# NilsJochem/audio-matcher

Hardware: AMD Instinct MI355X
Metric: audio samples/s matched (whole node), 10 s needle vs 1 h haystack, 1/2/4/8 GPU (higher is better)
Workload: dtype f32

## Files before the change

audio-matcher_amd/build.py:

```python
from __future__ import annotations

import os
import shutil
import subprocess
import sys
from concurrent.futures import ThreadPoolExecutor

HERE = os.path.dirname(os.path.abspath(__file__))
CSRC = os.path.join(HERE, "csrc")
OBJ = os.path.join(HERE, "build")
LIB = os.path.join(HERE, "libaudiomatch_amd.so")
SOURCES = ["am_fft.hip", "am_peaks.hip", "am_context.hip", "am_correlate.hip", "am_engine.hip", "am_stream.hip", "am_monitor.hip", "am_pool.hip", "am_norm.hip", "am_hits.hip", "am_segments.hip", "am_bands.hip", "am_significance.hip", "am_resample.hip", "am_whiten.hip", "am_estimate.hip",
           "am_best.hip", "am_api.hip"]
HEADERS = [os.path.join(CSRC, "am_kernels.h"), os.path.join(CSRC, "am_internal.h"), os.path.join(CSRC, "am_walk.h"), os.path.join(CSRC, "am_spans.h"),
           os.path.join(HERE, "..", "include", "audiomatch.h")]
ARCH = "gfx950"
FLAGS = ["-O3", "-std=c++17", "-fPIC", f"--offload-arch={ARCH}", "-ffp-contract=fast", "-fno-slp-vectorize",
         "-Wall", "-Wno-unused-result"]


def _hipcc() -> str:
    for cand in (shutil.which("hipcc"), "/opt/rocm/bin/hipcc"):
        if cand and os.path.exists(cand):
            return cand
    raise RuntimeError("hipcc not found: the HIP extension cannot be built")


def _stale(target: str, deps: list[str]) -> bool:
    if not os.path.exists(target):
        return True
    t = os.path.getmtime(target)
    return any(os.path.getmtime(d) > t for d in deps if os.path.exists(d))


def build_library(force: bool = False, verbose: bool = False) -> str:
    srcs = [os.path.join(CSRC, s) for s in SOURCES]
    if not force and not _stale(LIB, srcs + HEADERS + [os.path.abspath(__file__)]):
        return LIB
    os.makedirs(OBJ, exist_ok=True)
    hipcc = _hipcc()

    def compile_one(src: str) -> str:
        obj = os.path.join(OBJ, os.path.basename(src) + ".o")
        if force or _stale(obj, [src] + HEADERS + [os.path.abspath(__file__)]):
            cmd = [hipcc, *FLAGS, "-c", src, "-o", obj]
            if verbose:
                print(" ".join(cmd), file=sys.stderr)
            subprocess.check_call(cmd)
        return obj

    with ThreadPoolExecutor(max_workers=len(srcs)) as ex:
        objs = list(ex.map(compile_one, srcs))
    cmd = [hipcc, "-shared", "-fPIC", f"--offload-arch={ARCH}", "-o", LIB, *objs]
    if verbose:
        print(" ".join(cmd), file=sys.stderr)
    subprocess.check_call(cmd)
    return LIB


def build_variant(name: str, defines: list[str]) -> str:
    vdir = os.path.join(OBJ, "variants")
    odir = os.path.join(OBJ, "variants_obj", name)
    os.makedirs(vdir, exist_ok=True)
    os.makedirs(odir, exist_ok=True)
    hipcc = _hipcc()
    objs = []
    for s_ in SOURCES:
        obj = os.path.join(odir, s_ + ".o")
        subprocess.check_call([hipcc, *FLAGS, *[f"-D{d}" for d in defines], "-c", os.path.join(CSRC, s_), "-o", obj])
        objs.append(obj)
    out = os.path.join(vdir, name + ".so")
    subprocess.check_call([hipcc, "-shared", "-fPIC", f"--offload-arch={ARCH}", "-o", out, *objs])
    return out


CLI = os.path.join(HERE, "bin", "audiomatch")
HOST = os.path.join(HERE, "host")


def build_cli(force: bool = False) -> str:
    lib = build_library()
    srcs = [os.path.join(HOST, "audiomatch_cli.cpp"), os.path.join(HOST, "am_host.hpp")]
    if not force and not _stale(CLI, srcs + [lib]):
        return CLI
    os.makedirs(os.path.dirname(CLI), exist_ok=True)
    cmd = [_hipcc(), "-O2", "-std=c++17", "-x", "c++", srcs[0], "-o", CLI,
           f"-L{HERE}", "-laudiomatch_amd", "-Wl,-rpath,$ORIGIN/.."]
    subprocess.check_call(cmd)
    return CLI


PUSHBENCH = os.path.join(HERE, "bin", "pushbench")


def build_pushbench(force: bool = False) -> str:
    lib = build_library()
    src = os.path.join(HOST, "pushbench.cpp")
    if not force and not _stale(PUSHBENCH, [src, lib]):
        return PUSHBENCH
    os.makedirs(os.path.dirname(PUSHBENCH), exist_ok=True)
    subprocess.check_call([_hipcc(), "-O2", "-std=c++17", "-x", "c++", src, "-o", PUSHBENCH,
                           f"-L{HERE}", "-laudiomatch_amd", "-Wl,-rpath,$ORIGIN/.."])
    return PUSHBENCH


def build_selftest() -> str:
    out = os.path.join(OBJ, "am_host_selftest")
    os.makedirs(OBJ, exist_ok=True)
    src = os.path.join(HOST, "selftest.cpp")
    if _stale(out, [src, os.path.join(HOST, "am_host.hpp")]):
        subprocess.check_call(["g++", "-std=c++17", "-O1", "-I", os.path.join(HERE, "..", "include"), "-o", out, src])
    return out


if __name__ == "__main__":
    print(build_library(force="--force" in sys.argv, verbose=True))
    print(build_cli(force="--force" in sys.argv))
    print(build_pushbench(force="--force" in sys.argv))
```

audio-matcher_amd/csrc/am_context.hip:

```cpp
#include "am_internal.h"

namespace am {

thread_local std::string t_err;

int fail(int code, const std::string& msg) {
    t_err = msg;
    return code;
}
int hip_fail(hipError_t e, const char* what) {
    char buf[256];
    snprintf(buf, sizeof(buf), "%s: %s", what, hipGetErrorString(e));
    t_err = buf;
    return e == hipErrorOutOfMemory ? AM_ERR_OOM : AM_ERR_HIP;
}

static std::mutex g_hooks_mu;
static Hooks g_hooks;
Hooks snapshot_hooks() {
    std::lock_guard<std::mutex> lk(g_hooks_mu);
    return g_hooks;
}

using OptRule = const char* (*)(long long& v);
static const char* opt_any(long long&) { return nullptr; }
static const char* opt_bool(long long& v) { v = v ? 1 : 0; return nullptr; }
static const char* opt_log_n(long long& v) { return v != 0 && (v < kLogNMin || v > kLogNMax) ? "log_n out of range" : nullptr; }
static const char* opt_half(long long& v) { v = v <= 0 ? 0 : (v >= 2 ? 2 : 1); return nullptr; }
static const char* opt_every(long long& v) { v = v < 1 ? 1 : v; return nullptr; }
static const char* opt_arm_at(long long& v) { v = v < -1 ? -2 : v; return nullptr; }
static const char* opt_needle_group(long long& v) { return v < 1 || v > kMaxNeedleGroup ? "needle_group out of range" : nullptr; }
static const char* opt_pairs(long long& v) { return v < 1 || v > 64 ? "pairs_per_group out of range" : nullptr; }
static const char* opt_score_norm(long long& v) { return v < 0 || v > 1 ? "score_norm out of range (0 = off, 1 = NCC)" : nullptr; }
static const char* opt_floor_db(long long& v) { return v < 0 || v > 200 ? "score_norm_floor_db out of range (0..200)" : nullptr; }
static const char* opt_distance(long long& v) {
    return v < 0 || v > 3 ? "distance_rule out of range (bit 0: inclusive, bit 1: between plateau starts)" : nullptr;
}
struct Option {
    const char* name;
    std::atomic<long long> value;
    OptRule rule;
    long long Opts::*field;
};
static Option g_options[] = {
    {"log_n", {0}, opt_log_n, &Opts::log_n},
    {"pairs_per_group", {64}, opt_pairs, &Opts::pairs_per_group},
    {"profile_mask", {-1}, opt_any, &Opts::profile_mask},
    {"profile_every", {1}, opt_every, &Opts::profile_every},
    {"half_pipeline", {0}, opt_half, &Opts::half},
    {"batch_overlap", {1}, opt_bool, &Opts::batch_overlap},
    {"needle_group", {8}, opt_needle_group, &Opts::needle_group},
    {"pick_stream_priority", {0}, opt_bool, &Opts::pick_priority},
    {"pick_group", {1}, opt_bool, &Opts::pick_group},
    {"k3_group", {1}, opt_bool, &Opts::k3_group},
    {"host_pick_wait", {1}, opt_bool, &Opts::host_pick_wait},
    {"device_redo", {1}, opt_bool, &Opts::device_redo},
    {"tail_block", {1}, opt_bool, &Opts::tail_block},
    {"dense_scores", {0}, opt_bool, &Opts::dense},
    {"score_norm", {0}, opt_score_norm, &Opts::score_norm},
    {"score_norm_floor_db", {60}, opt_floor_db, &Opts::score_norm_floor_db},
    {"debug_no_realloc", {0}, opt_bool, &Opts::debug_no_realloc},
    {"debug_redo_arm_at", {-2}, opt_arm_at, &Opts::debug_redo_arm_at},
    {"peak_filter_order", {0}, opt_bool, &Opts::peak_filter_order},
    {"distance_rule", {0}, opt_distance, &Opts::distance_rule},
    {"tail_window", {0}, opt_bool, &Opts::tail_window},
    {"surrounding_from", {0}, opt_bool, &Opts::surrounding_from},
};
static Option* find_option(const char* key) {
    for (Option& r : g_options)
        if (!strcmp(key, r.name)) return &r;
    return nullptr;
}

thread_local const Opts* t_opts_pin = nullptr;
Opts snapshot_opts(const am_needle* h) {
    if (t_opts_pin) return *t_opts_pin;
    Opts o;
    for (const Option& r : g_options) o.*r.field = r.value.load(std::memory_order_relaxed);
    if (h && h->opt_log_n >= 0) o.log_n = h->opt_log_n;
    if (h && h->opt_half >= 0) o.half = h->opt_half;
    if (h && h->opt_score_norm >= 0) o.score_norm = h->opt_score_norm;
    return o;
}

thread_local int t_no_realloc = 0;
int realloc_refused(const char* what, size_t bytes, size_t cap) {
    char buf[160];
    snprintf(buf, sizeof(buf), "debug_no_realloc: %s buffer would grow from %zu to %zu bytes while a call is queueing", what, cap, bytes);
    return fail(AM_ERR_HIP, buf);
}

static const char* kKernelNames[] = {"k1_cols_fwd", "k2_rows", "k3_cols_inv", "tile_stats", "peaks", "other"};
static std::mutex g_ctx_mu;
static std::map<int, Ctx*> g_ctx;

int get_ctx(int device, Ctx** out) {
    std::lock_guard<std::mutex> lk(g_ctx_mu);
    int n = 0;
    hipError_t e = hipGetDeviceCount(&n);
    if (e != hipSuccess || n <= 0) return fail(AM_ERR_NO_DEVICE, "no HIP device available");
    if (device < 0 || device >= n) return fail(AM_ERR_NO_DEVICE, "device ordinal out of range");
    auto it = g_ctx.find(device);
    if (it != g_ctx.end()) { *out = it->second; AM_HIP(hipSetDevice(device)); return AM_OK; }
    AM_HIP(hipSetDevice(device));
    (void)hipSetDeviceFlags(hipDeviceScheduleSpin);
    (void)hipGetLastError();
    AM_HIP(fft_kernels_init());
    Ctx* c = new Ctx();
    c->device = device;
    c->hdr.flags = hipHostMallocMapped | hipHostMallocCoherent;
    c->failcnt.flags = hipHostMallocMapped | hipHostMallocCoherent;
    c->spill.flags = hipHostMallocMapped | hipHostMallocCoherent;
    hipError_t se = hipStreamCreateWithFlags(&c->stream, hipStreamNonBlocking);
    if (se != hipSuccess) { delete c; return hip_fail(se, "hipStreamCreate"); }
    {
        int least = 0, greatest = 0;
        if (snapshot_opts(nullptr).pick_priority && hipDeviceGetStreamPriorityRange(&least, &greatest) == hipSuccess && least != greatest)
            (void)hipStreamCreateWithPriority(&c->stream2, hipStreamNonBlocking, least);
        else
            (void)hipStreamCreateWithFlags(&c->stream2, hipStreamNonBlocking);
        (void)hipGetLastError();
    }
    (void)hipStreamCreateWithFlags(&c->stream_tail, hipStreamNonBlocking);
    (void)hipEventCreateWithFlags(&c->ev_fork, kSyncEvent);
    (void)hipEventCreateWithFlags(&c->ev_join, kSyncEvent);
    (void)hipGetLastError();
    for (int i = 0; i < 2; ++i) {
        (void)hipEventCreateWithFlags(&c->ev_k3[i], kSyncEvent);
        (void)hipEventCreateWithFlags(&c->ev_pick[i], kSyncEvent);
    }
    g_ctx[device] = c;
    *out = c;
    return AM_OK;
}

static hipEvent_t prof_event(Ctx* c) {
    if (!c->pool.empty()) { hipEvent_t e = c->pool.back(); c->pool.pop_back(); return e; }
    hipEvent_t e = nullptr;
    (void)hipEventCreateWithFlags(&e, AM_EVENT_NO_SYSTEM_FENCE ? hipEventDisableSystemFence : hipEventDefault);
    return e;
}
ProfScope::ProfScope(Ctx* c_, int name_, hipStream_t st_) : c(c_), name(name_), st(st_ ? st_ : c_->stream) {
    on = c->prof;
    if (on) {
        const Opts o = snapshot_opts(nullptr);
        on = ((o.profile_mask >> name) & 1) && (c->prof_seq[name]++ % (uint64_t)std::max<long long>(1, o.profile_every)) == 0;
    }
    if (on) { e0 = prof_event(c); e1 = prof_event(c); (void)hipEventRecord(e0, st); }
}
static void prof_harvest(Ctx* c) {
    if (c->pending.empty()) return;
    (void)hipStreamSynchronize(c->stream);
    if (c->stream2) (void)hipStreamSynchronize(c->stream2);
    if (c->stream_tail) (void)hipStreamSynchronize(c->stream_tail);
    for (auto& r : c->pending) {
        float ms = 0.f;
        if (hipEventElapsedTime(&ms, r.e0, r.e1) == hipSuccess) { c->prof_ms[r.name] += ms; c->prof_n[r.name] += 1; }
        c->pool.push_back(r.e0); c->pool.push_back(r.e1);
    }
    c->pending.clear();
}

hipError_t copy_on_stream(Ctx* c, void* dst, const void* src, size_t bytes, hipMemcpyKind kind) {
    hipError_t e = hipMemcpyAsync(dst, src, bytes, kind, c->stream);
    if (e != hipSuccess) return e;
    return hipStreamSynchronize(c->stream);
}

static void fill_twiddles(std::vector<float2>& v, size_t off, size_t count, double denom, double mult) {
    for (size_t k = 0; k < count; ++k) {
        const double ang = -2.0 * M_PI * (double)k * mult / denom;
        v[off + k] = make_float2((float)std::cos(ang), (float)std::sin(ang));
    }
}

static void build_mfma_tables(std::vector<unsigned>& tab) {
    tab.assign((size_t)k2_mfma_table_dwords(), 0u);
    auto pack = [](double re, double im) {
        const _Float16 a = (_Float16)re, b = (_Float16)im;
        unsigned short ua, ub;
        memcpy(&ua, &a, 2); memcpy(&ub, &b, 2);
        return (unsigned)ua | ((unsigned)ub << 16);
    };
    auto operand = [&](size_t base, int m_off, int p_off, double denom) {
        for (int ri = 0; ri < 2; ++ri)
            for (int lane = 0; lane < 64; ++lane)
                for (int pp = 0; pp < 4; ++pp) {
                    const int m = m_off + (lane & 15), pt = p_off + 4 * (lane >> 4) + pp;
                    const double ang = 2.0 * M_PI * (double)((m * pt) % (int)denom) / denom;
                    tab[base + (size_t)ri * 256 + (size_t)lane * 4 + pp] = ri == 0 ? pack(std::cos(ang), std::sin(ang)) : pack(-std::sin(ang), std::cos(ang));
                }
    };
    operand(0, 0, 0, 16.0);
    for (int mb = 0; mb < 2; ++mb)
        for (int ks = 0; ks < 2; ++ks) operand(512 + (size_t)(mb * 2 + ks) * 512, 16 * mb, 16 * ks, 32.0);
    const size_t t1 = 512 + 2048, t2 = t1 + 256 * 32;
    for (int t = 0; t < 256; ++t) {
        const int w = t >> 6, g = (t >> 4) & 3, n = t & 15;
        for (int gl = 0; gl < 4; ++gl)
            for (int e = 0; e < 2; ++e)
                for (int r = 0; r < 4; ++r) {
                    const long long m = ((long long)(32 * (4 * w + gl) + 2 * n + e) * (4 * g + r)) % 8192;
                    const double ang = -2.0 * M_PI * (double)m / 8192.0;
                    tab[t1 + (size_t)t * 32 + gl * 8 + e * 4 + r] = pack(std::cos(ang), std::sin(ang));
                }
        for (int ch = 0; ch < 2; ++ch)
            for (int r = 0; r < 4; ++r) {
                const int m = ((16 * ch + n) * (4 * g + r)) % 512;
                const double ang = -2.0 * M_PI * (double)m / 512.0;
                tab[t2 + (size_t)t * 8 + ch * 4 + r] = pack(std::cos(ang), std::sin(ang));
            }
    }
}

int get_plan(Ctx* c, int logN, const Plan** out, int force_logN1) {
    const int key = force_logN1 ? 1000 * force_logN1 + logN : logN;
    auto it = c->plans.find(key);
    if (it != c->plans.end()) { *out = &it->second; return AM_OK; }
    if (logN < kLogNMin || logN > kLogNMax) return fail(AM_ERR_INVALID_ARG, "unsupported transform size");
    Plan p;
    int logN1 = logN - 13;
    if (logN1 < kColsLog) logN1 = kColsLog;
    if (logN1 > 10) logN1 = 10;
    if (force_logN1) logN1 = force_logN1;
    int logN2 = logN - logN1;
    const int logLo = (logN + 1) / 2;
    const size_t n1h = (size_t)1 << (logN1 - 1), n2h = (size_t)1 << (logN2 - 1);
    const size_t nlo = (size_t)1 << logLo, nhi = (size_t)1 << (logN - logLo);
    const size_t f2count = (n1h + n2h + nlo + nhi + 1) & ~(size_t)1;
    const size_t nk2j = logN2 == 13 ? 2 * 256 : 0, nk2c = logN2 == 13 ? 2 * 16 : 0;
    std::vector<float2> host(f2count + 2 * (nlo + nhi + nk2j + nk2c));
    fill_twiddles(host, 0, n1h, (double)(1u << logN1), 1.0);
    fill_twiddles(host, n1h, n2h, (double)(1u << logN2), 1.0);
    fill_twiddles(host, n1h + n2h, nlo, (double)((size_t)1 << logN), 1.0);
    fill_twiddles(host, n1h + n2h + nlo, nhi, (double)((size_t)1 << logN), (double)nlo);
    auto tw = [](double num, double denom) {
        const double ang = -2.0 * M_PI * std::fmod(num, denom) / denom;
        return make_float2((float)std::cos(ang), (float)std::sin(ang));
    };
    const double dN = (double)((size_t)1 << logN);
    size_t o = f2count;
    const size_t o_lo4 = o;
    for (size_t k = 0; k < nlo; ++k) { host[o++] = tw((double)k, dN); host[o++] = tw(4.0 * (double)k, dN); }
    const size_t o_hi4 = o;
    for (size_t k = 0; k < nhi; ++k) { host[o++] = tw((double)k * (double)nlo, dN); host[o++] = tw(4.0 * (double)k * (double)nlo, dN); }
    const size_t o_k2j = o;
    for (size_t t = 0; t < nk2j / 2; ++t) {
        host[o++] = tw(2.0 * t, 8192.0); host[o++] = tw(2.0 * t + 1.0, 8192.0);
        host[o++] = tw(8.0 * t, 8192.0); host[o++] = tw(8.0 * t + 4.0, 8192.0);
    }
    const size_t o_k2c = o;
    for (size_t cidx = 0; cidx < nk2c / 2; ++cidx) {
        host[o++] = tw(32.0 * cidx, 8192.0); host[o++] = tw(32.0 * cidx + 16.0, 8192.0);
        host[o++] = tw(128.0 * cidx, 8192.0); host[o++] = tw(128.0 * cidx + 64.0, 8192.0);
    }
    AM_HIP(hipMalloc((void**)&p.tables, host.size() * sizeof(float2)));
    AM_HIP(copy_on_stream(c, p.tables, host.data(), host.size() * sizeof(float2), hipMemcpyHostToDevice));
    p.dev.logN = logN; p.dev.logN1 = logN1; p.dev.logN2 = logN2; p.dev.logLo = logLo;
    p.dev.tw1 = p.tables;
    p.dev.tw2 = p.tables + n1h;
    p.dev.twlo = p.tables + n1h + n2h;
    p.dev.twhi = p.tables + n1h + n2h + nlo;
    p.dev.twlo4 = reinterpret_cast<const float4*>(p.tables + o_lo4);
    p.dev.twhi4 = reinterpret_cast<const float4*>(p.tables + o_hi4);
    p.dev.k2j = nk2j ? reinterpret_cast<const float4*>(p.tables + o_k2j) : nullptr;
    p.dev.k2c = nk2c ? reinterpret_cast<const float4*>(p.tables + o_k2c) : nullptr;
    p.dev.mf = nullptr;
    if (logN2 == 13) {
        std::vector<unsigned> tab;
        build_mfma_tables(tab);
        AM_HIP(hipMalloc((void**)&p.mf, tab.size() * sizeof(unsigned)));
        AM_HIP(copy_on_stream(c, p.mf, tab.data(), tab.size() * sizeof(unsigned), hipMemcpyHostToDevice));
        p.dev.mf = p.mf;
    }
    auto ins = c->plans.emplace(key, p);
    *out = &ins.first->second;
    return AM_OK;
}

static int needle_spectrum(am_needle* h, const Plan* pl, const float2** out) {
    Ctx* c = h->ctx;
    const int key = pl->dev.logN;
    auto it = h->spectra.find(key);
// ... 27 lines not shown
    std::map<int, unsigned*>& cache = mfma ? h->spectra16m : h->spectra16;
    auto it = cache.find(key);
    if (it != cache.end()) { *out = reinterpret_cast<const float2*>(it->second); return AM_OK; }
    const float2* hc = nullptr;
    int rc = needle_spectrum(h, pl, &hc);
    if (rc) return rc;
    Ctx* c = h->ctx;
    const size_t N = (size_t)1 << pl->dev.logN;
    unsigned* h16 = nullptr;
    AM_HIP(hipMalloc((void**)&h16, N * sizeof(unsigned)));
    hipError_t e;
    { ProfScope ps(c, KN_OTHER);
      e = mfma ? launch_spectrum_to_half_mfma(c->stream, hc, (long long)N, hscale, h16) : launch_spectrum_to_half(c->stream, hc, (long long)N, hscale, h16); }
    if (e == hipSuccess) e = hipStreamSynchronize(c->stream);
    if (e != hipSuccess) { (void)hipFree(h16); return hip_fail(e, "needle spectrum (f16)"); }
    cache[key] = h16;
    *out = reinterpret_cast<const float2*>(h16);
    return AM_OK;
}
HalfScale half_scale(const am_needle* h, const Opts& o, const PlanDev& pl) {
    HalfScale s{0, 1.0f, 1.0f};
    if (!o.half || !(plan_is_r16(pl) || plan_is_c512(pl))) return s;
    s.level = o.half >= 2 ? 2 : 1;
    if (s.level == 1) s.hscale = kHalfGain * h->inv_autocorr;
    else {
        s.pre = 1.0f / 128.0f;
        s.hscale = (float)((double)(1ull << pl.logN) * std::sqrt((double)h->inv_autocorr) / 8.0);
    }
    return s;
}

int needle_k2_spectrum(am_needle* h, const Opts& o, const Plan* pl, const float2** hc, HalfScale* hs) {
    int rc = needle_spectrum(h, pl, hc);
    if (rc) return rc;
    *hs = half_scale(h, o, pl->dev);
    return hs->level == 2 ? needle_spectrum16(h, pl, hs->hscale, hc) : AM_OK;
}

int check_needle(const am_needle* h) {
    if (!h || !h->ctx) return fail(AM_ERR_INVALID_ARG, "null needle handle");
    AM_HIP(hipSetDevice(h->ctx->device));
    return AM_OK;
}

int create_needle_common(Ctx* c, float* d_needle, size_t n, am_needle** out) {
    am_needle* h = new am_needle();
    h->ctx = c; h->d_needle = d_needle; h->n = n;
    const int parts = sumsq_parts((long long)n);
    int rc = c->sum.ensure(sizeof(double) * (size_t)parts);
    if (rc) { (void)hipFree(d_needle); delete h; return rc; }
    hipError_t e = launch_sumsq(c->stream, d_needle, (long long)n, (double*)c->sum.p);
    std::vector<double> part((size_t)parts, 0.0);
    if (e == hipSuccess) e = hipStreamSynchronize(c->stream);
    if (e == hipSuccess) e = copy_on_stream(c, part.data(), c->sum.p, sizeof(double) * (size_t)parts, hipMemcpyDeviceToHost);
    if (e != hipSuccess) { (void)hipFree(d_needle); delete h; return hip_fail(e, "needle energy"); }
    double ss = 0.0;
    for (double v : part) ss += v;
    h->inv_autocorr = (float)(1.0 / ss);
    h->energy = ss;
    *out = h;
    return AM_OK;
}

}

using namespace am;

extern "C" {

int am_needle_create(int device, const float* needle, size_t n, am_needle** out) {
    if (!needle || !out || n == 0) return fail(AM_ERR_INVALID_ARG, "needle must be non-empty");
    Ctx* c = nullptr;
    int rc = get_ctx(device, &c);
    if (rc) return rc;
    std::lock_guard<std::recursive_mutex> lk(c->mu);
    float* d = nullptr;
    AM_HIP(hipMalloc((void**)&d, n * sizeof(float)));
    hipError_t e = copy_on_stream(c, d, needle, n * sizeof(float), hipMemcpyHostToDevice);
    if (e != hipSuccess) { (void)hipFree(d); return hip_fail(e, "copy_on_stream(c, needle)"); }
    return create_needle_common(c, d, n, out);
}

int am_needle_create_device(int device, const float* d_needle, size_t n, am_needle** out) {
    if (!d_needle || !out || n == 0) return fail(AM_ERR_INVALID_ARG, "needle must be non-empty");
    Ctx* c = nullptr;
    int rc = get_ctx(device, &c);
    if (rc) return rc;
    std::lock_guard<std::recursive_mutex> lk(c->mu);
    float* d = nullptr;
    AM_HIP(hipMalloc((void**)&d, n * sizeof(float)));
    hipError_t e = copy_on_stream(c, d, d_needle, n * sizeof(float), hipMemcpyDeviceToDevice);
    if (e != hipSuccess) { (void)hipFree(d); return hip_fail(e, "copy_on_stream(c, needle d2d)"); }
    return create_needle_common(c, d, n, out);
}

void am_needle_destroy(am_needle* h) {
    if (!h) return;
    if (h->ctx) {
        std::lock_guard<std::recursive_mutex> lk(h->ctx->mu);
        (void)hipSetDevice(h->ctx->device);
        (void)hipStreamSynchronize(h->ctx->stream);
        auto free_spectra = [](am_needle* x) {
            for (auto& kv : x->spectra) (void)hipFree(kv.second);
            for (auto* m : {&x->spectra16, &x->spectra16m})
                for (auto& kv : *m) (void)hipFree(kv.second);
        };
        for (am_needle* sub : h->segments) { free_spectra(sub); delete sub; }
        free_spectra(h);
        if (h->d_needle && h->owns_data) (void)hipFree(h->d_needle);
    }
    delete h;
}

int am_needle_len(const am_needle* h, size_t* n) {
    if (!h || !n) return fail(AM_ERR_INVALID_ARG, "null pointer");
    *n = h->n;
    return AM_OK;
}

int am_needle_inv_autocorr(const am_needle* h, float* out) {
    if (!h || !out) return fail(AM_ERR_INVALID_ARG, "null pointer");
    *out = h->inv_autocorr;
    return AM_OK;
}

int am_needle_create_pcm16(int device, const int16_t* interleaved, size_t frames, am_needle** out) {
    if (!interleaved || !out || frames == 0) return fail(AM_ERR_INVALID_ARG, "needle must be non-empty");
    Ctx* c = nullptr;
    int rc = get_ctx(device, &c);
    if (rc) return rc;
    std::lock_guard<std::recursive_mutex> lk(c->mu);
    if ((rc = c->io_in.ensure(frames * 2 * sizeof(int16_t)))) return rc;
    AM_HIP(copy_on_stream(c, c->io_in.p, interleaved, frames * 2 * sizeof(int16_t), hipMemcpyHostToDevice));
    float* d = nullptr;
    AM_HIP(hipMalloc((void**)&d, frames * sizeof(float)));
    hipError_t e = launch_pcm_downmix(c->stream, (const int16_t*)c->io_in.p, (long long)frames, d);
    if (e == hipSuccess) e = hipStreamSynchronize(c->stream);
    if (e != hipSuccess) { (void)hipFree(d); return hip_fail(e, "needle down-mix"); }
    return create_needle_common(c, d, frames, out);
}

int am_shutdown(void) {
    std::lock_guard<std::mutex> lk(g_ctx_mu);
    for (auto& kv : g_ctx) {
        Ctx* c = kv.second;
        std::lock_guard<std::recursive_mutex> lk2(c->mu);
        (void)hipSetDevice(c->device);
        (void)hipStreamSynchronize(c->stream);
        if (c->stream2) (void)hipStreamSynchronize(c->stream2);
        if (c->stream_tail) (void)hipStreamSynchronize(c->stream_tail);
        for (ScoreSide& sd : c->side)
            for (DevBuf* b : {&sd.scores, &sd.stats, &sd.stats32, &sd.wflags, &sd.peaks, &sd.work}) b->release();
        for (DevBuf* b : {&c->work2, &c->segs, &c->redo_pairs[0], &c->redo_pairs[1],
                          &c->io_in, &c->io_out, &c->sum, &c->arena_cur, &c->wide_ctl, &c->wide_list, &c->wide_tiles})
            b->release();
        for (HostBuf* b : {&c->pinned, &c->hdr, &c->spill, &c->badflag, &c->failcnt}) b->release();
        c->ranges.release(); c->range_flags.release(); c->big.release(); c->norm_blk.release();
        for (DevBuf* b : {&c->hit_tab, &c->hit_parts, &c->hit_flags, &c->hit_out, &c->hit_stage}) b->release();
        c->hit_io.release();
        for (DevBuf* b : {&c->sig_span, &c->sig_scores, &c->sig_psum, &c->sig_pmax, &c->sig_mean, &c->sig_hmax}) b->release();
        for (DevBuf* b : {&c->best_stats, &c->best_lmax, &c->best_ctl, &c->best_trans, &c->best_list, &c->best_scores, &c->best_mono}) b->release();
        for (auto& kv : c->rs_taps) kv.second.release();
        c->rs_taps.clear();
        c->lag_parts.release(); c->lag_r.release();
        for (auto& kv : c->band_tabs) kv.second.release();
        c->band_tabs.clear();
        c->work_tail.release(); c->tail_scores.release(); c->tail_stats.release(); c->work_tail2.release();
        for (int set = 0; set < 2; ++set)
            for (int i = 0; i < kMaxNeedleGroup; ++i) { c->grp_scores[set][i].release(); c->grp_stats32[set][i].release(); c->grp_wflags[set][i].release(); }
        for (int i = 0; i < kMaxNeedleGroup; ++i) c->grp_stats[i].release();
        c->segs_resident.clear();
        for (auto& pk : c->plans) { if (pk.second.tables) (void)hipFree(pk.second.tables); if (pk.second.mf) (void)hipFree(pk.second.mf); }
        c->plans.clear();
        for (auto& r : c->pending) { (void)hipEventDestroy(r.e0); (void)hipEventDestroy(r.e1); }
        c->pending.clear();
        for (hipEvent_t e : c->pool) (void)hipEventDestroy(e);
        c->pool.clear();
    }
    return AM_OK;
}

int am_set_progress_callback(am_progress_fn fn, void* user) {
    std::lock_guard<std::mutex> lk(g_hooks_mu);
    g_hooks.fn = fn;
    g_hooks.user = user;
    return AM_OK;
}

int am_set_chunk_progress_callback(am_chunk_progress_fn fn, void* user) {
    std::lock_guard<std::mutex> lk(g_hooks_mu);
    g_hooks.chunk_fn = fn;
    g_hooks.chunk_user = user;
    return AM_OK;
}

int am_profile_enable(int device, int on) {
    Ctx* c = nullptr;
    int rc = get_ctx(device, &c);
    if (rc) return rc;
    std::lock_guard<std::recursive_mutex> lk(c->mu);
    prof_harvest(c);
    c->prof = on != 0;
    return AM_OK;
}
int am_profile_reset(int device) {
    Ctx* c = nullptr;
    int rc = get_ctx(device, &c);
    if (rc) return rc;
    std::lock_guard<std::recursive_mutex> lk(c->mu);
    prof_harvest(c);
    for (int i = 0; i < KN_COUNT; ++i) { c->prof_ms[i] = 0; c->prof_n[i] = 0; }
    return AM_OK;
}
int am_profile_query(int device, const char* kernel, double* total_ms, uint64_t* launches) {
    if (!kernel || !total_ms || !launches) return fail(AM_ERR_INVALID_ARG, "null pointer");
    Ctx* c = nullptr;
    int rc = get_ctx(device, &c);
    if (rc) return rc;
    std::lock_guard<std::recursive_mutex> lk(c->mu);
    prof_harvest(c);
    double ms = 0; uint64_t n = 0; bool found = false;
    for (int i = 0; i < KN_COUNT; ++i) {
        if (!strcmp(kernel, "*") || !strcmp(kernel, kKernelNames[i])) { ms += c->prof_ms[i]; n += c->prof_n[i]; found = true; }
    }
    if (!found) return fail(AM_ERR_INVALID_ARG, "unknown kernel name");
    *total_ms = ms; *launches = n;
    return AM_OK;
}

int am_set_option(const char* key, long long value) {
    if (!key) return fail(AM_ERR_INVALID_ARG, "null key");
    if (!strcmp(key, "k2_mfma")) { set_k2_mfma(value != 0); return AM_OK; }
    Option* r = find_option(key);
    if (!r) return fail(AM_ERR_INVALID_ARG, "unknown option");
    if (const char* err = r->rule(value)) return fail(AM_ERR_INVALID_ARG, err);
    r->value = value;
    return AM_OK;
}
int am_get_option(const char* key, long long* value) {
    if (!key || !value) return fail(AM_ERR_INVALID_ARG, "null pointer");
    if (!strcmp(key, "k2_mfma")) { *value = k2_mfma_enabled() ? 1 : 0; return AM_OK; }
    const Option* r = find_option(key);
    if (!r) return fail(AM_ERR_INVALID_ARG, "unknown option");
    *value = r->value.load();
    return AM_OK;
}

int am_needle_set_option(am_needle* h, const char* key, long long value) {
    if (!h || !h->ctx || !key) return fail(AM_ERR_INVALID_ARG, "null pointer");
    std::lock_guard<std::recursive_mutex> lk(h->ctx->mu);
    if (!strcmp(key, "log_n")) {
        if (value > 0 && (value < kLogNMin || value > kLogNMax)) return fail(AM_ERR_INVALID_ARG, "log_n out of range");
        h->opt_log_n = value < 0 ? -1 : value; return AM_OK;
    }
    if (!strcmp(key, "half_pipeline")) { h->opt_half = value < 0 ? -1 : (value >= 2 ? 2 : (value ? 1 : 0)); return AM_OK; }
    if (!strcmp(key, "score_norm")) {
        if (value > 1) return fail(AM_ERR_INVALID_ARG, "score_norm out of range (-1 = default, 0 = off, 1 = NCC)");
        h->opt_score_norm = value < 0 ? -1 : value; return AM_OK;
    }
    return fail(AM_ERR_INVALID_ARG, "unknown per-handle option (log_n, half_pipeline, score_norm)");
}
int am_needle_get_option(const am_needle* h, const char* key, long long* value) {
    if (!h || !h->ctx || !key || !value) return fail(AM_ERR_INVALID_ARG, "null pointer");
    std::lock_guard<std::recursive_mutex> lk(h->ctx->mu);
    if (!strcmp(key, "log_n")) { *value = h->opt_log_n; return AM_OK; }
    if (!strcmp(key, "half_pipeline")) { *value = h->opt_half; return AM_OK; }
    if (!strcmp(key, "score_norm")) { *value = h->opt_score_norm; return AM_OK; }
    return fail(AM_ERR_INVALID_ARG, "unknown per-handle option (log_n, half_pipeline, score_norm)");
}

}
```

audio-matcher_amd/csrc/am_correlate.hip:

```cpp
#include "am_internal.h"

namespace am {

static int pick_log_n(size_t s, long long out_count, const Opts& o, int* logN_out) {
    int min_log = kLogNMin;
    while (min_log <= kLogNMax && ((size_t)1 << min_log) < s + 1) ++min_log;
    if (min_log > kLogNMax) return fail(AM_ERR_INVALID_ARG, "needle too long for a forced transform size (2^23 at most; leave log_n at 0 for needle partitioning)");
    if (o.log_n > 0) {
        int l = (int)o.log_n;
        if (l < min_log) l = min_log;
        if (l > kLogNMax) l = kLogNMax;
        *logN_out = l;
        return AM_OK;
    }
    const long long span = out_count + (long long)s - 1;
    if (span > (1ll << 19)) {
        if ((long long)s <= kWideFromSamples) { *logN_out = 21; return AM_OK; }
        if ((long long)s <= kWidestFromSamples) {
            long long hop21 = (1ll << 21) - (long long)s + 1;
            if (hop21 >= 8 * kTile) hop21 = (hop21 / kTile) * kTile;
            *logN_out = (hop21 > 0 && out_count <= 2 * hop21) ? 21 : 22;
            return AM_OK;
        }
        if ((long long)s <= kSegmentFrom) {
// ... 143 lines not shown
        const BallotLayout bl = ballot_layout(pp.pl->dev.logN1, pp.pl->dev.logN2);
        const size_t blk = (size_t)(pp.g.nblocks - 1);
        AM_HIP(hipMemsetAsync(main_scan.wbits + blk * bl.words, 0xFF, bl.words * sizeof(unsigned long long), st));
        AM_HIP(hipMemsetD32Async(reinterpret_cast<hipDeviceptr_t>(main_scan.tile_theta + blk * bl.tiles), (int)0xFF7FFFFFu, bl.tiles, st));
    }
    return AM_OK;
}

static int run_correlation_one(am_needle* h, const PassPlan& pp, const void* d_src, long long src_len, long long lead,
                               float* d_dst, long long out_count, float factor,
                               const ScanRequest* scan_req, ScanResult* res, int src_kind, bool accumulate);

int run_correlation(am_needle* h, const Opts& o, const void* d_src, long long src_len, long long lead,
                           float* d_dst, long long out_count, float factor,
                           const ScanRequest* scan_req, ScanResult* res, int src_kind, const PassPlan* plan) {
    int rc;
    PassPlan own;
    if (!plan) {
        if ((rc = pass_plan(h, o, out_count, scan_req && !scan_req->no_scan && lead == 0, &own))) return rc;
        plan = &own;
    }
    if (res) { res->fused = false; res->redo_ok = false; res->sparse = plain_scores(); }
    if (plan->kind != PassKind::Partitioned) return run_correlation_one(h, *plan, d_src, src_len, lead, d_dst, out_count, factor, scan_req, res, src_kind, false);
    if (scan_req && scan_req->skip_launch) return fail(AM_ERR_INVALID_ARG, "internal: streaming ingest does not run early pairs for partitioned needles");
    for (size_t i = 0; i < plan->parts.size(); ++i) {
        ScanRequest plain{};
        if (scan_req) {
            plain.margin = -1.0f; plain.range_a = scan_req->range_a; plain.range_b = scan_req->range_b;
            plain.before_k3 = i == 0 ? scan_req->before_k3 : nullptr;
            plain.no_scan = true;
        }
        if ((rc = run_correlation_one(h->segments[i], plan->parts[i], d_src, src_len, lead - h->seg_off[i], d_dst, out_count, factor,
                                      scan_req ? &plain : nullptr, nullptr, src_kind, i > 0)))
            return rc;
    }
    return AM_OK;
}

static int run_correlation_one(am_needle* h, const PassPlan& pp, const void* d_src, long long src_len, long long lead,
                               float* d_dst, long long out_count, float factor,
                               const ScanRequest* scan_req, ScanResult* res, int src_kind, bool accumulate) {
    Ctx* c = h->ctx;
    Job job{};
    job.src = d_src; job.src_len = src_len; job.lead = lead; job.src_kind = src_kind;
    job.dst = d_dst; job.out_count = out_count;
    if (pp.kind == PassKind::Direct) {
        ProfScope ps(c, KN_OTHER);
        AM_HIP(launch_direct(c->stream, job, h->d_needle, (int)h->n, factor));
        return AM_OK;
    }
    int rc;
    const PlanDev& pl = pp.pl->dev;
    const HalfScale& hs = pp.hs;
    const TailPlan& tail = pp.tail;
    const long long N = pp.g.N, hop = pp.g.hop, npairs = pp.npairs, ppg = pp.ppg;
    const ScanBuffers out = (scan_req && scan_req->out.work) ? scan_req->out : scan_buffers(c->side[0]);
    DevBuf& wk = *out.work;
    if ((rc = wk.ensure((size_t)ppg * (size_t)N * sizeof(float2)))) return rc;
    ScanCfg scan{};
    bool fused = false;
    if (scan_req && !scan_req->no_scan) {
        if (res) res->sparse = SparseScores{nullptr, nullptr, nullptr, (int)hop, pl.logN2, pl.logN1, 1.0 / (double)hop};
        if (pp.fused) {
            const long long side_blocks = std::max(pp.g.nblocks, scan_req->side_nblocks);
            if ((rc = out.stats32->ensure((size_t)((out_count + 31) / 32) * sizeof(float2)))) return rc;
            if ((rc = out.wflags->ensure(sparse_bytes(side_blocks, pl)))) return rc;
            fill_scan_cfg(&scan, out.stats32->p, out.wflags->p, side_blocks, pl, scan_req->margin, scan_req->hist_min, scan_req->seg_c, scan_req->seg_d);
            fused = true;
            if (res) { res->fused = true; res->sparse = sparse_view(scan, hop, pl); }
        }
    }
    const float k3scale = hs.k3(factor);
    job.out_count = pp.main_count; job.hop = (int)hop; job.nblocks = (int)pp.nblocks;
    if (scan_req && scan_req->skip_launch) return AM_OK;
    long long pair_lo = 0, pair_hi = npairs;
    bool with_tail = tail.on;
    if (scan_req && scan_req->range_b > scan_req->range_a) {
        pair_lo = (scan_req->range_a / hop) / 2;
        pair_hi = std::min(npairs, ((scan_req->range_b - 1) / hop) / 2 + 1);
        with_tail = tail.on && scan_req->range_b > tail.T;
    }
    if (scan_req && scan_req->tail_by_caller) with_tail = false;
    if (with_tail) {
        AM_HIP(hipEventRecord(c->ev_fork, c->stream));
        AM_HIP(hipStreamWaitEvent(c->stream_tail, c->ev_fork, 0));
        if ((rc = run_tail_block(c, pp, d_src, src_len, d_dst, out_count, factor, scan, src_kind))) return rc;
        AM_HIP(hipEventRecord(c->ev_join, c->stream_tail));
    }
    bool waited = false;
    for (long long first = pair_lo; first < pair_hi; first += ppg) {
        const int np = (int)std::min(ppg, pair_hi - first);
        job.first_pair = (int)first;
        { ProfScope ps(c, KN_K1); AM_HIP(launch_k1(c->stream, job, np, (float2*)wk.p, pl, hs.level)); }
        { ProfScope ps(c, KN_K2); AM_HIP(launch_k2(c->stream, np, (float2*)wk.p, pp.hc, pl, nullptr, hs.level, hs.hscale, hs.pre)); }
        if (!waited && scan_req && scan_req->before_k3) AM_HIP(hipStreamWaitEvent(c->stream, scan_req->before_k3, 0));
        waited = true;
        { ProfScope ps(c, KN_K3); AM_HIP(launch_k3(c->stream, job, np, (const float2*)wk.p, pl, k3scale, scan, hs.level, accumulate)); }
    }
    if (with_tail) AM_HIP(hipStreamWaitEvent(c->stream, c->ev_join, 0));
    if (res && fused && !accumulate && pair_lo == 0 && pair_hi == npairs && npairs <= ppg) {
        res->redo_ok = true;
        job.first_pair = 0;
        res->redo_job = job; res->redo_pl = pl; res->redo_scale = k3scale; res->redo_half = hs.level;
        res->redo_npairs = (int)npairs; res->redo_work = (const float2*)wk.p; res->redo_cfg = scan;
    }
    return AM_OK;
}

float scale_factor(const am_needle* h, int scale, size_t w) {
    if (scale == AM_SCALE_LIB) return h->inv_autocorr;
    if (scale == AM_SCALE_MY) return h->inv_autocorr / (float)w;
    return 1.0f;
}

static uint64_t start_nanos(uint64_t start, uint32_t sr) {
    const double t = (double)start / (double)sr;
    if (!(t > 0.0)) return 0;
    int e = 0;
    const double m = std::frexp(t, &e);
    const unsigned long long mant = (unsigned long long)std::ldexp(m, 53);
    const int sh = e - 53;
    unsigned __int128 v = (unsigned __int128)mant * 1000000000ull;
    if (sh >= 0) return (uint64_t)(v << sh);
    const int r = -sh;
    if (r >= 127) return 0;
    unsigned __int128 q = v >> r;
    const unsigned __int128 rem = v & (((unsigned __int128)1 << r) - 1);
    const unsigned __int128 half = (unsigned __int128)1 << (r - 1);
    if (rem > half || (rem == half && (q & 1))) ++q;
    return (uint64_t)q;
}

static bool is_overshadowed(const am_peak& element, const am_peak* other, uint32_t sr, double max_distance_s) {
    if (!other) return false;
    uint64_t e = start_nanos(element.start, sr), b = start_nanos(other->start, sr);
    if (e < b) std::swap(e, b);
    const uint64_t maxd = (uint64_t)std::llround(max_distance_s * 1e9);
    return (e - b) < maxd && other->prominence > element.prominence;
}

int upload_segments(Ctx* c, const std::vector<Segment>& segs) {
    const size_t bytes = sizeof(Segment) * segs.size();
    if (c->segs.p && segs.size() == c->segs_resident.size() &&
        memcmp(segs.data(), c->segs_resident.data(), bytes) == 0)
        return AM_OK;
    int rc;
    c->segs_resident.clear();
    if ((rc = c->segs.ensure(bytes))) return rc;
    if ((rc = c->pinned.ensure(bytes))) return rc;
    memcpy(c->pinned.p, segs.data(), bytes);
    AM_HIP(hipMemcpyAsync(c->segs.p, c->pinned.p, bytes, hipMemcpyHostToDevice, c->stream));
    AM_HIP(hipStreamSynchronize(c->stream));
    c->segs_resident = segs;
    return AM_OK;
}

int prepare_results(Ctx* c, size_t nhdr, size_t arena_entries, PeakArena* arena) {
    const size_t hdr_bytes = (sizeof(SegHeader) * nhdr + 63) / 64 * 64;
    int rc;
    if ((rc = c->hdr.ensure(hdr_bytes + sizeof(am_peak) * arena_entries))) return rc;
    if ((rc = c->arena_cur.ensure(sizeof(unsigned)))) return rc;
    AM_HIP(hipMemsetAsync(c->arena_cur.p, 0, sizeof(unsigned), c->stream));
    arena->base = reinterpret_cast<am_peak*>(static_cast<char*>(c->hdr.p) + hdr_bytes);
    arena->cursor = static_cast<unsigned*>(c->arena_cur.p);
    arena->cap = (unsigned)arena_entries;
    return AM_OK;
}

int wide_reserve(Ctx* c, size_t n) {
    int rc;
    if ((rc = c->wide_ctl.ensure(n * kWideCtlBytes))) return rc;
    if ((rc = c->wide_list.ensure(n * AM_MAX_PEAKS_PER_CHUNK * sizeof(am_peak)))) return rc;
    return c->wide_tiles.ensure(n * kWideTileList * sizeof(int));
}
WideState wide_carve(Ctx* c, size_t n) {
    WideState wide{};
    wide.best = static_cast<unsigned long long*>(c->wide_ctl.p);
    wide.state = reinterpret_cast<int*>(wide.best + n);
    wide.count = reinterpret_cast<unsigned*>(wide.state + n);
    wide.seg_min = reinterpret_cast<float*>(wide.state + 2 * n);
    wide.ntiles = wide.state + 3 * n;
    wide.tiles = static_cast<int*>(c->wide_tiles.p);
    wide.list = static_cast<am_peak*>(c->wide_list.p);
    wide.cap = AM_MAX_PEAKS_PER_CHUNK;
    return wide;
}

int launch_pick(Ctx* c, ScoreSide& side, const float* d_scores, long long n_scores, int seg_off, int nsegs,
                       float min_prom, long long min_dist, int* bad, const ScanResult* res, int hdr_off,
                       const PeakArena& arena, const PeakPolicy& pol, hipStream_t st, bool only_failed) {
    if (!st) st = c->stream;
    const SparseScores sp = (res && res->fused) ? res->sparse : plain_scores();
    if (nsegs == 0 || n_scores <= 0) return AM_OK;
    int rc;
    const long long ntiles = (n_scores + kTile - 1) / kTile;
    if ((rc = side.stats.ensure((size_t)ntiles * sizeof(float2)))) return rc;
    if (!only_failed) {
        ProfScope ps(c, KN_STATS, st);
        if (sp.stats32) AM_HIP(launch_stats_reduce(st, sp.stats32, n_scores, (float2*)side.stats.p, bad));
        else AM_HIP(launch_tile_stats(st, d_scores, n_scores, (float2*)side.stats.p, bad));
    }
    if ((rc = wide_reserve(c, (size_t)nsegs))) return rc;
    {
        ProfScope ps(c, KN_PEAKS, st);
        AM_HIP(launch_peaks(st, d_scores, n_scores, (const float2*)side.stats.p,
                            (const Segment*)c->segs.p + seg_off, nsegs, min_prom, min_dist,
                            (am_peak*)side.peaks.p, (SegHeader*)c->hdr.p + hdr_off, sp, arena, wide_carve(c, (size_t)nsegs), only_failed, pol));
    }
    return AM_OK;
}

int pick_chunk_big(Ctx* c, const float* d_scores, long long n_scores, int seg_idx, const Segment& sg,
                          float min_prom, long long min_dist, const ScanResult* res, float seg_min,
                          std::vector<am_peak>& all, const PeakPolicy& pol) {
    const long long a = sg.a, b = std::min(sg.b, n_scores);
    if (b - a >= 0xFFFFFFFFll) return fail(AM_ERR_PEAK_OVERFLOW, "chunk of 2^32 scores or more with more than AM_MAX_PEAKS_PER_CHUNK peaks");
    const SparseScores sp = (res && res->fused) ? res->sparse : plain_scores();
    const DevBuf& stats = c->side[0].stats;
    int rc;
    if ((rc = c->wide_ctl.ensure(kWideCtlBytes))) return rc;
    struct Ctl { unsigned long long best; int state; unsigned count; float seg_min; int ntiles; } ctl{0ull, 7, 0u, seg_min, -1};
    static_assert(sizeof(Ctl) == kWideCtlBytes, "one chunk's control words, in wide_carve's order");
    WideState wide = wide_carve(c, 1);
    wide.tiles = nullptr;
    const Segment* d_seg = (const Segment*)c->segs.p + seg_idx;
    wide.list = nullptr; wide.cap = 0;
    AM_HIP(hipMemcpyAsync(c->wide_ctl.p, &ctl, sizeof(ctl), hipMemcpyHostToDevice, c->stream));
    AM_HIP(launch_peaks_wide_one(c->stream, d_scores, n_scores, (const float2*)stats.p, d_seg, min_prom, min_dist, sp, wide, pol));
    unsigned n = 0;
    AM_HIP(hipMemcpyAsync(&n, wide.count, sizeof(unsigned), hipMemcpyDeviceToHost, c->stream));
    AM_HIP(hipStreamSynchronize(c->stream));
    if (n == 0) return AM_OK;
    if (n >= 0x40000000u) return fail(AM_ERR_PEAK_OVERFLOW, "peak list build failed");
    const size_t nb = min_dist > 0 ? (size_t)((b - a) / min_dist) + 3 : 1;
    const size_t off_out = sizeof(am_peak) * (size_t)n, off_keys = 2 * off_out, off_table = off_keys + 16 * (size_t)n,
                 off_idx = off_table + 8 * nb, off_n = off_idx + 8 * (size_t)n;
    if ((rc = c->big.ensure(off_n + 16))) return rc;
    char* base = static_cast<char*>(c->big.p);
    wide.list = reinterpret_cast<am_peak*>(base); wide.cap = n;
    AM_HIP(hipMemcpyAsync(c->wide_ctl.p, &ctl, sizeof(ctl), hipMemcpyHostToDevice, c->stream));
    AM_HIP(launch_peaks_wide_one(c->stream, d_scores, n_scores, (const float2*)stats.p, d_seg, min_prom, min_dist, sp, wide, pol));
    AM_HIP(hipMemsetAsync(base + off_table, 0xFF, 8 * nb, c->stream));
    AM_HIP(launch_peaks_big_finish(c->stream, wide.list, n, a, min_dist, reinterpret_cast<unsigned long long*>(base + off_keys),
                                   reinterpret_cast<unsigned*>(base + off_idx), reinterpret_cast<long long*>(base + off_table),
                                   reinterpret_cast<am_peak*>(base + off_out), reinterpret_cast<unsigned*>(base + off_n), pol));
    unsigned kept = 0;
    AM_HIP(hipMemcpyAsync(&kept, base + off_n, sizeof(unsigned), hipMemcpyDeviceToHost, c->stream));
    AM_HIP(hipStreamSynchronize(c->stream));
    if (kept > n) return fail(AM_ERR_PEAK_OVERFLOW, "peak filter failed");
    const size_t old = all.size();
    all.resize(old + kept);
    if (kept) {
        AM_HIP(hipMemcpyAsync(all.data() + old, base + off_out, sizeof(am_peak) * (size_t)kept, hipMemcpyDeviceToHost, c->stream));
        AM_HIP(hipStreamSynchronize(c->stream));
    }
    return AM_OK;
}

void make_segments(size_t len, size_t s, const am_match_params* p, bool drop_tail, std::vector<Segment>& segs,
                          std::vector<size_t>* widths, size_t max_windows) {
    const unsigned long long window = p->chunk + p->overlap;
    size_t i = 0;
    for (unsigned long long off = 0; off < len && i < max_windows; off += p->chunk, ++i) {
        const unsigned long long w = std::min<unsigned long long>(window, len - off);
        if (w < s || (drop_tail && w < window)) continue;
        Segment sg; sg.a = (long long)off; sg.b = (long long)(off + w - s + 1);
        segs.push_back(sg);
        if (widths) widths->push_back((size_t)w);
    }
}

int merge_peaks(std::vector<am_peak>& all, const am_match_params* p, bool from_filtered, am_peak* out, size_t cap, size_t* n_out) {
    std::stable_sort(all.begin(), all.end(), [](const am_peak& x, const am_peak& y) { return x.start < y.start; });
    MergeCursor cur;
    std::vector<am_peak> kept;
    merge_settle(p, from_filtered, cur, all.data(), all.size(), 0, true, &kept);
    const size_t n = kept.size();
    for (size_t i = 0; i < n && i < cap; ++i) out[i] = kept[i];
    *n_out = n;
    if (n > cap) return fail(AM_ERR_CAPACITY, "peak output buffer too small");
    return AM_OK;
}

size_t merge_settle(const am_match_params* p, bool from_filtered, MergeCursor& cur, const am_peak* sorted, size_t n,
                    uint64_t horizon, bool ended, std::vector<am_peak>* kept_out) {
    am_peak strongest{};
    strongest.start = horizon;
    strongest.prominence = INFINITY;
    for (size_t i = 0; i < n; ++i) {
        const am_peak& x = sorted[i];
        const am_peak* before = from_filtered ? (cur.has_kept ? &cur.kept : nullptr) : (cur.has_prev ? &cur.prev : nullptr);
        const am_peak* after = i + 1 < n ? &sorted[i + 1] : nullptr;
        const bool shadowed_before = is_overshadowed(x, before, p->sr, p->overshadow_distance_s);
        if (!after && !ended && !shadowed_before && is_overshadowed(x, &strongest, p->sr, p->overshadow_distance_s)) return i;
        if (!shadowed_before && !is_overshadowed(x, after, p->sr, p->overshadow_distance_s)) {
            cur.kept = x; cur.has_kept = true;
            if (kept_out) kept_out->push_back(x);
        }
        cur.prev = x; cur.has_prev = true;
    }
    return n;
}

void append_header_peaks(const SegHeader& hd, const PeakArena& arena, std::vector<am_peak>& all) {
    if (hd.n <= kInlinePeaks) {
        for (int j = 0; j < hd.n; ++j) all.push_back(hd.first[j]);
    } else {
        const am_peak* src = arena.base + hd.arena_off;
        all.insert(all.end(), src, src + hd.n);
    }
}

float write_margin(const Opts& o, const am_match_params* p) {
    return (p->scale != AM_SCALE_MY && !o.dense && p->min_prominence > 0.f) ? 0.5f * p->min_prominence : -1.0f;
}

Job tail_job(const TailPlan& t, const void* d_src, long long src_len, long long out_count, int src_kind) {
    Job job{};
    job.src = advance_src(d_src, (size_t)t.T);
    job.src_len = src_len - t.T; job.lead = 0; job.src_kind = src_kind;
    job.out_count = out_count - t.T; job.hop = (int)t.g.hop; job.nblocks = (int)t.g.nblocks; job.first_pair = 0;
    return job;
}

int nonfinite_flags(Ctx* c, const float* d_src, const Segment* ranges, int n, int* flags) {
    int rc;
    if ((rc = c->ranges.ensure(sizeof(Segment) * n))) return rc;
    if ((rc = c->range_flags.ensure(sizeof(int) * n))) return rc;
    AM_HIP(hipMemcpyAsync(c->ranges.p, ranges, sizeof(Segment) * n, hipMemcpyHostToDevice, c->stream));
    AM_HIP(hipMemsetAsync(c->range_flags.p, 0, sizeof(int) * n, c->stream));
    AM_HIP(launch_nonfinite_ranges(c->stream, d_src, (const Segment*)c->ranges.p, n, (int*)c->range_flags.p));
    AM_HIP(hipMemcpyAsync(flags, c->range_flags.p, sizeof(int) * n, hipMemcpyDeviceToHost, c->stream));
    AM_HIP(hipStreamSynchronize(c->stream));
    return AM_OK;
}
}

extern "C" int am_merge_ready(const am_match_params* p, const am_peak* sorted, size_t n, uint64_t horizon, int ended, size_t* n_ready) {
    using namespace am;
    if (!p || !n_ready || (!sorted && n)) return fail(AM_ERR_INVALID_ARG, "null pointer");
    if (p->sr == 0) return fail(AM_ERR_INVALID_ARG, "p->sr must be > 0");
    *n_ready = 0;
    for (size_t i = 1; i < n; ++i)
        if (sorted[i].start < sorted[i - 1].start) return fail(AM_ERR_INVALID_ARG, "sorted: peaks not sorted by start");
    if (!ended && n && sorted[n - 1].start >= horizon) return fail(AM_ERR_INVALID_ARG, "sorted: a peak starts at or after horizon");
    MergeCursor cur;
    *n_ready = merge_settle(p, snapshot_opts(nullptr).surrounding_from != 0, cur, sorted, n, horizon, ended != 0, nullptr);
    return AM_OK;
}
```

audio-matcher_amd/csrc/am_engine.hip:

```cpp
#include "am_internal.h"

namespace am {

static int launch_pick_group(Ctx* c, const K3Group& kg, long long n_scores, int seg_off, int nsegs, float min_prom, long long min_dist,
                             const SparseScores& sp_common, int* bad, const int* hdr_off, const PeakArena& arena, const PeakPolicy& pol,
                             hipStream_t st) {
    if (nsegs == 0 || n_scores <= 0 || kg.n <= 0) return AM_OK;
    int rc;
    const size_t nz = (size_t)kg.n, total = nz * (size_t)nsegs;
    const long long ntiles = (n_scores + kTile - 1) / kTile;
    PickGroup pg{};
    pg.n = kg.n;
    for (int z = 0; z < kg.n; ++z) {
        if ((rc = c->grp_stats[z].ensure((size_t)ntiles * sizeof(float2)))) return rc;
        pg.g[z] = kg.dst[z]; pg.stats[z] = static_cast<float2*>(c->grp_stats[z].p);
        pg.stats32[z] = kg.stats32[z]; pg.wbits[z] = kg.wbits[z]; pg.theta[z] = kg.tile_theta[z];
        pg.hdr_off[z] = hdr_off[z];
    }
    { ProfScope ps(c, KN_STATS, st);
      AM_HIP(launch_stats_reduce(st, pg.stats32[0], n_scores, pg.stats[0], bad, &pg)); }
    if ((rc = wide_reserve(c, total))) return rc;
    if ((rc = c->side[0].peaks.ensure(total * AM_MAX_PEAKS_PER_CHUNK * sizeof(am_peak)))) return rc;
    {
        ProfScope ps(c, KN_PEAKS, st);
        AM_HIP(launch_peaks(st, pg.g[0], n_scores, pg.stats[0], (const Segment*)c->segs.p + seg_off, nsegs, min_prom, min_dist,
                            (am_peak*)c->side[0].peaks.p, (SegHeader*)c->hdr.p, sp_common, arena, wide_carve(c, total), false, pol, &pg));
    }
    return AM_OK;
}


struct ChunkPlan {
    std::vector<Segment> segs, short_segs;
    std::vector<size_t> widths, short_w;
    std::vector<int> seg_off, short_off;
    std::vector<int> n_chunks;
    size_t max_scores = 0, max_segs = 1;
    int ns(size_t k) const { return seg_off[k + 1] - seg_off[k]; }
    bool too_many(size_t nn) const { return max_segs > (size_t)1 << 18 || segs.size() * nn > (size_t)1 << 24; }
};
static void plan_chunks(size_t s, const void* const* d_hays, const size_t* lens, size_t n_hay, const am_match_params* p, const Opts& o,
                        bool split_short, size_t max_windows, ChunkPlan* cp) {
    const size_t window = (size_t)(p->chunk + p->overlap);
    cp->seg_off.assign(n_hay + 1, 0);
    cp->short_off.assign(n_hay + 1, 0);
    cp->n_chunks.assign(n_hay, 0);
    for (size_t k = 0; k < n_hay; ++k) {
        cp->seg_off[k] = (int)cp->segs.size();
        cp->short_off[k] = (int)cp->short_segs.size();
        if (!d_hays[k] || lens[k] < s) continue;
        std::vector<Segment> one;
        std::vector<size_t> w1;
        make_segments(lens[k], s, p, o.tail_window != 0, one, &w1, max_windows);
        cp->n_chunks[k] = (int)one.size();
        for (size_t i = 0; i < one.size(); ++i) {
            const bool shorter = split_short && w1[i] != window;
            (shorter ? cp->short_segs : cp->segs).push_back(one[i]);
            (shorter ? cp->short_w : cp->widths).push_back(w1[i]);
        }
        if (!one.empty()) cp->max_scores = std::max(cp->max_scores, lens[k] - s + 1);
        cp->max_segs = std::max(cp->max_segs, cp->segs.size() - (size_t)cp->seg_off[k]);
    }
    cp->seg_off[n_hay] = (int)cp->segs.size();
    cp->short_off[n_hay] = (int)cp->short_segs.size();
}

struct ScoreSets {
    Ctx* c;
    bool overlap;
    size_t seq = 0;
    ScoreSets(Ctx* c_, const Opts& o, size_t n_items)
        : c(c_), overlap(o.batch_overlap && n_items > 1 && c_->stream2 && c_->ev_k3[0] && c_->ev_k3[1] && c_->ev_pick[0] && c_->ev_pick[1]) {}
    int count() const { return overlap ? 2 : 1; }
    int set() const { return overlap ? (int)(seq & 1) : 0; }
    ScoreSide& side() const { return c->side[set()]; }
    float* scores() const { return (float*)side().scores.p; }
    hipStream_t pick_stream() const { return overlap ? c->stream2 : c->stream; }
    int size(size_t max_scores, size_t max_segs) {
        int rc;
        for (int set = 0; set < count(); ++set) {
            ScoreSide& sd = c->side[set];
            if ((rc = sd.scores.ensure(max_scores * sizeof(float)))) return rc;
            if ((rc = sd.peaks.ensure(sizeof(am_peak) * max_segs * AM_MAX_PEAKS_PER_CHUNK))) return rc;
            if ((rc = sd.stats.ensure((max_scores + kTile - 1) / kTile * sizeof(float2)))) return rc;
        }
        return wide_reserve(c, max_segs);
    }
    int wait_pick(bool on_host) {
        if (!overlap || seq < 2) return AM_OK;
        if (on_host) AM_HIP(hipEventSynchronize(c->ev_pick[set()]));
        else AM_HIP(hipStreamWaitEvent(c->stream, c->ev_pick[set()], 0));
        return AM_OK;
    }
    int k3_done() {
        if (!overlap) return AM_OK;
        AM_HIP(hipEventRecord(c->ev_k3[set()], c->stream));
        AM_HIP(hipStreamWaitEvent(c->stream2, c->ev_k3[set()], 0));
        return AM_OK;
    }
    int pick_done() {
        if (overlap) AM_HIP(hipEventRecord(c->ev_pick[set()], c->stream2));
        ++seq;
        return AM_OK;
    }
    int drain() {
        AM_HIP(hipStreamSynchronize(c->stream));
        if (overlap) AM_HIP(hipStreamSynchronize(c->stream2));
        return AM_OK;
    }
};

static int match_alone(am_needle* h, const void* d_hay, size_t len, const am_match_params* p, am_peak* out, size_t cap, size_t slot,
                       size_t* n_out, int src_kind, const PartSpec* part, int* worst) {
    const int rc = match_many(h, &d_hay, &len, 1, p, out ? out + slot * cap : nullptr, cap, &n_out[slot], src_kind, 0, 1, false, nullptr, part);
    if (rc == AM_ERR_CAPACITY) *worst = rc;
    return rc == AM_ERR_CAPACITY ? AM_OK : rc;
}

static int pick_alone(am_needle* h, const Opts& o, const am_match_params* p, const void* src, long long src_len, float factor,
                      const ScanRequest& req, long long n_scores, int seg_idx, const Segment& sg, int spare_hdr, uint64_t shift, int src_kind,
                      const NormSpec& nrm, std::vector<am_peak>& all) {
    Ctx* c = h->ctx;
    const PeakPolicy pol = o.peak_policy();
    int rc;
    PeakArena own{};
    if ((rc = c->spill.ensure(sizeof(am_peak) * AM_MAX_PEAKS_PER_CHUNK))) return rc;
    AM_HIP(hipMemsetAsync(c->arena_cur.p, 0, sizeof(unsigned), c->stream));
    own.base = static_cast<am_peak*>(c->spill.p); own.cursor = static_cast<unsigned*>(c->arena_cur.p);
    own.cap = AM_MAX_PEAKS_PER_CHUNK;
    ScoreSide& side = c->side[0];
    if ((rc = side.scores.ensure((size_t)n_scores * sizeof(float)))) return rc;
    float* d_scores = (float*)side.scores.p;
    ScanResult res{};
    if ((rc = run_correlation(h, o, src, src_len, 0, d_scores, n_scores, factor, &req, &res, src_kind))) return rc;
    if (nrm.on) {
        if ((rc = normalise_scores(c, c->stream, nrm, src, src_len, src_kind, 0, (long long)h->n, d_scores, sg.a, std::min(sg.b, n_scores))))
            return rc;
        res.fused = false;
    }
    if ((rc = launch_pick(c, side, d_scores, n_scores, seg_idx, 1, p->min_prominence, (long long)p->min_distance, nullptr, &res, spare_hdr, own, pol))) return rc;
    AM_HIP(hipStreamSynchronize(c->stream));
    const SegHeader& hd = static_cast<const SegHeader*>(c->hdr.p)[spare_hdr];
    const size_t old = all.size();
    if (hd.overflow & 1) {
        if ((rc = pick_chunk_big(c, d_scores, n_scores, seg_idx, sg, p->min_prominence, (long long)p->min_distance, &res, hd.seg_min, all, pol)))
            return rc;
    } else append_header_peaks(hd, own, all);
    for (size_t j = old; j < all.size(); ++j) { all[j].start += shift; all[j].end += shift; }
    return AM_OK;
}

struct TailSlots { size_t scores, stats; };
static bool tail_batchable(const TailPlan& t) { return t.on && t.g.logN == 21; }
static int launch_tail_batch(am_needle* h, const std::vector<PassPlan>& plans, const std::vector<size_t>& members, int half_idx,
                             const TailSlots& sl, const void* const* d_hays, const size_t* lens, float factor, int src_kind) {
    Ctx* c = h->ctx;
    const PassPlan& lead = plans[members[0]];
    const TailPlan& first = lead.tail;
    const Plan* pl = lead.tail_pl;
    const float2* hc = lead.tail_hc;
    const HalfScale& hs = lead.tail_hs;
    TailBatch tb{};
    tb.n = (int)members.size();
    for (int j = 0; j < tb.n; ++j) {
        const size_t k = members[j];
        const size_t slot = (size_t)half_idx * kMaxTailBatch + (size_t)j;
        const Job job = tail_job(plans[k].tail, d_hays[k], (long long)lens[k], (long long)(lens[k] - h->n + 1), src_kind);
        tb.src[j] = job.src;
        tb.src_len[j] = job.src_len;
        tb.out_count[j] = job.out_count;
        tb.dst[j] = static_cast<float*>(c->tail_scores.p) + slot * sl.scores;
        tb.stats32[j] = static_cast<float2*>(c->tail_stats.p) + slot * sl.stats;
    }
    float2* work = static_cast<float2*>(c->work_tail.p);
    { ProfScope ps(c, KN_OTHER); AM_HIP(launch_tail_batch_k1(c->stream, tb, (int)first.g.hop, src_kind, work, pl->dev, hs.level)); }
    { ProfScope ps(c, KN_OTHER); AM_HIP(launch_k2(c->stream, tb.n, work, hc, pl->dev, nullptr, hs.level, hs.hscale, hs.pre, true)); }
    { ProfScope ps(c, KN_OTHER); AM_HIP(launch_tail_batch_k3(c->stream, tb, (int)first.g.hop, work, pl->dev, hs.k3(factor), hs.level)); }
    return AM_OK;
}

static int classify_nonfinite(am_needle* h, const PassPlan& pp, const float* d_hay, size_t len,
                              const std::vector<Segment>& segs, int s0, int s1,
                              std::vector<char>* drop, std::vector<char>* again) {
    Ctx* c = h->ctx;
    const long long s = (long long)h->n;
    const int nch = s1 - s0;
    drop->assign(nch, 0); again->assign(nch, 0);
    std::vector<Segment> ranges;
    for (int i = s0; i < s1; ++i)
        ranges.push_back(Segment{segs[i].a, std::min<long long>((long long)len, segs[i].b + s - 1)});
    const long long npairs = pp.kind == PassKind::Transform ? pp.npairs : 0;
    for (long long q = 0; q < npairs; ++q) ranges.push_back(pp.pair_reads(q, (long long)len));
    if (pp.tail.on) ranges.push_back(pp.tail_reads((long long)len));
    std::vector<int> flags(ranges.size(), 0);
    int rc = nonfinite_flags(c, d_hay, ranges.data(), (int)ranges.size(), flags.data());
    if (rc) return rc;
    for (int i = 0; i < nch; ++i) {
        if (flags[i]) { (*drop)[i] = 1; continue; }
        if (pp.kind == PassKind::Partitioned) { (*again)[i] = 1; continue; }
        const Segment sg = segs[s0 + i];
        for (long long q = 0; q < npairs && !(*again)[i]; ++q)
            if (flags[nch + q] && 2 * q * pp.g.hop < sg.b && (2 * q + 2) * pp.g.hop > sg.a) (*again)[i] = 1;
        if (pp.tail.on && flags[nch + npairs] && pp.tail.T < sg.b) (*again)[i] = 1;
    }
    return AM_OK;
}

int match_many(am_needle* h, const void* const* d_hays, const size_t* lens, size_t n_hay,
               const am_match_params* p, am_peak* out, size_t cap_per_hay, size_t* n_out, int src_kind,
               size_t index_base, size_t index_stride, bool fire_hooks, const StreamPre* pre, const PartSpec* part) {
    Ctx* c = h->ctx;
    const Opts o = snapshot_opts(h);
    const PeakPolicy pol = o.peak_policy();
    Hooks hooks = fire_hooks ? snapshot_hooks() : Hooks{};
    if (part) hooks.fn = nullptr;
    if (part && n_hay != 1) return fail(AM_ERR_INVALID_ARG, "internal: a part is one haystack");
    auto G = [&](size_t k) { return index_base + k * index_stride; };
    const size_t s = h->n;
    if (p->chunk == 0) return fail(AM_ERR_INVALID_ARG, "chunk must be > 0");
    if (p->scale < AM_SCALE_NONE || p->scale > AM_SCALE_MY) return fail(AM_ERR_INVALID_ARG, "bad scale");
    const NormSpec nrm = norm_spec(h, o);
    if (nrm.on && (pre || part)) return fail(AM_ERR_INVALID_ARG, AM_NORM_UNSUPPORTED);
    int rc = norm_check(nrm, p->scale);
    if (rc) return rc;
    const bool my = p->scale == AM_SCALE_MY;
    const float factor = nrm.on ? norm_factor(nrm) : scale_factor(h, p->scale, (size_t)(p->chunk + p->overlap));
    const int sm = p->scale == AM_SCALE_LIB ? 1 : 0;
    ScanRequest base{};
    base.margin = nrm.on ? -1.0f : write_margin(o, p);
    const bool sparse_ok = base.margin >= 0.0f;
    base.hist_min = nrm.on ? FLT_MAX : h->hist_min(sm);
    base.seg_c = (long long)p->chunk;
    base.seg_d = (long long)(p->chunk + p->overlap) - (long long)s;
    for (size_t k = 0; k < n_hay; ++k) n_out[G(k)] = 0;
    ChunkPlan cp;
    plan_chunks(s, d_hays, lens, n_hay, p, o, my, part ? part->max_windows : (size_t)-1, &cp);
    const std::vector<Segment>& segs = cp.segs;
    const std::vector<int>& seg_off = cp.seg_off;
    const size_t nsegs = segs.size();
    if (nsegs == 0 && cp.short_segs.empty()) return AM_OK;
    if (cp.too_many(1)) return fail(AM_ERR_INVALID_ARG, "chunk size too small for this haystack (more than 2^18 chunks)");
    size_t n_active = 0;
    for (size_t k = 0; k < n_hay; ++k) n_active += cp.ns(k) > 0;
    ScoreSets sets(c, o, n_active);
    if ((rc = sets.size(cp.max_scores, cp.max_segs))) return rc;
    std::vector<PassPlan> plans(n_hay);
    Footprint need;
    for (size_t k = 0; k < n_hay; ++k) {
        if (cp.n_chunks[k] == 0 || cp.ns(k) == 0) continue;
        if ((rc = pass_plan(h, o, (long long)(lens[k] - s + 1), pre == nullptr, &plans[k]))) return rc;
        need.take(plans[k].need);
    }
    std::vector<int> tail_slot(n_hay, -1);
    TailSlots tslots{0, 0};
    bool batch_tails = false;
    if (need.work_tail) {
        size_t n_tails = 0;
        for (size_t k = 0; k < n_hay; ++k)
            if (tail_batchable(plans[k].tail)) {
                ++n_tails;
                tslots.scores = std::max(tslots.scores, (size_t)(2 * plans[k].tail.g.hop));
            }
        tslots.stats = tslots.scores / 32;
        batch_tails = sets.overlap && n_tails > 1;
        const size_t nslot = batch_tails ? kMaxTailBatch : 1;
        if ((rc = c->work_tail.ensure(need.work_tail * nslot))) return rc;
        if (batch_tails) {
            if ((rc = c->tail_scores.ensure(2 * kMaxTailBatch * tslots.scores * sizeof(float)))) return rc;
            if ((rc = c->tail_stats.ensure(2 * kMaxTailBatch * tslots.stats * sizeof(float2)))) return rc;
        }
    }
    int tail_batches = 0;
    for (int set = 0; set < sets.count(); ++set) {
        if (need.work && (rc = c->side[set].work.ensure(need.work))) return rc;
        if (pre) continue;
        if (need.stats32 && (rc = c->side[set].stats32.ensure(need.stats32))) return rc;
        if (need.side && (rc = c->side[set].wflags.ensure(need.side))) return rc;
    }
    PeakArena arena{};
    if ((rc = prepare_results(c, nsegs + 1, std::min<size_t>(cp.max_segs * AM_MAX_PEAKS_PER_CHUNK, (size_t)1 << 20) + nsegs * 8, &arena))) return rc;
    std::vector<Segment> resident = segs;
    for (const Segment& sg : cp.short_segs) resident.push_back(Segment{0, sg.b - sg.a});
    const int local_seg = (int)resident.size();
    resident.push_back(Segment{0, std::max<long long>(base.seg_d + 1, 1)});
    if ((rc = upload_segments(c, resident))) return rc;
    if ((rc = c->badflag.ensure(sizeof(int) * n_hay))) return rc;
    int* h_bad = static_cast<int*>(c->badflag.p);
    memset(h_bad, 0, sizeof(int) * n_hay);
    if ((rc = c->failcnt.ensure(nsegs + 1))) return rc;
    if (nrm.on) {
        size_t max_len = 0;
        for (size_t k = 0; k < n_hay; ++k) if (cp.ns(k) > 0) max_len = std::max(max_len, lens[k]);
        if ((rc = norm_reserve(c, (long long)max_len))) return rc;
    }
    unsigned char* h_fail = static_cast<unsigned char*>(c->failcnt.p);
    memset(h_fail, 0, nsegs + 1);
    const bool device_redo = sets.overlap && sparse_ok && !needle_is_segmented(h, o) && o.device_redo != 0;
    if (device_redo) {
        for (int set = 0; set < 2; ++set)
            if ((rc = c->redo_pairs[set].ensure(sizeof(int) * (size_t)std::max<long long>(need.npairs, 1)))) return rc;
    }
    SegHeader* h_hdr = static_cast<SegHeader*>(c->hdr.p);
    auto chunk_events = [&](size_t k, int stage) {
        if (hooks.chunk_fn)
            for (int i = 0; i < cp.n_chunks[k]; ++i)
                hooks.chunk_fn(hooks.chunk_user, G(k), (part ? part->chunk_base : 0) + (size_t)i,
                               part ? part->chunk_total : (size_t)cp.n_chunks[k], stage);
    };
    const bool arm_forced = o.debug_redo_arm_at >= -1;
    bool redo_armed = device_redo && (arm_forced ? o.debug_redo_arm_at == 0 : h->redo_armed_left[sm] > 0);
    QueueingScope queueing(o.debug_no_realloc != 0);
    for (size_t k = 0; k < n_hay; ++k) {
        const int ns = cp.ns(k);
        if (cp.n_chunks[k] == 0) continue;
        if (device_redo && arm_forced) redo_armed = o.debug_redo_arm_at >= 0 && (long long)k >= o.debug_redo_arm_at;
        else if (device_redo && !redo_armed && (k & 3) == 0) {
            const volatile unsigned char* f = h_fail;
            for (int i = 0; i < seg_off[k] && !redo_armed; ++i) redo_armed = f[i] != 0;
        }
        if (hooks.fn) hooks.fn(hooks.user, G(k), 0, (size_t)cp.n_chunks[k]);
        chunk_events(k, 0);
        if (ns == 0) continue;
        const long long out_count = (long long)(lens[k] - s + 1);
        const int set = sets.set();
        const PassPlan& pp = plans[k];
        ScoreSide& side = sets.side();
        float* d_scores = sets.scores();
        ScanRequest req = base;
        req.out = scan_buffers(side);
        if ((rc = sets.wait_pick(o.host_pick_wait != 0))) return rc;
        int* d_redo = nullptr;
        if (redo_armed) {
            AM_HIP(hipMemsetAsync(c->redo_pairs[set].p, 0, sizeof(int) * (size_t)std::max<long long>(pp.g.npairs, 1), c->stream));
            d_redo = static_cast<int*>(c->redo_pairs[set].p);
        }
        int* bad = ((src_kind == 0 || o.half) && std::isfinite(factor)) ? &h_bad[k] : nullptr;
        if (pre) {
            d_scores = pre->scores;
            req.out.stats32 = pre->stats32; req.out.wflags = pre->side;
            req.side_nblocks = pre->layout_nblocks;
            req.range_a = std::min(pre->pairs_done, pp.g.npairs) * 2 * pp.g.hop;
            req.range_b = out_count;
            req.skip_launch = req.range_a >= out_count;
        }
        if (batch_tails && tail_batchable(pp.tail)) {
            if (tail_slot[k] < 0) {
                std::vector<size_t> members;
                for (size_t k2 = k; k2 < n_hay && members.size() < (size_t)kMaxTailBatch; ++k2)
                    if (tail_batchable(plans[k2].tail) && tail_slot[k2] < 0) {
                        tail_slot[k2] = (tail_batches & 1) * kMaxTailBatch + (int)members.size();
                        members.push_back(k2);
                    }
                if ((rc = launch_tail_batch(h, plans, members, tail_batches & 1, tslots, d_hays, lens, factor, src_kind))) return rc;
                ++tail_batches;
            }
            req.tail_by_caller = true;
        }
        ScanResult res{};
        if ((rc = run_correlation(h, o, d_hays[k], (long long)lens[k], 0, d_scores, out_count, factor, &req, &res, src_kind, &pp))) return rc;
        if ((rc = sets.k3_done())) return rc;
        if (req.tail_by_caller && res.fused) {
            const TailPlan& t = pp.tail;
            const BallotLayout bl = ballot_layout(res.sparse.log_n1, res.sparse.log_n2);
            const size_t blk = (size_t)(t.T / res.sparse.hop);
            ProfScope ps(c, KN_OTHER, c->stream2);
            AM_HIP(launch_tail_commit(c->stream2, static_cast<const float*>(c->tail_scores.p) + (size_t)tail_slot[k] * tslots.scores, d_scores + t.T,
                                      out_count - t.T, static_cast<const float2*>(c->tail_stats.p) + (size_t)tail_slot[k] * tslots.stats,
                                      const_cast<float2*>(res.sparse.stats32) + t.T / 32,
                                      res.sparse.wbits ? const_cast<unsigned long long*>(res.sparse.wbits) + blk * bl.words : nullptr, (long long)bl.words,
                                      res.sparse.tile_theta ? const_cast<float*>(res.sparse.tile_theta) + blk * bl.tiles : nullptr, (int)bl.tiles));
        }
        if (res.fused && res.sparse.wbits) {
            res.sparse.fail_flags = h_fail + seg_off[k];
            res.sparse.redo_pairs = (redo_armed && res.redo_ok) ? d_redo : nullptr;
        }
        if (nrm.on) {
            if ((rc = normalise_scores(c, sets.pick_stream(), nrm, d_hays[k], (long long)lens[k], src_kind, 0, (long long)s, d_scores, 0, out_count)))
                return rc;
        }
        if ((rc = launch_pick(c, side, d_scores, out_count, seg_off[k], ns, p->min_prominence,
                              (long long)p->min_distance, bad, nrm.on ? nullptr : &res, seg_off[k], arena, pol, sets.pick_stream()))) return rc;
        if (res.fused && res.sparse.redo_pairs) {
            ScanCfg cfg = res.redo_cfg;
            cfg.margin = -1.0f;
            cfg.only_pairs = d_redo;
            { ProfScope ps(c, KN_OTHER, c->stream2);
              AM_HIP(launch_k3(c->stream2, res.redo_job, res.redo_npairs, res.redo_work, res.redo_pl, res.redo_scale, cfg, res.redo_half)); }
            res.sparse.redo_pairs = nullptr; res.sparse.fail_flags = nullptr;
            if ((rc = launch_pick(c, side, d_scores, out_count, seg_off[k], ns, p->min_prominence, (long long)p->min_distance,
                                  nullptr, &res, seg_off[k], arena, pol, c->stream2, true))) return rc;
        }
        if ((rc = sets.pick_done())) return rc;
    }
    queueing.end();
    if ((rc = sets.drain())) return rc;
    int worst = AM_OK;
    std::vector<am_peak> all;
    std::vector<size_t> retry_f32;
    const int spare_hdr = (int)nsegs;
    for (size_t k = 0; k < n_hay; ++k) {
        const int s0 = seg_off[k], s1 = seg_off[k + 1];
        if (cp.n_chunks[k] == 0) continue;
        const long long out_count = (long long)(lens[k] - s + 1);
        if (h_bad[k] && o.half) { retry_f32.push_back(k); continue; }
        if (!my && !nrm.on && !h_bad[k] && s1 > s0) {
            std::vector<float> mins;
            int failed = 0;
            for (int i = s0; i < s1; ++i) { mins.push_back(h_hdr[i].seg_min); failed += h_fail[i] != 0; }
            std::sort(mins.begin(), mins.end());
            if (failed * 8 > s1 - s0) h->conservative_left[sm] = 64;
            const bool robust = device_redo && h->conservative_left[sm] == 0;
            h->remember_min(sm, robust ? mins[mins.size() / 2] : mins.front());
            if (h->conservative_left[sm] > 0) --h->conservative_left[sm];
            if (failed) h->redo_armed_left[sm] = 64;
            else if (h->redo_armed_left[sm] > 0) --h->redo_armed_left[sm];
        }
        all.clear();
        std::vector<char> drop, again;
        if (h_bad[k]) {
            if ((rc = classify_nonfinite(h, plans[k], (const float*)d_hays[k], lens[k], segs, s0, s1, &drop, &again))) return rc;
        }
        for (int i = s0; i < s1; ++i) {
            if (!drop.empty() && drop[i - s0]) continue;
            const Segment sg = segs[i];
            if (!again.empty() && again[i - s0]) {
                ScanRequest one{};
                one.margin = -1.0f;
                if ((rc = pick_alone(h, o, p, advance_src(d_hays[k], (size_t)sg.a), (long long)cp.widths[i], factor, one, sg.b - sg.a,
                                     local_seg, Segment{0, sg.b - sg.a}, spare_hdr, (uint64_t)sg.a, src_kind, nrm, all))) return rc;
                continue;
            }
            if (!(h_hdr[i].overflow & 7)) { append_header_peaks(h_hdr[i], arena, all); continue; }
            ScanRequest full = base;
            full.margin = -1.0f;
            full.range_a = sg.a; full.range_b = sg.b;
            if ((rc = pick_alone(h, o, p, d_hays[k], (long long)lens[k], factor, full, out_count, i, sg, spare_hdr, 0, src_kind, nrm, all))) return rc;
        }
        for (int i = cp.short_off[k]; i < cp.short_off[k + 1]; ++i) {
            const Segment sg = cp.short_segs[i];
            ScanRequest one{};
            one.margin = -1.0f;
            if ((rc = pick_alone(h, o, p, advance_src(d_hays[k], (size_t)sg.a), (long long)cp.short_w[i], scale_factor(h, p->scale, cp.short_w[i]),
                                 one, sg.b - sg.a, (int)nsegs + i, Segment{0, sg.b - sg.a}, spare_hdr, (uint64_t)sg.a, src_kind, nrm, all))) return rc;
        }
        if (part) {
            for (am_peak& q : all) { q.start += part->first_sample; q.end += part->first_sample; }
            part->raw->insert(part->raw->end(), all.begin(), all.end());
            n_out[G(k)] = all.size();
            rc = AM_OK;
        } else rc = merge_peaks(all, p, o.surrounding_from != 0, out ? out + G(k) * cap_per_hay : nullptr, cap_per_hay, &n_out[G(k)]);
        chunk_events(k, 1);
        if (hooks.fn) hooks.fn(hooks.user, G(k), 1, (size_t)cp.n_chunks[k]);
        if (rc == AM_ERR_CAPACITY) worst = rc;
        else if (rc) return rc;
    }
    for (size_t k : retry_f32) {
        const long long keep = h->opt_half;
        h->opt_half = 0;
        rc = match_alone(h, d_hays[k], lens[k], p, out, cap_per_hay, G(k), n_out, src_kind, part, &worst);
        h->opt_half = keep;
        chunk_events(k, 1);
        if (hooks.fn) hooks.fn(hooks.user, G(k), 1, (size_t)cp.n_chunks[k]);
        if (rc) return rc;
    }
    return worst;
}

int match_multi_many(am_needle* const* needles, size_t nn, const void* const* d_hays, const size_t* lens, size_t n_hay,
                     int src_kind, const am_match_params* p, am_peak* out, size_t cap_per_pair, size_t* n_out,
                     size_t index_base, size_t index_stride, const uint64_t* overlaps, bool varlen) {
    am_needle* h0 = needles[0];
    Ctx* c = h0->ctx;
    const Opts o = snapshot_opts(h0);
    const PeakPolicy pol = o.peak_policy();
    const Hooks hooks = snapshot_hooks();
    auto G = [&](size_t k) { return index_base + k * index_stride; };
    for (size_t j = 0; j < nn; ++j) {
        if (!needles[j] || needles[j]->ctx != c) return fail(AM_ERR_INVALID_ARG, "needles must live on one device");
        if (!varlen && needles[j]->n != h0->n) return fail(AM_ERR_INVALID_ARG, "am_match_multi: needles must have equal length");
    }
    if (o.score_norm) return fail(AM_ERR_INVALID_ARG, AM_NORM_UNSUPPORTED);
    if (p->chunk == 0) return fail(AM_ERR_INVALID_ARG, "chunk must be > 0");
    if (p->scale != AM_SCALE_NONE && p->scale != AM_SCALE_LIB)
        return fail(AM_ERR_INVALID_ARG, "am_match_multi supports AM_SCALE_NONE and AM_SCALE_LIB");
    for (size_t k = 0; k < n_hay; ++k)
        for (size_t j = 0; j < nn; ++j) n_out[G(k) * nn + j] = 0;
    std::vector<am_match_params> pj(nn, *p);
    if (overlaps)
        for (size_t j = 0; j < nn; ++j) pj[j].overlap = overlaps[j];
    int rc, worst = AM_OK;
    std::vector<size_t> ord;
    bool any_segmented = false;
    for (size_t j = 0; j < nn; ++j) {
        if (needle_is_segmented(needles[j], o)) any_segmented = true;
        else ord.push_back(j);
    }
    if (any_segmented)
        for (size_t k = 0; k < n_hay; ++k)
            for (size_t j = 0; j < nn; ++j)
                if (needle_is_segmented(needles[j], o) &&
                    (rc = match_alone(needles[j], d_hays[k], lens[k], &pj[j], out, cap_per_pair, G(k) * nn + j, n_out, src_kind, nullptr, &worst)))
                    return rc;
    if (ord.empty()) return worst;
    std::stable_sort(ord.begin(), ord.end(), [&](size_t a, size_t b) { return needles[a]->n > needles[b]->n; });
    const size_t m = ord.size();
    const size_t s = needles[ord[0]]->n;
    const size_t s_min = needles[ord[m - 1]]->n;
    const int sm = p->scale == AM_SCALE_LIB ? 1 : 0;
    std::vector<ChunkPlan> cps;
    std::vector<std::pair<size_t, uint64_t>> keys;
    std::vector<int> plan_of(m), seg_base, hdr_base(m);
    for (size_t i = 0; i < m; ++i) {
        const size_t j = ord[i];
        const std::pair<size_t, uint64_t> key(needles[j]->n, pj[j].overlap);
        const size_t u = (size_t)(std::find(keys.begin(), keys.end(), key) - keys.begin());
        if (u == keys.size()) {
            keys.push_back(key);
            cps.emplace_back();
            plan_chunks(key.first, d_hays, lens, n_hay, &pj[j], o, false, (size_t)-1, &cps.back());
        }
        plan_of[i] = (int)u;
    }
    std::vector<Segment> all_segs;
    size_t max_scores = 0, max_segs = 1, nhdr = 0;
    bool too_many = false;
    for (const ChunkPlan& cpu : cps) {
        seg_base.push_back((int)all_segs.size());
        all_segs.insert(all_segs.end(), cpu.segs.begin(), cpu.segs.end());
        max_scores = std::max(max_scores, cpu.max_scores);
        max_segs = std::max(max_segs, cpu.max_segs);
        too_many = too_many || cpu.too_many(1);
    }
    for (size_t i = 0; i < m; ++i) { hdr_base[i] = (int)nhdr; nhdr += cps[plan_of[i]].segs.size(); }
    if (nhdr == 0) return worst;
    if (too_many || nhdr > (size_t)1 << 24) return fail(AM_ERR_INVALID_ARG, "chunk size too small for this batch (too many chunks)");
    auto plan_i = [&](size_t i) -> const ChunkPlan& { return cps[plan_of[i]]; };
    auto seg_of = [&](size_t k, size_t i) { return seg_base[plan_of[i]] + plan_i(i).seg_off[k]; };
    auto hdr_of = [&](size_t k, size_t i) { return hdr_base[i] + plan_i(i).seg_off[k]; };
    auto ns_max = [&](size_t k) { int n = 0; for (const ChunkPlan& cpu : cps) n = std::max(n, cpu.ns(k)); return n; };
    auto count_of = [&](size_t k, size_t i) { return (long long)lens[k] - (long long)needles[ord[i]]->n + 1; };
    std::vector<Geometry> geo(n_hay);
    std::vector<TailPlan> tails(n_hay);
    size_t max_matrix = 0, max_wflags = 0, max_tail = 0;
    for (size_t k = 0; k < n_hay; ++k) {
        if (ns_max(k) == 0) continue;
        const long long out_count = (long long)(lens[k] - s_min + 1);
        if ((rc = plan_geometry(s, out_count, o, &geo[k]))) return rc;
        max_matrix = std::max(max_matrix, (size_t)geo[k].npairs * (size_t)geo[k].N);
// ... 244 lines not shown
```

audio-matcher_amd/csrc/am_internal.h:

```cpp
#pragma once
#include <algorithm>
#include <atomic>
#include <cfloat>
#include <cmath>
#include <cstdio>
#include <cstring>
#include <map>
#include <mutex>
#include <string>
#include <vector>

#include "am_kernels.h"
#include "am_spans.h"

namespace am {

extern thread_local std::string t_err;
int fail(int code, const std::string& msg);
int hip_fail(hipError_t e, const char* what);
#define AM_HIP(call)                                         \
    do {                                                     \
        hipError_t e_ = (call);                              \
        if (e_ != hipSuccess) return hip_fail(e_, #call);    \
    } while (0)

struct Hooks {
    am_progress_fn fn = nullptr;
    void* user = nullptr;
    am_chunk_progress_fn chunk_fn = nullptr;
    void* chunk_user = nullptr;
};
Hooks snapshot_hooks();

struct Opts {
    long long log_n, pairs_per_group, half, batch_overlap, needle_group, dense, device_redo, debug_no_realloc, debug_redo_arm_at;
    long long peak_filter_order, distance_rule, tail_window, surrounding_from, k3_group, pick_group, tail_block, host_pick_wait;
    long long profile_mask, profile_every, pick_priority;
    long long score_norm, score_norm_floor_db;
    PeakPolicy peak_policy() const { return PeakPolicy{(int)peak_filter_order, (int)(distance_rule & 1), (int)((distance_rule >> 1) & 1)}; }
};
static const float kHalfGain = 1024.0f;
static const double kMinEfficiency = 0.75;
static const int kLogNMin = 10, kLogNMax = 23;
static const long long kWideFromSamples = 140000;
static const long long kWidestFromSamples = 1500000;
static const long long kSegmentFrom = 1ll << 22;
static const long long kSegmentLen = 1ll << 22;

extern thread_local int t_no_realloc;
struct QueueingScope {
    bool on;
    explicit QueueingScope(bool enable) : on(enable) { if (on) ++t_no_realloc; }
    ~QueueingScope() { end(); }
    void end() { if (on) { --t_no_realloc; on = false; } }
    QueueingScope(const QueueingScope&) = delete;
    QueueingScope& operator=(const QueueingScope&) = delete;
};
int realloc_refused(const char* what, size_t bytes, size_t cap);

struct DevBuf {
    void* p = nullptr;
    size_t cap = 0;
    int ensure(size_t bytes) {
        if (bytes <= cap) return AM_OK;
        if (t_no_realloc > 0) return realloc_refused("a device", bytes, cap);
        release();
        size_t want = bytes + bytes / 8;
        hipError_t e = hipMalloc(&p, want);
        if (e != hipSuccess) {
            e = hipMalloc(&p, bytes);
            want = bytes;
            if (e != hipSuccess) { p = nullptr; return hip_fail(e, "hipMalloc(scratch)"); }
        }
        cap = want;
        return AM_OK;
    }
    void release() {
        if (p) (void)hipFree(p);
        p = nullptr; cap = 0;
    }
};
struct HostBuf {
    void* p = nullptr;
    size_t cap = 0;
    unsigned flags = hipHostMallocDefault;
    int ensure(size_t bytes) {
        if (bytes <= cap) return AM_OK;
        if (t_no_realloc > 0) return realloc_refused("a pinned host", bytes, cap);
        release();
        hipError_t e = hipHostMalloc(&p, bytes, flags);
        if (e != hipSuccess) { p = nullptr; return hip_fail(e, "hipHostMalloc"); }
        cap = bytes;
        return AM_OK;
    }
    void release() {
        if (p) (void)hipHostFree(p);
        p = nullptr; cap = 0;
    }
};

struct Plan {
    PlanDev dev{};
    float2* tables = nullptr;
    unsigned* mf = nullptr;
};

struct ScoreSide { DevBuf scores, stats, stats32, wflags, peaks, work; };

struct ProfRec { int name; hipEvent_t e0, e1; };
enum { KN_K1 = 0, KN_K2, KN_K3, KN_STATS, KN_PEAKS, KN_OTHER, KN_COUNT };

struct Ctx {
    int device = -1;
    hipStream_t stream = nullptr;
    hipStream_t stream2 = nullptr;
    hipStream_t stream_tail = nullptr;
    hipEvent_t ev_fork = nullptr, ev_join = nullptr;
    DevBuf work_tail, tail_scores, tail_stats;
    DevBuf work_tail2;
    std::recursive_mutex mu;
    std::map<int, Plan> plans;
    ScoreSide side[2];
    DevBuf work2, segs, io_in, io_out, sum, arena_cur, wide_ctl, wide_list, wide_tiles;
    DevBuf norm_blk;
    DevBuf hit_tab, hit_parts, hit_flags, hit_out, hit_stage;
    HostBuf hit_io;
    std::map<int, DevBuf> band_tabs;
    DevBuf sig_span, sig_scores, sig_psum, sig_pmax, sig_mean, sig_hmax;
    std::map<std::pair<int, int>, DevBuf> rs_taps;
    DevBuf lag_parts, lag_r;
    DevBuf redo_pairs[2];
    DevBuf grp_scores[2][kMaxNeedleGroup], grp_stats32[2][kMaxNeedleGroup], grp_wflags[2][kMaxNeedleGroup];
    DevBuf grp_stats[kMaxNeedleGroup];
    HostBuf failcnt;
    hipEvent_t ev_k3[2] = {nullptr, nullptr}, ev_pick[2] = {nullptr, nullptr};
    HostBuf pinned;
    HostBuf hdr;
    HostBuf spill;
    HostBuf badflag;
    DevBuf ranges, range_flags;
    DevBuf big;
    DevBuf best_stats, best_lmax, best_ctl, best_trans, best_list, best_scores, best_mono;
    std::vector<Segment> segs_resident;
    bool prof = false;
    std::vector<ProfRec> pending;
    std::vector<hipEvent_t> pool;
    double prof_ms[KN_COUNT] = {0};
    uint64_t prof_n[KN_COUNT] = {0};
    uint64_t prof_seq[KN_COUNT] = {0};
};

#ifndef AM_EVENT_NO_SYSTEM_FENCE
#define AM_EVENT_NO_SYSTEM_FENCE 1
#endif
constexpr unsigned kSyncEvent = hipEventDisableTiming | (AM_EVENT_NO_SYSTEM_FENCE ? hipEventDisableSystemFence : 0u);

int get_ctx(int device, Ctx** out);
struct ProfScope {
    Ctx* c; int name; hipStream_t st; hipEvent_t e0 = nullptr, e1 = nullptr;
    bool on;
    ProfScope(Ctx* c_, int name_, hipStream_t st_ = nullptr);
    ~ProfScope() {
        if (on) { (void)hipEventRecord(e1, st); c->pending.push_back({name, e0, e1}); }
    }
};
hipError_t copy_on_stream(Ctx* c, void* dst, const void* src, size_t bytes, hipMemcpyKind kind);
int get_plan(Ctx* c, int logN, const Plan** out, int force_logN1 = 0);

}

struct am_needle {
    am::Ctx* ctx = nullptr;
    float* d_needle = nullptr;
    size_t n = 0;
    float inv_autocorr = 0.f;
    double energy = 0.0;
    std::map<int, float2*> spectra;
    std::map<int, unsigned*> spectra16;
    std::map<int, unsigned*> spectra16m;
    static constexpr int kRecent = 8;
    float recent_min[2][kRecent];
    int recent_n[2] = {0, 0}, recent_pos[2] = {0, 0};
    void remember_min(int sm, float v) {
        recent_min[sm][recent_pos[sm]] = v;
        recent_pos[sm] = (recent_pos[sm] + 1) % kRecent;
        if (recent_n[sm] < kRecent) ++recent_n[sm];
    }
    int conservative_left[2] = {0, 0};
    int redo_armed_left[2] = {0, 0};
    float hist_min(int sm) const {
        float m = FLT_MAX;
        for (int i = 0; i < recent_n[sm]; ++i) m = std::min(m, recent_min[sm][i]);
        return m;
    }
    long long opt_log_n = -1, opt_half = -1, opt_score_norm = -1;
    std::vector<am_needle*> segments;
    std::vector<long long> seg_off;
    bool owns_data = true;
};

namespace am {

struct ScanBuffers { DevBuf* work; DevBuf* stats32; DevBuf* wflags; };
inline ScanBuffers scan_buffers(ScoreSide& sd) { return ScanBuffers{&sd.work, &sd.stats32, &sd.wflags}; }
struct ScanRequest {
    float margin;
    float hist_min;
    long long seg_c, seg_d;
    ScanBuffers out;
    hipEvent_t before_k3;
    long long range_a, range_b;
    long long side_nblocks;
    bool skip_launch;
    bool tail_by_caller;
    bool no_scan;
};
struct ScanResult {
    bool fused;
    SparseScores sparse;
    bool redo_ok;
    Job redo_job; PlanDev redo_pl; float redo_scale; int redo_half; int redo_npairs; const float2* redo_work; ScanCfg redo_cfg;
};
inline SparseScores plain_scores() { return SparseScores{nullptr, nullptr, nullptr, 1, 5, 5, 1.0}; }
struct Geometry {
    int logN;
    long long N, hop, nblocks, npairs;
};
struct TailPlan {
    bool on;
    long long T;
    Geometry g;
};
struct HalfScale {
    int level;
    float pre, hscale;
    float k3(float factor) const { return level ? factor / (hscale * pre) : factor; }
};
struct Footprint {
    size_t work = 0, stats32 = 0, side = 0, work_tail = 0;
    long long npairs = 0;
    void take(const Footprint& f) {
        work = std::max(work, f.work); stats32 = std::max(stats32, f.stats32); side = std::max(side, f.side);
        work_tail = std::max(work_tail, f.work_tail);
        npairs = std::max(npairs, f.npairs);
    }
};
enum class PassKind { Direct, Partitioned, Transform };
struct PassPlan {
    PassKind kind = PassKind::Direct;
    Geometry g{};
    const Plan* pl = nullptr;
    const float2* hc = nullptr;
    HalfScale hs{};
    bool fused = false;
    TailPlan tail{};
    const Plan* tail_pl = nullptr;
    const float2* tail_hc = nullptr;
    HalfScale tail_hs{};
    long long nblocks = 0, npairs = 0;
    long long ppg = 0;
    long long main_count = 0;
    std::vector<PassPlan> parts;
    Footprint need;
    Segment pair_reads(long long q, long long len) const {
        const long long last_block = (2 * q + 1 < nblocks) ? 2 * q + 1 : 2 * q;
        return Segment{2 * q * g.hop, std::min(len, last_block * g.hop + g.N)};
    }
    Segment tail_reads(long long len) const { return Segment{tail.T, std::min(len, tail.T + (tail.g.nblocks - 1) * tail.g.hop + tail.g.N)}; }
};
struct PartSpec {
    size_t max_windows;
    uint64_t first_sample;
    size_t chunk_base, chunk_total;
    std::vector<am_peak>* raw;
};
struct StreamPre {
    float* scores;
    DevBuf* stats32; DevBuf* side;
    long long pairs_done;
    long long layout_nblocks;
};

inline const void* advance_src(const void* src, size_t elements) {
    return static_cast<const char*>(src) + 4 * elements;
}

Opts snapshot_opts(const am_needle* h);
extern thread_local const Opts* t_opts_pin;
struct OptsPin {
    const Opts* prev;
    explicit OptsPin(const Opts* o) : prev(t_opts_pin) { t_opts_pin = o; }
    ~OptsPin() { t_opts_pin = prev; }
    OptsPin(const OptsPin&) = delete;
    OptsPin& operator=(const OptsPin&) = delete;
};
int check_needle(const am_needle* h);
// ... 4 lines not shown
struct NormSpec { bool on; double energy, thr; };
NormSpec norm_spec(const am_needle* h, const Opts& o);
int norm_check(const NormSpec& ns, int scale);
float norm_factor(const NormSpec& ns);
int norm_reserve(Ctx* c, long long max_src_len);
int normalise_scores(Ctx* c, hipStream_t st, const NormSpec& ns, const void* src, long long src_len, int src_kind, long long lead,
                     long long s, float* scores, long long a, long long b);
#define AM_NORM_UNSUPPORTED "score_norm: not supported by this entry point"

int hit_check_format(int sample_format);
double hit_floor(const am_needle* h);
double hit_floor_ratio(const am_needle* h);
struct HitWhere { long long pair; size_t hay, needle, hit; };
std::string hit_pair_name(const HitWhere& w);
std::string hit_needle_name(long long j);
int hit_check_device(const void* p, int device, const HitWhere& where);
int hit_desc(const am_needle* h, const void* hay, size_t len, int sample_format, const am_peak& pk, double thr,
             const HitWhere& where, HitDesc* d);

int hit_single_prelude(const am_needle* h, int sample_format, size_t n, const void* hay, const am_peak* peaks, const void* out,
                       const void* params, bool* done);
int hit_batch_counts(size_t n_needles, size_t n_hay, int sample_format, const void* needles, const void* d_haystacks, const void* lens,
                     const am_peak* peaks, size_t cap_per_pair, const size_t* n_peaks, const void* out, const void* params, size_t* total);
int hit_batch_needles(const am_needle* const* needles, size_t n_needles);
int stage_spans(Ctx* c, const void* haystack, const HitRange* r, size_t n, const void** at);
int hit_io_reserve(Ctx* c, size_t tab_bytes, size_t out_bytes);
int hit_table_put(Ctx* c, const void* rows, size_t off, size_t bytes);
int hit_results_get(Ctx* c, size_t tab_bytes, size_t out_bytes, const void** res);


template <class F>
int stage_host_spans(const F& f, Ctx* c, const am_needle* h, const void* haystack, size_t len, const am_peak* peaks,
                     std::vector<typename F::Desc>& hits) {
    const size_t n = hits.size();
    std::vector<HitRange> r(n);
    std::vector<const void*> at(n);
    for (size_t i = 0; i < n; ++i) r[i] = f.span(h, (size_t)peaks[i].start, len);
    int rc;
    if ((rc = stage_spans(c, haystack, r.data(), n, at.data()))) return rc;
    for (size_t i = 0; i < n; ++i) {
        const size_t e = (size_t)(static_cast<const char*>(hits[i].win) - static_cast<const char*>(haystack)) / 4;
        hits[i].win = advance_src(at[i], e - r[i].lo);
    }
    return AM_OK;
}

template <class F>
int hit_call(const F& f, bool on_host, const am_needle* h, const void* hay, size_t len, int sample_format, const am_peak* peaks,
             size_t n, typename F::Rec* out) {
    bool done = false;
    int rc = hit_single_prelude(h, sample_format, n, hay, peaks, out, f.params(), &done);
    if (rc || done) return rc;
    if ((rc = f.check_call()) || (rc = f.check(h, -1))) return rc;
    Ctx* c = h->ctx;
    std::lock_guard<std::recursive_mutex> lk(c->mu);
    if (!on_host && (rc = hit_check_device(hay, c->device, HitWhere{-1, 0, 0, 0}))) return rc;
    const double floor = f.floor(h);
    std::vector<typename F::Desc> hits(n);
    std::vector<typename F::Rec*> dst(n);
    for (size_t i = 0; i < n; ++i) {
        if ((rc = f.desc(h, hay, len, sample_format, peaks[i], floor, HitWhere{-1, 0, 0, i}, &hits[i]))) return rc;
        dst[i] = out + i * f.recs();
    }
    if (on_host && (rc = stage_host_spans(f, c, h, hay, len, peaks, hits))) return rc;
    return f.score(c, hits, dst.data());
}

template <class F>
int hit_call_batch(const F& f, const am_needle* const* needles, size_t n_needles, const void* const* d_haystacks, const size_t* lens,
                   size_t n_hay, int sample_format, const am_peak* peaks, size_t cap_per_pair, const size_t* n_peaks,
                   typename F::Rec* out) {
    size_t total = 0;
    int rc = hit_batch_counts(n_needles, n_hay, sample_format, needles, d_haystacks, lens, peaks, cap_per_pair, n_peaks, out, f.params(), &total);
    if (rc || total == 0) return rc;
    if ((rc = f.check_call()) || (rc = hit_batch_needles(needles, n_needles))) return rc;
    for (size_t j = 0; j < n_needles; ++j)
        if ((rc = f.check(needles[j], (long long)j))) return rc;
    Ctx* c = needles[0]->ctx;
    std::lock_guard<std::recursive_mutex> lk(c->mu);
    std::vector<double> floor(n_needles);
    for (size_t j = 0; j < n_needles; ++j) floor[j] = f.floor(needles[j]);
    std::vector<typename F::Desc> hits;
    std::vector<typename F::Rec*> dst;
    hits.reserve(total);
    dst.reserve(total);
    for (size_t k = 0; k < n_hay; ++k) {
        bool checked = false;
        for (size_t j = 0; j < n_needles; ++j) {
            const size_t pair = k * n_needles + j, np = std::min(n_peaks[pair], cap_per_pair);
            if (np == 0) continue;
            if (!checked) {
                const HitWhere w{(long long)pair, k, j, 0};
                if (!d_haystacks[k]) return fail(AM_ERR_INVALID_ARG, hit_pair_name(w) + "null haystack");
                if ((rc = hit_check_device(d_haystacks[k], c->device, w))) return rc;
                checked = true;
            }
            for (size_t i = 0; i < np; ++i) {
                typename F::Desc d{};
                const size_t slot = pair * cap_per_pair + i;
                if ((rc = f.desc(needles[j], d_haystacks[k], lens[k], sample_format, peaks[slot], floor[j], HitWhere{(long long)pair, k, j, i}, &d)))
                    return rc;
                hits.push_back(d);
                dst.push_back(out + slot * f.recs());
            }
        }
    }
    return f.score(c, hits, dst.data());
}

template <class Desc, class Rec, class Launch>
int hit_round_trip(Ctx* c, const std::vector<Desc>& hits, size_t part_bytes, size_t n_parts, size_t recs, Rec* const* out, Launch launch) {
    const size_t n = hits.size(), tab_bytes = sizeof(Desc) * n, out_bytes = sizeof(Rec) * recs * n;
    int rc;
    if ((rc = hit_io_reserve(c, tab_bytes, out_bytes)) || (rc = c->hit_parts.ensure(part_bytes * n_parts)) ||
        (rc = c->hit_flags.ensure(sizeof(unsigned) * n_parts)) || (rc = hit_table_put(c, hits.data(), 0, tab_bytes)))
        return rc;
    {
        ProfScope ps(c, KN_OTHER, c->stream);
        AM_HIP(launch(static_cast<const Desc*>(c->hit_tab.p), static_cast<double*>(c->hit_parts.p), static_cast<unsigned*>(c->hit_flags.p),
                      static_cast<Rec*>(c->hit_out.p)));
    }
    const void* res = nullptr;
    if ((rc = hit_results_get(c, tab_bytes, out_bytes, &res))) return rc;
    for (size_t i = 0; i < n; ++i) std::memcpy(out[i], static_cast<const Rec*>(res) + i * recs, sizeof(Rec) * recs);
    return AM_OK;
}

int estimate_slots(int method, int n);

int plan_geometry(size_t s, long long out_count, const Opts& o, Geometry* g);
bool plan_fuses_scan(const PlanDev& pl, const Geometry& g);
bool tail_plan(size_t s, long long out_count, const Opts& o, const Geometry& g, TailPlan* t);
int pass_plan(am_needle* h, const Opts& o, long long out_count, bool allow_tail, PassPlan* pp);
Job tail_job(const TailPlan& t, const void* d_src, long long src_len, long long out_count, int src_kind);
struct BallotLayout { size_t tiles, words; };
inline BallotLayout ballot_layout(int log_n1, int log_n2) {
    const size_t tiles = (size_t)1 << (log_n2 - kColsLog);
    return BallotLayout{tiles, tiles << (log_n1 - 6)};
}
size_t sparse_bytes(long long nblocks, const PlanDev& pl);
void fill_scan_cfg(ScanCfg* cfg, void* stats32, void* side, long long nblocks, const PlanDev& pl, float margin, float hist_min,
                   long long seg_c, long long seg_d);
SparseScores sparse_view(const ScanCfg& cfg, long long hop, const PlanDev& pl);
bool needle_is_segmented(const am_needle* h, const Opts& o);
float write_margin(const Opts& o, const am_match_params* p);
int run_correlation(am_needle* h, const Opts& o, const void* d_src, long long src_len, long long lead,
                    float* d_dst, long long out_count, float factor, const ScanRequest* scan_req = nullptr, ScanResult* res = nullptr,
                    int src_kind = 0, const PassPlan* plan = nullptr);
int nonfinite_flags(Ctx* c, const float* d_src, const Segment* ranges, int n, int* flags);
float scale_factor(const am_needle* h, int scale, size_t w);
void make_segments(size_t len, size_t s, const am_match_params* p, bool drop_tail, std::vector<Segment>& segs,
                   std::vector<size_t>* widths = nullptr, size_t max_windows = (size_t)-1);
int upload_segments(Ctx* c, const std::vector<Segment>& segs);
int prepare_results(Ctx* c, size_t nhdr, size_t arena_entries, PeakArena* arena);
constexpr size_t kWideCtlBytes = sizeof(unsigned long long) + sizeof(int) + sizeof(unsigned) + sizeof(float) + sizeof(int);
int wide_reserve(Ctx* c, size_t n);
WideState wide_carve(Ctx* c, size_t n);
int launch_pick(Ctx* c, ScoreSide& side, const float* d_scores, long long n_scores, int seg_off, int nsegs,
                float min_prom, long long min_dist, int* bad, const ScanResult* res, int hdr_off,
                const PeakArena& arena, const PeakPolicy& pol, hipStream_t st = nullptr, bool only_failed = false);
int pick_chunk_big(Ctx* c, const float* d_scores, long long n_scores, int seg_idx, const Segment& sg,
                   float min_prom, long long min_dist, const ScanResult* res, float seg_min,
                   std::vector<am_peak>& all, const PeakPolicy& pol);
int find_peaks_host_array(Ctx* c, const float* d_scores, long long n, float min_prom, long long min_dist, std::vector<am_peak>& all);
int valid_scores(am_needle* h, const Opts& o0, const NormSpec& nrm, float factor, const float* d_x, long long w, float* d_out);
int best_transitions(Ctx* c, const float* d_x, long long n, std::vector<long long>& trans);
int best_select(Ctx* c, const float* d_g, long long n, float min_prom, long long min_dist, size_t k, const PeakPolicy& pol,
                std::vector<am_peak>& res);
int match_best_one(am_needle* h, const void* d_hay, size_t len, int sample_format, const am_best_params* bp, am_peak* out,
                   size_t* n_out);
int merge_peaks(std::vector<am_peak>& all, const am_match_params* p, bool from_filtered, am_peak* out, size_t cap, size_t* n_out);
struct MergeCursor { am_peak prev{}, kept{}; bool has_prev = false, has_kept = false; };
size_t merge_settle(const am_match_params* p, bool from_filtered, MergeCursor& cur, const am_peak* sorted, size_t n,
                    uint64_t horizon, bool ended, std::vector<am_peak>* kept_out);
void append_header_peaks(const SegHeader& hd, const PeakArena& arena, std::vector<am_peak>& all);

int match_many(am_needle* h, const void* const* d_hays, const size_t* lens, size_t n_hay,
               const am_match_params* p, am_peak* out, size_t cap_per_hay, size_t* n_out, int src_kind = 0,
               size_t index_base = 0, size_t index_stride = 1, bool fire_hooks = true, const StreamPre* pre = nullptr,
               const PartSpec* part = nullptr);
int match_multi_many(am_needle* const* needles, size_t nn, const void* const* d_hays, const size_t* lens, size_t n_hay,
                     int src_kind, const am_match_params* p, am_peak* out, size_t cap_per_pair, size_t* n_out,
                     size_t index_base = 0, size_t index_stride = 1, const uint64_t* overlaps = nullptr, bool varlen = false);

}
```

audio-matcher_amd/csrc/am_kernels.h:

```cpp
#pragma once

#include <hip/hip_runtime.h>
#include <stdint.h>

#include "../../include/audiomatch.h"

namespace am {

struct Job {
    const void* src;
    long long src_len;
    long long lead;
    float* dst;
    long long out_count;
    int hop;
    int nblocks;
    int first_pair;
    int src_kind;
};

struct PlanDev {
    int logN, logN1, logN2, logLo;
    const float2* tw1;
    const float2* tw2;
    const float2* twlo;
    const float2* twhi;
    const float4* twlo4;
    const float4* twhi4;
    const float4* k2j;
    const float4* k2c;
    const unsigned* mf;
};

constexpr int kColsLog = 5;
constexpr int kCols = 1 << kColsLog;
constexpr int kTile = 1024;
constexpr int kFftThreads = 256;

struct Segment {
    long long a, b;
};

hipError_t launch_k1(hipStream_t st, const Job& job, int npairs, float2* work, const PlanDev& pl, int half = 0);
hipError_t launch_k2(hipStream_t st, int npairs, float2* work, const float2* hc, const PlanDev& pl, float2* dst = nullptr,
                     int half = 0, float hscale = 1.0f, float pre = 1.0f, bool tail = false);
hipError_t launch_spectrum_to_half(hipStream_t st, const float2* hc, long long n, float scale, unsigned* out);
void set_k2_mfma(int on);
bool k2_mfma_enabled();
int k2_mfma_table_dwords();
hipError_t launch_spectrum_to_half_mfma(hipStream_t st, const float2* hc, long long n, float scale, unsigned* out);
hipError_t launch_k2_spectrum(hipStream_t st, float2* work, float2* hc_out, const PlanDev& pl);
constexpr int kMaxNeedleGroup = 8;
struct K2Group {
    const float2* hc[kMaxNeedleGroup];
    float2* dst[kMaxNeedleGroup];
    int n;
};
bool plan_k2_has_group(const PlanDev& pl);
hipError_t launch_k2_group(hipStream_t st, int npairs, const float2* work, const K2Group& grp, const PlanDev& pl);
struct ScanCfg {
    float2* stats32;
    unsigned long long* wbits;
    float* tile_theta;
    float margin;
    float hist_min;
    long long seg_c, seg_d;
    double inv_c;
    const int* only_pairs;
    int redo_tiles;
    static constexpr int kMaxEdgeSlots = 64;
    int edges_n;
    int edge_rel[kMaxEdgeSlots][4];
};
hipError_t launch_k3(hipStream_t st, const Job& job, int npairs, const float2* work,
                     const PlanDev& pl, float out_scale, const ScanCfg& scan, int half = 0, bool accumulate = false);
struct K3Group {
    int n;
    const float2* work[kMaxNeedleGroup];
    float* dst[kMaxNeedleGroup];
    float2* stats32[kMaxNeedleGroup];
    unsigned long long* wbits[kMaxNeedleGroup];
    float* tile_theta[kMaxNeedleGroup];
    float hist_min[kMaxNeedleGroup];
    float out_scale[kMaxNeedleGroup];
    long long out_count[kMaxNeedleGroup];
    long long seg_d[kMaxNeedleGroup];
    long long seg_c;
    double inv_c;
};
bool plan_k3_has_group(const PlanDev& pl);
constexpr int kMaxTailBatch = 8;
struct TailBatch {
    int n;
    const void* src[kMaxTailBatch];
    long long src_len[kMaxTailBatch];
    float* dst[kMaxTailBatch];
    long long out_count[kMaxTailBatch];
    float2* stats32[kMaxTailBatch];
};
hipError_t launch_tail_batch_k1(hipStream_t st, const TailBatch& tb, int hop, int src_kind, float2* work, const PlanDev& pl, int half);
hipError_t launch_tail_batch_k3(hipStream_t st, const TailBatch& tb, int hop, const float2* work, const PlanDev& pl, float out_scale, int half);
hipError_t launch_tail_preset_group(hipStream_t st, const K3Group& grp, long long blk, int log_n1, int log_n2);
hipError_t launch_tail_commit(hipStream_t st, const float* tail_scores, float* scores, long long n, const float2* tail_stats32, float2* stats32,
                              unsigned long long* wbits, long long words, float* theta, int tiles);
hipError_t launch_k3_group(hipStream_t st, const Job& job, int npairs, const K3Group& grp, const PlanDev& pl, const ScanCfg& scan);
constexpr int kDirectMaxNeedle = 64;
hipError_t launch_direct(hipStream_t st, const Job& job, const float* needle, int s, float out_scale);
bool plan_is_r16(const PlanDev& pl);
bool plan_is_c512(const PlanDev& pl);
bool plan_is_c512w(const PlanDev& pl);
bool plan_is_c1024(const PlanDev& pl);
bool plan_has_scan(const PlanDev& pl);
bool plan_k2_is_r16(const PlanDev& pl);
hipError_t fft_kernels_init();

hipError_t launch_nonfinite_ranges(hipStream_t st, const float* x, const Segment* ranges, int nranges, int* flags);
hipError_t launch_tile_stats(hipStream_t st, const float* g, long long n, float2* stats, int* bad = nullptr);
struct PickGroup {
    int n;
    const float* g[kMaxNeedleGroup];
    float2* stats[kMaxNeedleGroup];
    const float2* stats32[kMaxNeedleGroup];
    const unsigned long long* wbits[kMaxNeedleGroup];
    const float* theta[kMaxNeedleGroup];
    int hdr_off[kMaxNeedleGroup];
};
hipError_t launch_stats_reduce(hipStream_t st, const float2* stats32, long long n, float2* stats, int* bad = nullptr,
                               const PickGroup* grp = nullptr);
constexpr int kInlinePeaks = 4;
struct SegHeader {
    int n;
    int overflow;
    float seg_min;
    int arena_off;
    am_peak first[kInlinePeaks];
};
struct PeakArena {
    am_peak* base;
    unsigned* cursor;
    unsigned cap;
};
struct SparseScores {
    const unsigned long long* wbits;
    const float2* stats32;
    const float* tile_theta;
    int hop, log_n2, log_n1;
    double inv_hop;
    int* redo_pairs;
    unsigned char* fail_flags;
};
struct WideState {
    int* state;
    unsigned* count;
    float* seg_min;
    unsigned long long* best;
    am_peak* list;
    unsigned cap;
    int* ntiles;
    int* tiles;
};
constexpr int kWideTileList = 1024;
struct PeakPolicy {
    int order;
    int inclusive;
    int from_start;
};
hipError_t launch_peaks_wide_one(hipStream_t st, const float* g, long long g_len, const float2* stats, const Segment* d_seg,
                                 float min_prom, long long min_dist, const SparseScores& sp, const WideState& wide, const PeakPolicy& pol);
hipError_t launch_peaks_big_finish(hipStream_t st, const am_peak* list, unsigned n, long long a, long long min_dist,
                                   unsigned long long* keys, unsigned* idx, long long* table, am_peak* out, unsigned* out_n,
                                   const PeakPolicy& pol);
hipError_t launch_peaks(hipStream_t st, const float* g, long long g_len, const float2* stats,
                        const Segment* d_segs, int nsegs, float min_prom, long long min_dist,
                        am_peak* d_out, SegHeader* d_hdr, const SparseScores& sp, const PeakArena& arena,
                        const WideState& wide, bool only_failed, const PeakPolicy& pol, const PickGroup* grp = nullptr);
int sumsq_parts(long long n);
hipError_t launch_sumsq(hipStream_t st, const float* x, long long n, double* d_parts);
hipError_t launch_synth(hipStream_t st, float* out, uint32_t seed, uint32_t stream, uint64_t first,
                        long long n, float amp);
hipError_t launch_axpy(hipStream_t st, float* dst, const float* src, long long n, float gain);
hipError_t launch_synth_pcm16(hipStream_t st, int16_t* out, uint32_t seed, uint32_t stream, uint64_t first, long long frames, float amp);
hipError_t launch_add_pcm16(hipStream_t st, int16_t* dst, const int16_t* src, long long frames);
hipError_t launch_pcm_downmix(hipStream_t st, const int16_t* in, long long frames, float* out);

__device__ __forceinline__ float norm_downmix(short2 lr) {
    return __fmul_rn((float)((int)lr.x + (int)lr.y), 0.5f * (1.0f / 65535.0f));
}
typedef __attribute__((address_space(1))) const float gfloat;
typedef __attribute__((address_space(1))) const unsigned guint;
template <int KIND>
__device__ __forceinline__ float hit_sample(const void* win, long long u) {
    return KIND ? norm_downmix(__builtin_bit_cast(short2, ((guint*)win)[u])) : ((gfloat*)win)[u];
}

constexpr int kNormBlock = 1024;
constexpr int kNormTile = 2048;
inline long long norm_blocks(long long src_len) { return (src_len + kNormBlock - 1) / kNormBlock; }
hipError_t launch_block_energy(hipStream_t st, const void* src, long long src_len, int src_kind, double* blk);
struct NormJob {
    const void* src;
    long long src_len;
    int src_kind;
    long long lead, s;
    const double* blk;
    long long nblk;
    double thr;
    float* scores;
    long long a, b;
};
hipError_t launch_norm_scores(hipStream_t st, const NormJob& j);

constexpr int kHitSlice = 4096;
constexpr long long kHitMaxGridY = 65535;
struct HitDesc {
    const void* win;
    const float* needle;
    long long s;
    int kind;
    int edge;
    long long t;
    double en, thr;
    long long part0;
};
hipError_t launch_hit_scores(hipStream_t st, const HitDesc* d_hits, long long n, long long max_slices, int kind, double* parts,
                             unsigned* pflags, am_hit_score* d_out);

constexpr int kSegRadii[3] = {1, 4, 16};
inline int seg_kernel_radius(int r) { return r <= kSegRadii[0] ? kSegRadii[0] : r <= kSegRadii[1] ? kSegRadii[1] : kSegRadii[2]; }
inline int seg_record_len(int rt) { return 2 * (2 * rt + 1) + 1; }
struct SegDesc {
    const void* win;
    const float* needle;
    long long s;
    long long ulo, uhi;
    long long part0;
    double floor_ratio;
    int kind;
    int nsl;
};
hipError_t launch_hit_segments(hipStream_t st, const SegDesc* d_hits, long long n, int m, int r, int max_nsl, int kind,
                               double* parts, unsigned* pflags, am_hit_segment* d_out);

constexpr int kBandGroup = 8;
inline int band_record_len(int n_bands) { return 4 * n_bands + 1; }
struct BandDesc {
    const void* win;
    const float* needle;
    long long nframes;
    long long part0;
    double floor_ratio;
    int kind;
    int ngroups;
};
hipError_t launch_hit_bands(hipStream_t st, const BandDesc* d_hits, long long n, const am_band_params& bp, int max_groups,
                            double empty_ratio, const double* tab, double* parts, unsigned* pflags, am_hit_band* d_out);

constexpr int kSigSlice = 4096;
struct SigDesc {
    long long z0;
    long long nz;
    long long c;
    long long g;
    long long part0;
    unsigned flags;
    unsigned pad;
};
hipError_t launch_hit_significance(hipStream_t st, const SigDesc* d_hits, long long n, long long max_slices, const float* scores,
                                   double* psum, unsigned* pmax, double* mean, unsigned* hmax, am_significance* d_out);

constexpr int kRsThreads = 256;
constexpr int kRsJ = 8;
constexpr int kRsTc = 8;
struct ResampleJob {
    const void* src;
    long long n_in;
    float* dst;
    long long n_out;
    const float* taps;
    int L, M, H, ts;
    int W;
    int xs_cap;
    int tab_lds;
    int vec;
};
hipError_t launch_resample(hipStream_t st, const ResampleJob& j, int kind);

constexpr int kLagBlock = 8192;
constexpr int kLagThreads = 256;
constexpr int kLagChunk = 8;
constexpr int kLagHist = AM_WHITEN_MAX_ORDER + kLagChunk;
inline long long lag_blocks(long long n) { return (n + kLagBlock - 1) / kLagBlock; }
hipError_t launch_lag_products(hipStream_t st, const void* src, long long n, int kind, int vec, int order, double* parts, double* r);
constexpr int kFirThreads = 256;
constexpr int kFirPer = 4;
constexpr int kFirPasses = 2;
constexpr int kFirTile = kFirThreads * kFirPer * kFirPasses;
constexpr int kFirChunk = 8;
constexpr int kFirHist = AM_FIR_MAX_TAPS - 1 + kFirChunk;
struct FirJob {
    const void* src;
    long long n_in, lead;
    float* dst;
    long long n_out;
    int n_taps;
    int vec;
    int vec_out;
    float taps[AM_FIR_MAX_TAPS + kFirChunk - 1];
};
hipError_t launch_fir(hipStream_t st, const FirJob& j, int kind);

struct EstHit {
    const void* src;
// ... 19 lines not shown
```

audio-matcher_amd/csrc/am_peaks.hip:

```cpp
#include "am_kernels.h"

#include <float.h>

namespace am {

constexpr int kPeakThreads = 256;
constexpr int kWaves = kPeakThreads / 64;
constexpr int kQueueCap = kTile / 2;
constexpr int kCandCap = kWideTileList;

#include "am_walk.h"

__global__ void __launch_bounds__(256) tile_stats(const float* __restrict__ g, long long n, float2* __restrict__ stats, int* bad) {
    __shared__ float smin[4], smax[4];
    const long long base = (long long)blockIdx.x * kTile;
    float mn = FLT_MAX, mx = -FLT_MAX;
    bool nf = false;
    for (int i = threadIdx.x; i < kTile; i += 256) {
        const long long idx = base + i;
        if (idx < n) { const float v = g[idx]; mn = fminf(mn, v); mx = fmaxf(mx, v); nf |= not_finite(v); }
    }
    if (nf && bad != nullptr) *bad = 1;
    mn = wave_min(mn); mx = wave_max(mx);
    const int lane = threadIdx.x & 63, wv = threadIdx.x >> 6;
    if (lane == 0) { smin[wv] = mn; smax[wv] = mx; }
    __syncthreads();
    if (threadIdx.x == 0) {
        for (int k = 1; k < 4; ++k) { mn = fminf(mn, smin[k]); mx = fmaxf(mx, smax[k]); }
        stats[blockIdx.x] = make_float2(fminf(mn, smin[0]), fmaxf(mx, smax[0]));
    }
}

__device__ __forceinline__ bool bad_run(float mn, float mx) { return !(mn <= mx) || not_finite(mn) || not_finite(mx); }
__global__ void __launch_bounds__(256) stats_reduce(const float2* __restrict__ s32, long long n32,
                                                    float2* __restrict__ stats, long long ntiles, int* bad, PickGroup grp) {
    if (grp.n > 0) { s32 = grp.stats32[blockIdx.y]; stats = grp.stats[blockIdx.y]; }
    const long long gid = (long long)blockIdx.x * 256 + threadIdx.x;
    const long long tile = gid >> 3;
    const int l = threadIdx.x & 7;
    float mn = FLT_MAX, mx = -FLT_MAX;
    const long long idx = tile * 32 + 4 * l;
    if (tile < ntiles) {
        if (idx + 3 < n32) {
            const float4 a = *reinterpret_cast<const float4*>(s32 + idx);
            const float4 b = *reinterpret_cast<const float4*>(s32 + idx + 2);
            mn = fminf(fminf(a.x, a.z), fminf(b.x, b.z));
            mx = fmaxf(fmaxf(a.y, a.w), fmaxf(b.y, b.w));
            if (bad != nullptr && (bad_run(a.x, a.y) || bad_run(a.z, a.w) || bad_run(b.x, b.y) || bad_run(b.z, b.w))) *bad = 1;
        } else {
            for (int k = 0; k < 4; ++k)
                if (idx + k < n32) {
                    const float2 v = s32[idx + k]; mn = fminf(mn, v.x); mx = fmaxf(mx, v.y);
                    if (bad != nullptr && bad_run(v.x, v.y)) *bad = 1;
                }
        }
    }
#pragma unroll
    for (int o = 4; o > 0; o >>= 1) { mn = fminf(mn, __shfl_xor(mn, o)); mx = fmaxf(mx, __shfl_xor(mx, o)); }
    if (l == 0 && tile < ntiles) stats[tile] = make_float2(mn, mx);
}

struct Cand { long long ps, pe; float h; };

#ifndef AM_PEAK_HALO
#define AM_PEAK_HALO 256
#endif
constexpr int kHalo = AM_PEAK_HALO;
constexpr int kNear = 32;
constexpr int kWin = kTile + 2 * kHalo;
constexpr int kWinRuns = kWin / 32 + 1;

struct ChunkView {
    const float* g;
    const float2* stats;
    SparseScores sp;
    long long a, b;
    float seg_min, min_prom;
    int keep_failed;
};
__device__ __forceinline__ float failed_prom() { return __uint_as_float(0x7FC00000u); }
__device__ __forceinline__ long long dist_pos(const am_peak& pk, int from_start) {
    return from_start ? (long long)pk.start : (long long)((pk.start + pk.end) / 2);
}
__device__ __forceinline__ bool too_close(long long d, long long min_dist, int inclusive) {
    return inclusive ? d <= min_dist : d < min_dist;
}

template <int STEP>
__device__ __forceinline__ bool side_scan(const float* win, int from, int end, float h, float& mn) {
    int j = from;
    while ((end - j) * STEP >= 8) {
        float v[8];
#pragma unroll
        for (int q = 0; q < 8; ++q) v[q] = win[j + q * STEP];
#pragma unroll
        for (int q = 0; q < 8; ++q) {
            if (v[q] > h) return true;
            mn = fminf(mn, v[q]);
        }
        j += 8 * STEP;
    }
    for (; j != end; j += STEP) {
        const float v = win[j];
        if (v > h) return true;
        mn = fminf(mn, v);
    }
    return false;
}

template <int STEP>
__device__ __forceinline__ bool side_scan_wave(const float* win, int from, int end, float h, float& mn, int lane) {
    for (int j = from; (end - j) * STEP > 0; j += 64 * STEP) {
        const int idx = j + lane * STEP;
        const bool valid = (end - idx) * STEP > 0;
        const float v = valid ? win[idx] : 0.0f;
        const unsigned long long higher = __ballot(valid && v > h);
        const int nval = __popcll(__ballot(valid));
        const int ntake = higher ? (__ffsll((long long)higher) - 1) : nval;
        mn = fminf(mn, wave_min(lane < ntake ? v : FLT_MAX));
        if (higher) return true;
    }
    return false;
}

template <class Emit>
__device__ void scan_piece(const ChunkView& cv, long long lo, long long hi, float* win, float2* wruns, Cand* queue, int qcap,
                           int* queue_n, int* overflow, int tid, Emit emit) {
    const int lane = tid & 63, wv = tid >> 6;
    const long long a = cv.a, b = cv.b;
    const long long w_lo = lo - kHalo > a ? lo - kHalo : a;
    const long long w_hi = hi + kHalo < b ? hi + kHalo : b;
    const int wn = (int)(w_hi - w_lo);
    const long long rb0 = w_lo >> 5;
    const int nr = (int)(((w_hi - 1) >> 5) - rb0) + 1;
    if (tid < nr) {
        const long long first = ((rb0 + tid) << 5) > w_lo ? ((rb0 + tid) << 5) : w_lo;
        const bool wr = run_written(cv.sp, first);
        wruns[tid] = make_float2(wr ? 1.0f : 0.0f, wr ? 0.0f : cv.sp.stats32[first >> 5].x);
    }
    __syncthreads();
    {
        float v[kWin / kPeakThreads];
#pragma unroll
        for (int q = 0; q < kWin / kPeakThreads; ++q) {
            const long long i = w_lo + tid + q * kPeakThreads;
            v[q] = (i < w_hi && wruns[(i >> 5) - rb0].x != 0.0f) ? cv.g[i] : 0.0f;
        }
#pragma unroll
        for (int q = 0; q < kWin / kPeakThreads; ++q) {
            const long long i = w_lo + tid + q * kPeakThreads;
            if (i < w_hi) { const float2 f = wruns[(i >> 5) - rb0]; win[i - w_lo] = f.x != 0.0f ? v[q] : f.y; }
        }
    }
    __syncthreads();
    for (int r = tid >> 3; r < nr; r += kPeakThreads >> 3) {
        const long long base = ((rb0 + r) << 5) + (tid & 7) * 4;
        float mn = FLT_MAX, mx = -FLT_MAX;
#pragma unroll
        for (int q = 0; q < 4; ++q)
            if (base + q >= w_lo && base + q < w_hi) { const float v = win[base + q - w_lo]; mn = fminf(mn, v); mx = fmaxf(mx, v); }
#pragma unroll
        for (int o = 4; o > 0; o >>= 1) { mn = fminf(mn, __shfl_xor(mn, o)); mx = fmaxf(mx, __shfl_xor(mx, o)); }
        if ((tid & 7) == 0) wruns[r] = make_float2(mn, mx);
    }
    __syncthreads();
    for (long long i = lo + tid; i < hi; i += kPeakThreads) {
        if (i <= a || i >= b - 1) continue;
        const int wi = (int)(i - w_lo);
        const float x = win[wi];
        if (!((x - cv.seg_min) >= cv.min_prom) || !(win[wi - 1] < x)) continue;
        long long k = i + 1;
        while (k < b - 1 && (k < w_hi ? win[k - w_lo] : score_for_cmp(cv.g, cv.sp, k)) == x) ++k;
        if (!((k < w_hi ? win[k - w_lo] : score_for_cmp(cv.g, cv.sp, k)) < x)) continue;
        {
            const int R = (int)((i >> 5) - rb0);
            const float2 own = wruns[R];
            bool rejected = false;
            if (!((x - own.x) >= cv.min_prom)) {
                rejected = own.y > x;
                float acc = own.x;
                for (int d = 1; !rejected && d <= 8 && R + d < nr; ++d) {
                    const float2 st = wruns[R + d];
                    acc = fminf(acc, st.x);
                    if ((x - acc) >= cv.min_prom) break;
                    rejected = st.y > x;
                }
                acc = own.x;
                for (int d = 1; !rejected && d <= 8 && R - d >= 0; ++d) {
                    const float2 st = wruns[R - d];
                    acc = fminf(acc, st.x);
                    if ((x - acc) >= cv.min_prom) break;
                    rejected = st.y > x;
                }
            }
            if (rejected) { if (cv.keep_failed) emit((long long)i, k, x, failed_prom()); continue; }
        }
// ... 18 lines not shown
    const int qn = *queue_n < qcap ? *queue_n : qcap;
    for (int q = wv; q < qn; q += kWaves) {
        const Cand cd = queue[q];
        if (cd.pe <= w_hi) {
            float lmn = cd.h, rmn = cd.h;
            const bool dl = side_scan_wave<-1>(win, (int)(cd.ps - 1 - w_lo), -1, cd.h, lmn, lane) || w_lo == a;
            if (dl && !((cd.h - lmn) >= cv.min_prom)) { if (cv.keep_failed && lane == 0) emit(cd.ps, cd.pe, cd.h, failed_prom()); continue; }
            const bool dr = side_scan_wave<1>(win, (int)(cd.pe - w_lo), wn, cd.h, rmn, lane) || w_hi == b;
            if (dr && !((cd.h - rmn) >= cv.min_prom)) { if (cv.keep_failed && lane == 0) emit(cd.ps, cd.pe, cd.h, failed_prom()); continue; }
            if (dl && dr) {
                if (lane == 0) emit(cd.ps, cd.pe, cd.h, cd.h - fmaxf(lmn, rmn));
                continue;
            }
        }
        float prom = 0.0f;
        const bool keep = prominence(cv.g, cv.stats, cv.sp, a, b, cd.ps, cd.pe, cd.h, cv.min_prom, lane, prom);
        if (lane == 0 && (keep || cv.keep_failed)) emit(cd.ps, cd.pe, cd.h, keep ? prom : failed_prom());
    }
    __syncthreads();
    if (tid == 0) *queue_n = 0;
    __syncthreads();
}

__device__ void finish_chunk(am_peak* res, int rn, int* order, int overflow, long long min_dist, float seg_min,
                             am_peak* my_out, SegHeader* hd, const PeakArena& arena, int* kept_s, int* spill_off_s, int tid,
                             const PeakPolicy& pol) {
    for (int i = tid; i < rn; i += kPeakThreads) {
        const float hi_ = res[i].height; const uint64_t si = res[i].start;
        int rank = 0;
        for (int j = 0; j < rn; ++j) {
            const float hj = res[j].height;
            if (hj > hi_ || (hj == hi_ && res[j].start < si)) ++rank;
        }
        order[rank] = i;
    }
    __syncthreads();
    if (tid == 0) {
        int kept = 0, nfilt = 0;
        for (int r = 0; r < rn; ++r) {
            const int ir = order[r];
            const am_peak pk = res[ir];
            const long long mid = dist_pos(pk, pol.from_start);
            bool ok = true;
            if (min_dist > 0) {
                for (int k = 0; k < nfilt && ok; ++k) {
                    const long long mk = dist_pos(res[order[k]], pol.from_start);
                    const long long d = mid > mk ? mid - mk : mk - mid;
                    if (too_close(d, min_dist, pol.inclusive)) ok = false;
                }
            }
            if (!ok) continue;
            order[nfilt++] = ir;
            if (pol.order && !(pk.prominence == pk.prominence)) continue;
            if (kept < kInlinePeaks) hd->first[kept] = pk;
            my_out[kept++] = pk;
        }
        int off = -1, ovf = overflow;
        if (kept > kInlinePeaks && arena.base != nullptr) {
            const unsigned o = atomicAdd(arena.cursor, (unsigned)kept);
            if (o + (unsigned)kept <= arena.cap) off = (int)o;
            else ovf |= 4;
        }
        *kept_s = kept; *spill_off_s = off;
        hd->n = kept;
        hd->overflow = ovf;
        hd->seg_min = seg_min;
        hd->arena_off = off;
    }
    __syncthreads();
    if (*spill_off_s >= 0) {
        __threadfence_block();
        for (int i = tid; i < *kept_s; i += kPeakThreads) arena.base[*spill_off_s + i] = my_out[i];
    }
}

__device__ __forceinline__ unsigned long long best_key(float h, long long rel) {
    unsigned u = __float_as_uint(h + 0.0f);
    u = (u & 0x80000000u) ? ~u : (u | 0x80000000u);
    return ((unsigned long long)u << 32) | (unsigned long long)(0xFFFFFFFFu - (unsigned)rel);
}
__device__ void finish_best(const ChunkView& cv, unsigned long long key, am_peak* my_out, SegHeader* hd,
                            long long* pe_s, int tid) {
    const int lane = tid & 63, wv = tid >> 6;
    if (key == 0ull) {
        if (tid == 0) { hd->n = 0; hd->overflow = 0; hd->seg_min = cv.seg_min; hd->arena_off = -1; }
        return;
    }
    unsigned u = (unsigned)(key >> 32);
    u = (u & 0x80000000u) ? (u & 0x7FFFFFFFu) : ~u;
    const long long ps = cv.a + (long long)(0xFFFFFFFFu - (unsigned)(key & 0xFFFFFFFFull));
    const float hk = __uint_as_float(u), hs = score_for_cmp(cv.g, cv.sp, ps);
    const float h = hs == hk ? hs : hk;
    if (tid == 0) {
        long long k = ps + 1;
        while (k < cv.b - 1 && score_for_cmp(cv.g, cv.sp, k) == h) ++k;
        *pe_s = k;
    }
    __syncthreads();
    if (wv == 0) {
        float prom = 0.0f;
        const bool keep = prominence(cv.g, cv.stats, cv.sp, cv.a, cv.b, ps, *pe_s, h, cv.min_prom, lane, prom);
        if (lane == 0) {
            if (keep) {
                am_peak pk; pk.start = (uint64_t)ps; pk.end = (uint64_t)*pe_s; pk.height = h; pk.prominence = prom;
                hd->first[0] = pk;
                my_out[0] = pk;
            }
            hd->n = keep ? 1 : 0; hd->overflow = 0; hd->seg_min = cv.seg_min; hd->arena_off = -1;
        }
    }
}

constexpr int kWideTiles = 0;
constexpr int kWideParts = 64;
constexpr int kWideRows = 16;
constexpr int kWideQueue = kTile / 2;

constexpr int kBoundSteps = 32;
__device__ __forceinline__ bool tile_can_qualify(const float2* tiles, long long t, long long tf, long long tl, float min_prom) {
    const float2* stats = tiles - tf;
    const float2 own = stats[t];
    const float M = own.y;
    float L = own.x;
    if ((M - L) >= min_prom) return true;
    for (long long u = t - 1, n = 0; u >= tf && n < kBoundSteps; --u, ++n) {
        const float2 v = stats[u];
        L = fminf(L, v.x);
        if ((M - L) >= min_prom) break;
        if (v.y > M) return false;
    }
    float R = own.x;
    for (long long u = t + 1, n = 0; u < tl && n < kBoundSteps; ++u, ++n) {
        const float2 v = stats[u];
        R = fminf(R, v.x);
        if ((M - R) >= min_prom) break;
        if (v.y > M) return false;
    }
    return true;
}

__device__ __forceinline__ void pick_group_view(const PickGroup& grp, unsigned z, unsigned nsegs, const float*& g, const float2*& stats,
                                                SparseScores& sp, SegHeader*& hdr, am_peak*& out, WideState& wide) {
    g = grp.g[z];
    stats = grp.stats[z];
    sp.stats32 = grp.stats32[z]; sp.wbits = grp.wbits[z]; sp.tile_theta = grp.theta[z];
    hdr += grp.hdr_off[z];
    const size_t zs = (size_t)z * nsegs;
    if (out != nullptr) out += zs * AM_MAX_PEAKS_PER_CHUNK;
    wide.state += zs; wide.count += zs; wide.seg_min += zs; wide.best += zs; wide.ntiles += zs;
    if (wide.tiles != nullptr) wide.tiles += zs * kWideTileList;
    if (wide.list != nullptr) wide.list += zs * wide.cap;
}

__global__ void __launch_bounds__(kPeakThreads)
peaks_kernel(const float* g, long long g_len, const float2* stats,
             const Segment* __restrict__ segs, float min_prom, long long min_dist,
             am_peak* out, SegHeader* hdr, SparseScores sp, PeakArena arena, WideState wide,
             int only_failed, PeakPolicy pol, PickGroup grp) {
    __shared__ float red[kWaves];
    __shared__ float seg_min_s;
    __shared__ Cand queue[kQueueCap];
    __shared__ int queue_n;
    __shared__ am_peak res[AM_MAX_PEAKS_PER_CHUNK];
    __shared__ int res_n;
    __shared__ int order[AM_MAX_PEAKS_PER_CHUNK];
    __shared__ int overflow;
    __shared__ int cand_tiles[kCandCap];
    __shared__ int cand_n;
    __shared__ int kept_s, spill_off_s;
    __shared__ float win[kWin];
    __shared__ float2 wruns[kWinRuns];
    __shared__ unsigned long long best_s;
    __shared__ long long pe_s;

    const int tid = threadIdx.x, lane = tid & 63, wv = tid >> 6;
    if (grp.n > 0) pick_group_view(grp, blockIdx.y, gridDim.x, g, stats, sp, hdr, out, wide);
    const Segment sg = segs[blockIdx.x];
    const long long a = sg.a, b = sg.b < g_len ? sg.b : g_len;
    am_peak* my_out = out + (size_t)blockIdx.x * AM_MAX_PEAKS_PER_CHUNK;
    if (tid == 0) { queue_n = 0; res_n = 0; overflow = 0; cand_n = 0; best_s = 0ull; wide.state[blockIdx.x] = 0; }
    if (only_failed && !(hdr[blockIdx.x].overflow & 2)) return;
    if (b - a < 3) {
        if (tid == 0) { hdr[blockIdx.x].n = 0; hdr[blockIdx.x].overflow = 0; hdr[blockIdx.x].seg_min = 0.f; hdr[blockIdx.x].arena_off = -1; }
        return;
    }
    const long long tf = (a + kTile - 1) / kTile;
    const long long tl = b / kTile;
    const bool has_full = tl > tf;
    const long long head_hi = has_full ? tf * kTile : b;
    const long long tail_lo = has_full ? tl * kTile : b;
    float2* tstats = reinterpret_cast<float2*>(res);
    constexpr long long kStage = (long long)(sizeof(res) / (sizeof(float2)));
    const long long nfull = has_full ? tl - tf : 0;
    const bool staged = nfull <= kStage;

    float mn = FLT_MAX;
    for (long long i = a + tid; i < head_hi; i += kPeakThreads) mn = fminf(mn, score_for_min(g, sp, i));
    for (long long i = tail_lo + tid; i < b; i += kPeakThreads) mn = fminf(mn, score_for_min(g, sp, i));
    if (has_full) for (long long t = tf + tid; t < tl; t += kPeakThreads) mn = fminf(mn, stats[t].x);
    mn = wave_min(mn);
    if (lane == 0) red[wv] = mn;
    __syncthreads();
    if (tid == 0) seg_min_s = fminf(fminf(red[0], red[1]), fminf(red[2], red[3]));
    __syncthreads();
    const float seg_min = seg_min_s;
    if (sp.wbits != nullptr) {
        __shared__ float th_s[kWaves];
        const int tiles = 1 << (sp.log_n2 - kColsLog);
        const long long b0 = a / sp.hop, b1 = (b - 1) / sp.hop;
        float th = -FLT_MAX;
        for (long long i = b0 * tiles + tid; i < (b1 + 1) * tiles; i += kPeakThreads) th = fmaxf(th, sp.tile_theta[i]);
        th = wave_max(th);
        if (lane == 0) th_s[wv] = th;
        __syncthreads();
        th = fmaxf(fmaxf(th_s[0], th_s[1]), fmaxf(th_s[2], th_s[3]));
        if (!((th - seg_min) < min_prom)) {
            if (tid == 0) { hdr[blockIdx.x].n = 0; hdr[blockIdx.x].overflow = 2; hdr[blockIdx.x].seg_min = seg_min; hdr[blockIdx.x].arena_off = -1; }
            if (sp.redo_pairs != nullptr)
                for (long long q = (b0 >> 1) + tid; q <= (b1 >> 1); q += kPeakThreads) sp.redo_pairs[q] = 1;
            if (tid == 0 && sp.fail_flags != nullptr) sp.fail_flags[blockIdx.x] = 1;
            return;
        }
    }

    {
        __shared__ float bestv_s[kWaves];
        __shared__ long long bestp_s[kWaves];
        __shared__ long long peak_i_s, peak_k_s;
        __shared__ int fast_s;
        float bv = -FLT_MAX;
        long long bp = 0x7fffffffffffffffll;
        auto take = [&](float v, long long pos) { if (v > bv || (v == bv && pos < bp)) { bv = v; bp = pos; } };
        for (long long i = a + tid; i < head_hi; i += kPeakThreads) take(score_for_cmp(g, sp, i), i);
        for (long long i = tail_lo + tid; i < b; i += kPeakThreads) take(score_for_cmp(g, sp, i), i);
        if (has_full) for (long long t = tf + tid; t < tl; t += kPeakThreads) take(stats[t].y, t * kTile);
#pragma unroll
        for (int o = 32; o > 0; o >>= 1) {
            const float ov = __shfl_xor(bv, o);
            const int olo = __shfl_xor((int)(bp & 0xffffffffll), o), ohi = __shfl_xor((int)(bp >> 32), o);
            take(ov, ((long long)ohi << 32) | (unsigned)olo);
        }
        if (lane == 0) { bestv_s[wv] = bv; bestp_s[wv] = bp; }
        if (tid == 0) { peak_i_s = 0x7fffffffffffffffll; fast_s = 0; }
        __syncthreads();
        bv = bestv_s[0]; bp = bestp_s[0];
        for (int k = 1; k < kWaves; ++k) take(bestv_s[k], bestp_s[k]);
        const float M = bv;
        if (!((M - seg_min) >= min_prom)) {
            if (tid == 0) { hdr[blockIdx.x].n = 0; hdr[blockIdx.x].overflow = 0; hdr[blockIdx.x].seg_min = seg_min; hdr[blockIdx.x].arena_off = -1; }
            return;
        }
        if (min_dist >= b - a) {
            const bool in_tile = has_full && bp >= tf * kTile && bp < tl * kTile;
            if (in_tile) {
                long long first = 0x7fffffffffffffffll;
                for (int q = tid; q < kTile; q += kPeakThreads)
                    if (score_for_cmp(g, sp, bp + q) == M && bp + q < first) first = bp + q;
                if (first != 0x7fffffffffffffffll) atomicMin((unsigned long long*)&peak_i_s, (unsigned long long)first);
            } else if (tid == 0) peak_i_s = bp;
            __syncthreads();
            const long long pi = peak_i_s;
            if (tid == 0) {
                long long k = pi + 1;
                bool ok = pi > a && pi < b - 1;
                if (ok) {
                    while (k < b - 1 && score_for_cmp(g, sp, k) == M) ++k;
                    ok = score_for_cmp(g, sp, k) < M;
                }
                peak_k_s = k;
                fast_s = ok ? 1 : 0;
            }
            __syncthreads();
            if (fast_s) {
                __shared__ float side_s[2][kWaves];
                const long long pk_end = peak_k_s;
                float lm = M, rm = M;
                {
                    auto range_min = [&](long long lo, long long hi) {
                        float m = FLT_MAX;
                        long long t0 = (lo + kTile - 1) / kTile, t1 = hi / kTile;
                        if (t0 < tf) t0 = tf;
                        if (t1 > tl) t1 = tl;
                        if (!has_full || t0 >= t1) {
                            for (long long i = lo + tid; i < hi; i += kPeakThreads) m = fminf(m, score_for_min(g, sp, i));
                            return m;
                        }
                        for (long long i = lo + tid; i < t0 * kTile; i += kPeakThreads) m = fminf(m, score_for_min(g, sp, i));
                        for (long long t = t0 + tid; t < t1; t += kPeakThreads) m = fminf(m, stats[t].x);
                        for (long long i = t1 * kTile + tid; i < hi; i += kPeakThreads) m = fminf(m, score_for_min(g, sp, i));
                        return m;
                    };
                    const float l = wave_min(range_min(a, pi)), r = wave_min(range_min(pk_end, b));
                    if (lane == 0) { side_s[0][wv] = l; side_s[1][wv] = r; }
                }
                __syncthreads();
                if (wv == 0) {
                    for (int k = 0; k < kWaves; ++k) { lm = fminf(lm, side_s[0][k]); rm = fminf(rm, side_s[1][k]); }
                    const float hM = score_for_cmp(g, sp, pi);
                    const float prom = hM - fmaxf(lm, rm);
                    const bool keep = prom >= min_prom;
                    if (lane == 0) {
                        if (keep) {
                            am_peak pk; pk.start = (uint64_t)pi; pk.end = (uint64_t)peak_k_s; pk.height = hM; pk.prominence = prom;
                            hdr[blockIdx.x].first[0] = pk;
                            my_out[0] = pk;
                            hdr[blockIdx.x].n = 1; hdr[blockIdx.x].overflow = 0; hdr[blockIdx.x].seg_min = seg_min; hdr[blockIdx.x].arena_off = -1;
                            fast_s = 2;
                        } else if (pol.order) {
                            hdr[blockIdx.x].n = 0; hdr[blockIdx.x].overflow = 0; hdr[blockIdx.x].seg_min = seg_min; hdr[blockIdx.x].arena_off = -1;
                            fast_s = 2;
                        } else fast_s = 0;
                    }
                }
                __syncthreads();
                if (fast_s == 2) return;
            }
        }
    }

    if (staged) for (long long i = tid; i < nfull; i += kPeakThreads) tstats[i] = stats[tf + i];
    __syncthreads();
    if (has_full) {
        for (long long t = tf + tid; t < tl; t += kPeakThreads) {
            if (!((stats[t].y - seg_min) >= min_prom)) continue;
            if (pol.order || (staged ? tile_can_qualify(tstats, t, tf, tl, min_prom) : tile_can_qualify(stats + tf, t, tf, tl, min_prom))) {
                const int slot = atomicAdd(&cand_n, 1);
                if (slot < kCandCap) cand_tiles[slot] = (int)(t - tf);
            }
        }
    }
    __shared__ float pmm_s[4][kWaves];
    __shared__ int piece_can_s;
    {
        float hmn = FLT_MAX, hmx = -FLT_MAX, tmn = FLT_MAX, tmx = -FLT_MAX;
        if (has_full) {
            for (long long i = a + tid; i < head_hi; i += kPeakThreads) {
                hmn = fminf(hmn, score_for_min(g, sp, i)); hmx = fmaxf(hmx, score_for_cmp(g, sp, i));
            }
            for (long long i = tail_lo + tid; i < b; i += kPeakThreads) {
                tmn = fminf(tmn, score_for_min(g, sp, i)); tmx = fmaxf(tmx, score_for_cmp(g, sp, i));
            }
        }
        hmn = wave_min(hmn); hmx = wave_max(hmx); tmn = wave_min(tmn); tmx = wave_max(tmx);
        if (lane == 0) { pmm_s[0][wv] = hmn; pmm_s[1][wv] = hmx; pmm_s[2][wv] = tmn; pmm_s[3][wv] = tmx; }
    }
    __syncthreads();
    if (tid == 0) {
        int can = (head_hi > a ? 1 : 0) | (b > tail_lo ? 2 : 0);
        if (has_full && !pol.order) {
            const float2* tl_stats = staged ? tstats : stats + tf;
            float m = FLT_MAX, M = -FLT_MAX;
            for (int k = 0; k < kWaves; ++k) { m = fminf(m, pmm_s[0][k]); M = fmaxf(M, pmm_s[1][k]); }
            if ((can & 1) && !((M - m) >= min_prom)) {
                float L = m;
                for (long long u = 0; u < nfull && u < kBoundSteps; ++u) {
                    const float2 v = tl_stats[u];
                    L = fminf(L, v.x);
                    if ((M - L) >= min_prom) break;
                    if (v.y > M) { can &= ~1; break; }
                }
            }
            m = FLT_MAX; M = -FLT_MAX;
            for (int k = 0; k < kWaves; ++k) { m = fminf(m, pmm_s[2][k]); M = fmaxf(M, pmm_s[3][k]); }
            if ((can & 2) && !((M - m) >= min_prom)) {
                float L = m;
                for (long long u = nfull - 1; u >= 0 && u >= nfull - kBoundSteps; --u) {
                    const float2 v = tl_stats[u];
                    L = fminf(L, v.x);
                    if ((M - L) >= min_prom) break;
                    if (v.y > M) { can &= ~2; break; }
                }
            }
        }
        piece_can_s = can;
    }
    __syncthreads();
    const int piece_can = piece_can_s;
    if (cand_n == 0 && piece_can == 0) {
        if (tid == 0) { hdr[blockIdx.x].n = 0; hdr[blockIdx.x].overflow = 0; hdr[blockIdx.x].seg_min = seg_min; hdr[blockIdx.x].arena_off = -1; }
        return;
    }
    if (cand_n > kWideTiles && wide.list != nullptr) {
        const bool listed = cand_n <= kCandCap;
        if (listed) for (int i = tid; i < cand_n; i += kPeakThreads) wide.tiles[(size_t)blockIdx.x * kCandCap + i] = cand_tiles[i];
        if (tid == 0) {
            wide.seg_min[blockIdx.x] = seg_min; wide.count[blockIdx.x] = 0; wide.best[blockIdx.x] = 0ull;
            wide.ntiles[blockIdx.x] = listed ? cand_n : -1;
            wide.state[blockIdx.x] = 1 | (piece_can << 1);
        }
        return;
    }
    const bool all_tiles = cand_n > kCandCap;
    const long long nmid = has_full ? (all_tiles ? (tl - tf) : cand_n) : 0;
    ChunkView cv{g, stats, sp, a, b, seg_min, min_prom, pol.order};
    const bool best_mode = min_dist >= b - a && b - a < 0xFFFFFFFFll;
    auto emit = [&](long long ps, long long pe, float h, float prom) {
        if (best_mode) { atomicMax(&best_s, best_key(h, ps - a)); return; }
        const int slot = atomicAdd(&res_n, 1);
        if (slot < AM_MAX_PEAKS_PER_CHUNK) {
            res[slot].start = (uint64_t)ps; res[slot].end = (uint64_t)pe;
            res[slot].height = h; res[slot].prominence = prom;
        } else overflow = 1;
    };
    const long long npieces = nmid + 2;
    for (long long pc = 0; pc < npieces; ++pc) {
        long long lo, hi;
        if (pc == 0) { lo = a; hi = (piece_can & 1) ? head_hi : a; }
        else if (pc == npieces - 1) { lo = tail_lo; hi = (piece_can & 2) ? b : tail_lo; }
        else {
            const long long t = tf + (all_tiles ? (pc - 1) : (long long)cand_tiles[pc - 1]);
            lo = t * kTile; hi = lo + kTile;
            if (all_tiles && !((stats[t].y - seg_min) >= min_prom && (pol.order || tile_can_qualify(stats + tf, t, tf, tl, min_prom)))) continue;
        }
        for (long long q0 = lo; q0 < hi; q0 += kTile)
            scan_piece(cv, q0, q0 + kTile < hi ? q0 + kTile : hi, win, wruns, queue, kQueueCap, &queue_n, &overflow, tid, emit);
    }
    if (best_mode) {
        finish_best(cv, best_s, my_out, &hdr[blockIdx.x], &pe_s, tid);
        return;
    }
    const int rn = res_n < AM_MAX_PEAKS_PER_CHUNK ? res_n : AM_MAX_PEAKS_PER_CHUNK;
    finish_chunk(res, rn, order, overflow, min_dist, seg_min, my_out, &hdr[blockIdx.x], arena, &kept_s, &spill_off_s, tid, pol);
}

__global__ void __launch_bounds__(kPeakThreads)
peaks_wide(const float* g, long long g_len, const float2* stats,
           const Segment* __restrict__ segs, int nsegs, float min_prom, long long min_dist, SparseScores sp, WideState wide, PeakPolicy pol,
           PickGroup grp) {
    __shared__ Cand queue[kWideQueue];
    __shared__ int queue_n;
    __shared__ int overflow;
    __shared__ float win[kWin];
    __shared__ float2 wruns[kWinRuns];
    const int part = blockIdx.x, tid = threadIdx.x;
    if (grp.n > 0) {
        SegHeader* no_hdr = nullptr; am_peak* no_out = nullptr;
        pick_group_view(grp, blockIdx.z, (unsigned)nsegs, g, stats, sp, no_hdr, no_out, wide);
    }
    for (int seg = blockIdx.y; seg < nsegs; seg += gridDim.y) {
    if (!(wide.state[seg] & 1)) continue;
    const Segment sg = segs[seg];
    const long long a = sg.a, b = sg.b < g_len ? sg.b : g_len;
    const long long tf = (a + kTile - 1) / kTile;
    const long long tl = b / kTile;
    const bool has_full = tl > tf;
    const long long head_hi = has_full ? tf * kTile : b;
    const long long tail_lo = has_full ? tl * kTile : b;
    const float seg_min = wide.seg_min[seg];
    if (tid == 0) { queue_n = 0; overflow = 0; }
    __syncthreads();
    ChunkView cv{g, stats, sp, a, b, seg_min, min_prom, pol.order};
    am_peak* list = wide.list + (size_t)seg * wide.cap;
    const bool best_mode = min_dist >= b - a && b - a < 0xFFFFFFFFll;
    auto emit = [&](long long ps, long long pe, float h, float prom) {
        if (best_mode) { atomicMax(&wide.best[seg], best_key(h, ps - a)); return; }
        const unsigned slot = atomicAdd(&wide.count[seg], 1u);
        if (slot < wide.cap) {
            am_peak pk; pk.start = (uint64_t)ps; pk.end = (uint64_t)pe; pk.height = h; pk.prominence = prom;
            list[slot] = pk;
        }
    };
    const int st = wide.state[seg];
    if (part == 0 && (st & 2))
        for (long long q0 = a; q0 < head_hi; q0 += kTile)
            scan_piece(cv, q0, q0 + kTile < head_hi ? q0 + kTile : head_hi, win, wruns, queue, kWideQueue, &queue_n, &overflow, tid, emit);
    if (part == 1 % kWideParts && (st & 4) && b > tail_lo) scan_piece(cv, tail_lo, b, win, wruns, queue, kWideQueue, &queue_n, &overflow, tid, emit);
    const int nlisted = wide.ntiles[seg];
    if (has_full && nlisted >= 0) {
        const int* tiles = wide.tiles + (size_t)seg * kCandCap;
        for (int k = part; k < nlisted; k += kWideParts) {
            const long long t = tf + tiles[k];
            scan_piece(cv, t * kTile, (t + 1) * kTile, win, wruns, queue, kWideQueue, &queue_n, &overflow, tid, emit);
        }
    } else if (has_full) {
        for (long long t = tf + part; t < tl; t += kWideParts) {
            if (!((stats[t].y - seg_min) >= min_prom && (pol.order || tile_can_qualify(stats + tf, t, tf, tl, min_prom)))) continue;
            scan_piece(cv, t * kTile, (t + 1) * kTile, win, wruns, queue, kWideQueue, &queue_n, &overflow, tid, emit);
        }
    }
    if (tid == 0 && overflow) atomicAdd(&wide.count[seg], 0x40000000u);
    __syncthreads();
    }
}

constexpr int kBigThreads = 256;
__global__ void __launch_bounds__(kBigThreads)
peaks_big_finish(const am_peak* __restrict__ list, unsigned n, long long a, long long min_dist,
                 unsigned long long* keys, unsigned* idx, long long* table, am_peak* __restrict__ out, unsigned* out_n, PeakPolicy pol) {
    __shared__ unsigned cnt[16 * kBigThreads];
    __shared__ unsigned part[kBigThreads];
    const int tid = threadIdx.x;
    unsigned long long* k0 = keys; unsigned long long* k1 = keys + n;
    unsigned* i0 = idx; unsigned* i1 = idx + n;
    for (unsigned i = tid; i < n; i += kBigThreads) { k0[i] = best_key(list[i].height, (long long)list[i].start - a); i0[i] = i; }
    const unsigned per = (n + kBigThreads - 1) / kBigThreads;
    const unsigned lo = (unsigned)tid * per < n ? (unsigned)tid * per : n;
    const unsigned hi = lo + per < n ? lo + per : n;
    for (int pass = 0; pass < 16; ++pass) {
        __syncthreads();
        const unsigned long long* kin = (pass & 1) ? k1 : k0;
        unsigned long long* kout = (pass & 1) ? k0 : k1;
        const unsigned* iin = (pass & 1) ? i1 : i0;
        unsigned* iout = (pass & 1) ? i0 : i1;
        const int sh = 4 * pass;
#pragma unroll
        for (int d = 0; d < 16; ++d) cnt[d * kBigThreads + tid] = 0;
        for (unsigned i = lo; i < hi; ++i) ++cnt[(15 - (int)((kin[i] >> sh) & 15ull)) * kBigThreads + tid];
        __syncthreads();
        unsigned sum = 0;
#pragma unroll
        for (int j = 0; j < 16; ++j) sum += cnt[tid * 16 + j];
        part[tid] = sum;
        __syncthreads();
        if (tid == 0) { unsigned run = 0; for (int t = 0; t < kBigThreads; ++t) { const unsigned v = part[t]; part[t] = run; run += v; } }
        __syncthreads();
        unsigned run = part[tid];
#pragma unroll
        for (int j = 0; j < 16; ++j) { const unsigned v = cnt[tid * 16 + j]; cnt[tid * 16 + j] = run; run += v; }
        __syncthreads();
        for (unsigned i = lo; i < hi; ++i) {
            const unsigned long long k = kin[i];
            const unsigned pos = cnt[(15 - (int)((k >> sh) & 15ull)) * kBigThreads + tid]++;
            kout[pos] = k; iout[pos] = iin[i];
        }
    }
    __syncthreads();
    if (tid >= 64) return;
    const int lane = tid;
    unsigned kept = 0;
    for (unsigned base = 0; base < n; base += 64) {
        const unsigned i = base + lane;
        bool ok = i < n;
        am_peak pk; pk.start = 0; pk.end = 0; pk.height = 0.f; pk.prominence = 0.f;
        long long mid = 0, bkt = 0;
        if (ok) {
            pk = list[i0[i]];
            mid = dist_pos(pk, pol.from_start) - a;
            if (min_dist > 0) {
                bkt = mid / min_dist;
                for (long long bb = bkt > 0 ? bkt - 1 : 0; bb <= bkt + 1 && ok; ++bb) {
                    const long long m = __hip_atomic_load(&table[bb], __ATOMIC_RELAXED, __HIP_MEMORY_SCOPE_AGENT);
                    if (m >= 0) { const long long d = mid > m ? mid - m : m - mid; if (too_close(d, min_dist, pol.inclusive)) ok = false; }
                }
            }
        }
        bool keep = ok;
        if (min_dist > 0) {
            keep = false;
            unsigned long long pending = __ballot(ok);
            while (pending) {
                const int L = __ffsll((long long)pending) - 1;
                const long long midL = ((long long)__shfl((int)(mid >> 32), L) << 32) | (unsigned)__shfl((int)(mid & 0xffffffffll), L);
                if (lane == L) keep = true;
                if (ok && lane > L) { const long long d = mid > midL ? mid - midL : midL - mid; if (too_close(d, min_dist, pol.inclusive)) ok = false; }
                pending = __ballot(ok && lane > L);
            }
        }
        const bool result = keep && !(pol.order && !(pk.prominence == pk.prominence));
        const unsigned long long kb = __ballot(result);
        if (result) out[kept + (unsigned)__popcll(kb & ((1ull << lane) - 1ull))] = pk;
        if (keep && min_dist > 0) __hip_atomic_store(&table[bkt], mid, __ATOMIC_RELAXED, __HIP_MEMORY_SCOPE_AGENT);
        kept += (unsigned)__popcll(kb);
        __builtin_amdgcn_fence(__ATOMIC_SEQ_CST, "agent");
    }
    if (lane == 0) *out_n = kept;
}

__global__ void __launch_bounds__(kPeakThreads)
peaks_finish(const float* g, long long g_len, const float2* stats,
             const Segment* __restrict__ segs, float min_prom, long long min_dist, am_peak* out,
             SegHeader* hdr, SparseScores sp, PeakArena arena, WideState wide, PeakPolicy pol, PickGroup grp) {
    __shared__ am_peak res[AM_MAX_PEAKS_PER_CHUNK];
    __shared__ int order[AM_MAX_PEAKS_PER_CHUNK];
    __shared__ int kept_s, spill_off_s;
    __shared__ long long pe_s;
    const int seg = blockIdx.x, tid = threadIdx.x;
    if (grp.n > 0) pick_group_view(grp, blockIdx.y, gridDim.x, g, stats, sp, hdr, out, wide);
    if (!(wide.state[seg] & 1)) return;
    am_peak* my_out = out + (size_t)seg * AM_MAX_PEAKS_PER_CHUNK;
    const Segment sg = segs[seg];
    const long long a = sg.a, b = sg.b < g_len ? sg.b : g_len;
    if (min_dist >= b - a && b - a < 0xFFFFFFFFll) {
        ChunkView cv{g, stats, sp, a, b, wide.seg_min[seg], min_prom, pol.order};
        finish_best(cv, wide.best[seg], my_out, &hdr[seg], &pe_s, tid);
        return;
    }
    const unsigned cnt = wide.count[seg];
    const int rn = cnt < (unsigned)AM_MAX_PEAKS_PER_CHUNK ? (int)cnt : AM_MAX_PEAKS_PER_CHUNK;
    const am_peak* list = wide.list + (size_t)seg * AM_MAX_PEAKS_PER_CHUNK;
    for (int i = tid; i < rn; i += kPeakThreads) res[i] = list[i];
    __syncthreads();
    finish_chunk(res, rn, order, cnt > (unsigned)AM_MAX_PEAKS_PER_CHUNK ? 1 : 0, min_dist, wide.seg_min[seg],
                 my_out, &hdr[seg], arena, &kept_s, &spill_off_s, tid, pol);
}

__global__ void __launch_bounds__(256) sumsq_kernel(const float* __restrict__ x, long long n, double* out) {
    __shared__ double part[4];
    double acc = 0.0;
    for (long long i = (long long)blockIdx.x * 256 + threadIdx.x; i < n; i += (long long)gridDim.x * 256) {
        const double v = (double)x[i];
        acc += v * v;
    }
#pragma unroll
    for (int o = 32; o > 0; o >>= 1) acc += __shfl_xor(acc, o);
    if ((threadIdx.x & 63) == 0) part[threadIdx.x >> 6] = acc;
    __syncthreads();
    if (threadIdx.x == 0) out[blockIdx.x] = (part[0] + part[1]) + (part[2] + part[3]);
}

__device__ __forceinline__ uint32_t fmix32(uint32_t h) {
    h ^= h >> 16; h *= 0x85ebca6bu; h ^= h >> 13; h *= 0xc2b2ae35u; h ^= h >> 16; return h;
}

__global__ void __launch_bounds__(256) synth_kernel(float* __restrict__ out, uint32_t seed, uint32_t stream,
                                                    uint64_t first, long long n, float amp) {
    const uint32_t key = fmix32(seed * 0x9E3779B9u + stream * 0x7F4A7C15u + 0x01234567u);
    for (long long k = (long long)blockIdx.x * 256 + threadIdx.x; k < n; k += (long long)gridDim.x * 256) {
        const uint64_t i = first + (uint64_t)k;
        uint32_t h = fmix32((uint32_t)i ^ key);
        h = fmix32(h + stream * 0x9E3779B9u + (uint32_t)(i >> 32) * 0xC2B2AE35u + seed);
        const int32_t v = (int32_t)(h >> 8) - (1 << 23);
        out[k] = ((float)v * (1.0f / 8388608.0f)) * amp;
    }
}

__device__ __forceinline__ float synth_value(uint32_t seed, uint32_t stream, uint64_t i, float amp) {
    const uint32_t key = fmix32(seed * 0x9E3779B9u + stream * 0x7F4A7C15u + 0x01234567u);
    uint32_t h = fmix32((uint32_t)i ^ key);
    h = fmix32(h + stream * 0x9E3779B9u + (uint32_t)(i >> 32) * 0xC2B2AE35u + seed);
    const int32_t v = (int32_t)(h >> 8) - (1 << 23);
    return __fmul_rn(__fmul_rn((float)v, 1.0f / 8388608.0f), amp);
}
__device__ __forceinline__ short to_s16(float x) {
    const float r = rintf(__fmul_rn(x, 32767.0f));
    return (short)fminf(fmaxf(r, -32768.0f), 32767.0f);
}
__global__ void __launch_bounds__(256) synth_pcm16_kernel(short2* __restrict__ out, uint32_t seed, uint32_t stream,
                                                          uint64_t first, long long frames, float amp) {
    for (long long k = (long long)blockIdx.x * 256 + threadIdx.x; k < frames; k += (long long)gridDim.x * 256) {
        const uint64_t i = first + (uint64_t)k;
        out[k] = make_short2(to_s16(synth_value(seed, stream, i, amp)), to_s16(synth_value(seed, stream + 5000u, i, amp)));
    }
}
__global__ void __launch_bounds__(256) add_pcm16_kernel(short* __restrict__ dst, const short* __restrict__ src, long long n) {
    for (long long k = (long long)blockIdx.x * 256 + threadIdx.x; k < n; k += (long long)gridDim.x * 256) {
        const int v = (int)dst[k] + (int)src[k];
        dst[k] = (short)(v < -32768 ? -32768 : (v > 32767 ? 32767 : v));
    }
}

__global__ void __launch_bounds__(256) axpy_kernel(float* __restrict__ dst, const float* __restrict__ src, long long n, float gain) {
    for (long long k = (long long)blockIdx.x * 256 + threadIdx.x; k < n; k += (long long)gridDim.x * 256)
        dst[k] = __fadd_rn(dst[k], __fmul_rn(gain, src[k]));
}

__global__ void __launch_bounds__(256) pcm_downmix_kernel(const int16_t* __restrict__ in, long long frames, float* __restrict__ out) {
    const float pcm_factor = 1.0f / 65535.0f;
    const short2* in2 = reinterpret_cast<const short2*>(in);
    for (long long k = (long long)blockIdx.x * 256 + threadIdx.x; k < frames; k += (long long)gridDim.x * 256) {
        const short2 lr = in2[k];
        const float sum = __fadd_rn((float)lr.x, (float)lr.y);
        out[k] = __fmul_rn(__fmul_rn(sum, 0.5f), pcm_factor);
    }
}

__global__ void __launch_bounds__(256) nonfinite_ranges_kernel(const float* __restrict__ x, const Segment* __restrict__ ranges,
                                                               int* __restrict__ flags) {
    const Segment r = ranges[blockIdx.y];
    bool found = false;
    for (long long i = r.a + (long long)blockIdx.x * 256 + threadIdx.x; i < r.b; i += (long long)gridDim.x * 256)
        found |= !(fabsf(x[i]) <= FLT_MAX);
    if (found) flags[blockIdx.y] = 1;
}

static inline int grid_for(long long n) {
    long long b = (n + 255) / 256;
    if (b < 1) b = 1;
    if (b > 2048) b = 2048;
    return (int)b;
}

hipError_t launch_tile_stats(hipStream_t st, const float* g, long long n, float2* stats, int* bad) {
    const long long tiles = (n + kTile - 1) / kTile;
    if (tiles <= 0) return hipSuccess;
    hipLaunchKernelGGL(tile_stats, dim3((unsigned)tiles), dim3(256), 0, st, g, n, stats, bad);
    return hipGetLastError();
}

hipError_t launch_stats_reduce(hipStream_t st, const float2* stats32, long long n, float2* stats, int* bad, const PickGroup* grp) {
    const long long n32 = (n + 31) / 32;
    const long long tiles = (n + kTile - 1) / kTile;
    if (tiles <= 0) return hipSuccess;
    const long long blocks = (tiles * 8 + 255) / 256;
    const PickGroup none{};
    hipLaunchKernelGGL(stats_reduce, dim3((unsigned)blocks, grp ? (unsigned)grp->n : 1u), dim3(256), 0, st, stats32, n32, stats, tiles, bad,
                       grp ? *grp : none);
    return hipGetLastError();
}

hipError_t launch_peaks(hipStream_t st, const float* g, long long g_len, const float2* stats,
                        const Segment* d_segs, int nsegs, float min_prom, long long min_dist,
                        am_peak* d_out, SegHeader* d_hdr, const SparseScores& sp, const PeakArena& arena,
                        const WideState& wide, bool only_failed, const PeakPolicy& pol, const PickGroup* grp) {
    if (nsegs <= 0) return hipSuccess;
    const PickGroup none{};
    const PickGroup& pg = grp ? *grp : none;
    const unsigned nz = grp ? (unsigned)grp->n : 1u;
    hipLaunchKernelGGL(peaks_kernel, dim3(nsegs, nz), dim3(kPeakThreads), 0, st, g, g_len, stats, d_segs,
                       min_prom, min_dist, d_out, d_hdr, sp, arena, wide, only_failed ? 1 : 0, pol, pg);
    if (wide.list != nullptr) {
        hipLaunchKernelGGL(peaks_wide, dim3(kWideParts, nsegs < kWideRows ? nsegs : kWideRows, nz), dim3(kPeakThreads), 0, st, g, g_len, stats, d_segs,
                           nsegs, min_prom, min_dist, sp, wide, pol, pg);
        hipLaunchKernelGGL(peaks_finish, dim3(nsegs, nz), dim3(kPeakThreads), 0, st, g, g_len, stats, d_segs, min_prom, min_dist,
                           d_out, d_hdr, sp, arena, wide, pol, pg);
    }
    return hipGetLastError();
}

hipError_t launch_nonfinite_ranges(hipStream_t st, const float* x, const Segment* ranges, int nranges, int* flags) {
    if (nranges <= 0) return hipSuccess;
    hipLaunchKernelGGL(nonfinite_ranges_kernel, dim3(64, nranges), dim3(256), 0, st, x, ranges, flags);
    return hipGetLastError();
}

hipError_t launch_peaks_wide_one(hipStream_t st, const float* g, long long g_len, const float2* stats, const Segment* d_seg,
                                 float min_prom, long long min_dist, const SparseScores& sp, const WideState& wide, const PeakPolicy& pol) {
    hipLaunchKernelGGL(peaks_wide, dim3(kWideParts, 1), dim3(kPeakThreads), 0, st, g, g_len, stats, d_seg, 1, min_prom, min_dist, sp, wide, pol, PickGroup{});
    return hipGetLastError();
}
hipError_t launch_peaks_big_finish(hipStream_t st, const am_peak* list, unsigned n, long long a, long long min_dist,
                                   unsigned long long* keys, unsigned* idx, long long* table, am_peak* out, unsigned* out_n,
                                   const PeakPolicy& pol) {
    hipLaunchKernelGGL(peaks_big_finish, dim3(1), dim3(kBigThreads), 0, st, list, n, a, min_dist, keys, idx, table, out, out_n, pol);
    return hipGetLastError();
}

int sumsq_parts(long long n) { return grid_for(n); }

hipError_t launch_sumsq(hipStream_t st, const float* x, long long n, double* d_parts) {
    hipLaunchKernelGGL(sumsq_kernel, dim3(grid_for(n)), dim3(256), 0, st, x, n, d_parts);
    return hipGetLastError();
}

hipError_t launch_synth(hipStream_t st, float* out, uint32_t seed, uint32_t stream, uint64_t first,
                        long long n, float amp) {
    hipLaunchKernelGGL(synth_kernel, dim3(grid_for(n)), dim3(256), 0, st, out, seed, stream, first, n, amp);
    return hipGetLastError();
}

hipError_t launch_synth_pcm16(hipStream_t st, int16_t* out, uint32_t seed, uint32_t stream, uint64_t first, long long frames, float amp) {
    hipLaunchKernelGGL(synth_pcm16_kernel, dim3(grid_for(frames)), dim3(256), 0, st, reinterpret_cast<short2*>(out), seed, stream, first, frames, amp);
    return hipGetLastError();
}

hipError_t launch_add_pcm16(hipStream_t st, int16_t* dst, const int16_t* src, long long frames) {
    hipLaunchKernelGGL(add_pcm16_kernel, dim3(grid_for(2 * frames)), dim3(256), 0, st, dst, src, 2 * frames);
    return hipGetLastError();
}

hipError_t launch_axpy(hipStream_t st, float* dst, const float* src, long long n, float gain) {
    hipLaunchKernelGGL(axpy_kernel, dim3(grid_for(n)), dim3(256), 0, st, dst, src, n, gain);
    return hipGetLastError();
}

hipError_t launch_pcm_downmix(hipStream_t st, const int16_t* in, long long frames, float* out) {
    hipLaunchKernelGGL(pcm_downmix_kernel, dim3(grid_for(frames)), dim3(256), 0, st, in, frames, out);
    return hipGetLastError();
}

}
```

Baseline: 226.3 billion.

## Cache chunk plan across calls, fuse wide-pick gating, and run last item's pick on the main stream

Adds a per-context call key that reuses the chunk plan and the resident segment upload when parameters, haystack lengths and presence match the previous call. It also skips the arena cursor memset when the cursor is known to be clean. A grid-wide counter at the end of the peaks kernel records whether any segment needs the wide pass, so the peaks_wide and peaks_finish kernels exit early when none does. The last haystack item picks directly on the main stream, and completion is drained by spinning on an event query. The aim is to cut host planning, H2D copies, memsets, stream syncs and empty kernel work in the per-call pipeline. The cost is cache invalidation complexity, reliance on a self-resetting device atomic counter, and CPU spin-waiting.

Result: no change. 228.6 billion, median of 3 (+1.0%).

```diff
diff --git a/audio-matcher_amd/build.py b/audio-matcher_amd/build.py
--- a/audio-matcher_amd/build.py
+++ b/audio-matcher_amd/build.py
@@ -12,7 +12,7 @@
 LIB = os.path.join(HERE, "libaudiomatch_amd.so")
 SOURCES = ["am_fft.hip", "am_peaks.hip", "am_context.hip", "am_correlate.hip", "am_engine.hip", "am_stream.hip", "am_monitor.hip", "am_pool.hip", "am_norm.hip", "am_hits.hip", "am_segments.hip", "am_bands.hip", "am_significance.hip", "am_resample.hip", "am_whiten.hip", "am_estimate.hip",
            "am_best.hip", "am_api.hip"]
-HEADERS = [os.path.join(CSRC, "am_kernels.h"), os.path.join(CSRC, "am_internal.h"), os.path.join(CSRC, "am_walk.h"), os.path.join(CSRC, "am_spans.h"),
+HEADERS = [os.path.join(CSRC, "am_kernels.h"), os.path.join(CSRC, "am_internal.h"), os.path.join(CSRC, "am_walk.h"), os.path.join(CSRC, "am_spans.h"), os.path.join(CSRC, "am_callkey.h"),
            os.path.join(HERE, "..", "include", "audiomatch.h")]
 ARCH = "gfx950"
 FLAGS = ["-O3", "-std=c++17", "-fPIC", f"--offload-arch={ARCH}", "-ffp-contract=fast", "-fno-slp-vectorize",
@@ -113,6 +113,16 @@
     return out
 
 
+def build_callkey_check() -> str:
+    out = os.path.join(OBJ, "am_callkey_check")
+    os.makedirs(OBJ, exist_ok=True)
+    src = os.path.join(HOST, "callkey_check.cpp")
+    if _stale(out, [src, os.path.join(CSRC, "am_callkey.h"), os.path.join(HERE, "..", "include", "audiomatch.h")]):
+        subprocess.check_call([_hipcc(), "-O1", "-g", "-std=c++17", "-x", "c++", "-Xarch_host", "-fsanitize=address,undefined",
+                               "-fno-sanitize-recover=undefined", src, "-o", out])
+    return out
+
+
 if __name__ == "__main__":
     print(build_library(force="--force" in sys.argv, verbose=True))
     print(build_cli(force="--force" in sys.argv))
diff --git a/audio-matcher_amd/csrc/am_callkey.h b/audio-matcher_amd/csrc/am_callkey.h
--- /dev/null
+++ b/audio-matcher_amd/csrc/am_callkey.h
@@ -0,0 +1,45 @@
+#pragma once
+#include <stddef.h>
+#include <stdint.h>
+#include <string.h>
+
+#include <vector>
+
+#include "../../include/audiomatch.h"
+
+namespace am {
+
+struct CallKey {
+    bool valid = false;
+    am_match_params p{};
+    size_t s = 0;
+    long long extra[3] = {0, 0, 0};
+    std::vector<size_t> lens;
+    std::vector<unsigned char> present;
+
+    static bool params_equal(const am_match_params& a, const am_match_params& b) {
+        return a.sr == b.sr && a.chunk == b.chunk && a.overlap == b.overlap &&
+               memcmp(&a.min_prominence, &b.min_prominence, sizeof(float)) == 0 && a.min_distance == b.min_distance &&
+               memcmp(&a.overshadow_distance_s, &b.overshadow_distance_s, sizeof(double)) == 0 && a.scale == b.scale;
+    }
+    bool same(const am_match_params& p_, size_t s_, const long long (&extra_)[3], const void* const* hays, const size_t* lens_, size_t n) const {
+        if (!valid || n != lens.size() || s_ != s || !params_equal(p_, p)) return false;
+        for (int i = 0; i < 3; ++i)
+            if (extra_[i] != extra[i]) return false;
+        if (n && memcmp(lens_, lens.data(), n * sizeof(size_t)) != 0) return false;
+        for (size_t k = 0; k < n; ++k)
+            if ((hays[k] != nullptr) != (present[k] != 0)) return false;
+        return true;
+    }
+    void store(const am_match_params& p_, size_t s_, const long long (&extra_)[3], const void* const* hays, const size_t* lens_, size_t n) {
+        p = p_; s = s_;
+        for (int i = 0; i < 3; ++i) extra[i] = extra_[i];
+        lens.assign(lens_, lens_ + n);
+        present.resize(n);
+        for (size_t k = 0; k < n; ++k) present[k] = hays[k] != nullptr;
+        valid = true;
+    }
+    void forget() { valid = false; }
+};
+
+}
diff --git a/audio-matcher_amd/csrc/am_context.hip b/audio-matcher_amd/csrc/am_context.hip
--- a/audio-matcher_amd/csrc/am_context.hip
+++ b/audio-matcher_amd/csrc/am_context.hip
@@ -54,6 +54,7 @@
     {"pick_group", {1}, opt_bool, &Opts::pick_group},
     {"k3_group", {1}, opt_bool, &Opts::k3_group},
     {"host_pick_wait", {1}, opt_bool, &Opts::host_pick_wait},
+    {"pick_fused", {1}, opt_bool, &Opts::pick_fused},
     {"device_redo", {1}, opt_bool, &Opts::device_redo},
     {"tail_block", {1}, opt_bool, &Opts::tail_block},
     {"dense_scores", {0}, opt_bool, &Opts::dense},
@@ -129,6 +130,8 @@
         (void)hipEventCreateWithFlags(&c->ev_k3[i], kSyncEvent);
         (void)hipEventCreateWithFlags(&c->ev_pick[i], kSyncEvent);
     }
+    (void)hipEventCreateWithFlags(&c->ev_done, hipEventDisableTiming);
+    (void)hipGetLastError();
     g_ctx[device] = c;
     *out = c;
     return AM_OK;
@@ -462,7 +465,7 @@
         for (ScoreSide& sd : c->side)
             for (DevBuf* b : {&sd.scores, &sd.stats, &sd.stats32, &sd.wflags, &sd.peaks, &sd.work}) b->release();
         for (DevBuf* b : {&c->work2, &c->segs, &c->redo_pairs[0], &c->redo_pairs[1],
-                          &c->io_in, &c->io_out, &c->sum, &c->arena_cur, &c->wide_ctl, &c->wide_list, &c->wide_tiles})
+                          &c->io_in, &c->io_out, &c->sum, &c->arena_cur, &c->wide_ctl, &c->wide_list, &c->wide_tiles, &c->wide_sync})
             b->release();
         for (HostBuf* b : {&c->pinned, &c->hdr, &c->spill, &c->badflag, &c->failcnt}) b->release();
         c->ranges.release(); c->range_flags.release(); c->big.release(); c->norm_blk.release();
@@ -480,6 +483,7 @@
             for (int i = 0; i < kMaxNeedleGroup; ++i) { c->grp_scores[set][i].release(); c->grp_stats32[set][i].release(); c->grp_wflags[set][i].release(); }
         for (int i = 0; i < kMaxNeedleGroup; ++i) c->grp_stats[i].release();
         c->segs_resident.clear();
+        c->call_key.forget(); c->call_plan.reset(); c->arena_clean = false;
         for (auto& pk : c->plans) { if (pk.second.tables) (void)hipFree(pk.second.tables); if (pk.second.mf) (void)hipFree(pk.second.mf); }
         c->plans.clear();
         for (auto& r : c->pending) { (void)hipEventDestroy(r.e0); (void)hipEventDestroy(r.e1); }
diff --git a/audio-matcher_amd/csrc/am_correlate.hip b/audio-matcher_amd/csrc/am_correlate.hip
--- a/audio-matcher_amd/csrc/am_correlate.hip
+++ b/audio-matcher_amd/csrc/am_correlate.hip
@@ -319,15 +319,18 @@
     AM_HIP(hipMemcpyAsync(c->segs.p, c->pinned.p, bytes, hipMemcpyHostToDevice, c->stream));
     AM_HIP(hipStreamSynchronize(c->stream));
     c->segs_resident = segs;
-    return AM_OK;
-}
-
-int prepare_results(Ctx* c, size_t nhdr, size_t arena_entries, PeakArena* arena) {
+    ++c->segs_gen;
+    return AM_OK;
+}
+
+int prepare_results(Ctx* c, size_t nhdr, size_t arena_entries, PeakArena* arena, bool keep_clean) {
     const size_t hdr_bytes = (sizeof(SegHeader) * nhdr + 63) / 64 * 64;
     int rc;
     if ((rc = c->hdr.ensure(hdr_bytes + sizeof(am_peak) * arena_entries))) return rc;
+    if (!c->arena_cur.p) c->arena_clean = false;
     if ((rc = c->arena_cur.ensure(sizeof(unsigned)))) return rc;
-    AM_HIP(hipMemsetAsync(c->arena_cur.p, 0, sizeof(unsigned), c->stream));
+    if (!(keep_clean && c->arena_clean)) AM_HIP(hipMemsetAsync(c->arena_cur.p, 0, sizeof(unsigned), c->stream));
+    c->arena_clean = false;
     arena->base = reinterpret_cast<am_peak*>(static_cast<char*>(c->hdr.p) + hdr_bytes);
     arena->cursor = static_cast<unsigned*>(c->arena_cur.p);
     arena->cap = (unsigned)arena_entries;
@@ -336,6 +339,11 @@
 
 int wide_reserve(Ctx* c, size_t n) {
     int rc;
+    if (!c->wide_sync.p) {
+        if ((rc = c->wide_sync.ensure(2 * sizeof(unsigned)))) return rc;
+        AM_HIP(hipMemsetAsync(c->wide_sync.p, 0, 2 * sizeof(unsigned), c->stream));
+        AM_HIP(hipStreamSynchronize(c->stream));
+    }
     if ((rc = c->wide_ctl.ensure(n * kWideCtlBytes))) return rc;
     if ((rc = c->wide_list.ensure(n * AM_MAX_PEAKS_PER_CHUNK * sizeof(am_peak)))) return rc;
     return c->wide_tiles.ensure(n * kWideTileList * sizeof(int));
@@ -350,12 +358,13 @@
     wide.tiles = static_cast<int*>(c->wide_tiles.p);
     wide.list = static_cast<am_peak*>(c->wide_list.p);
     wide.cap = AM_MAX_PEAKS_PER_CHUNK;
+    wide.sync = snapshot_opts(nullptr).pick_fused ? static_cast<unsigned*>(c->wide_sync.p) : nullptr;
     return wide;
 }
 
 int launch_pick(Ctx* c, ScoreSide& side, const float* d_scores, long long n_scores, int seg_off, int nsegs,
                        float min_prom, long long min_dist, int* bad, const ScanResult* res, int hdr_off,
-                       const PeakArena& arena, const PeakPolicy& pol, hipStream_t st, bool only_failed) {
+                       const PeakArena& arena, const PeakPolicy& pol, hipStream_t st, bool only_failed, const TailCommit* tail) {
     if (!st) st = c->stream;
     const SparseScores sp = (res && res->fused) ? res->sparse : plain_scores();
     if (nsegs == 0 || n_scores <= 0) return AM_OK;
@@ -364,7 +373,11 @@
     if ((rc = side.stats.ensure((size_t)ntiles * sizeof(float2)))) return rc;
     if (!only_failed) {
         ProfScope ps(c, KN_STATS, st);
-        if (sp.stats32) AM_HIP(launch_stats_reduce(st, sp.stats32, n_scores, (float2*)side.stats.p, bad));
+        if (tail) {
+            ProfScope pc(c, KN_OTHER, st);
+            if (!sp.stats32) return fail(AM_ERR_INVALID_ARG, "internal: a tail commit needs the level-0 summary");
+            AM_HIP(launch_stats_reduce(st, sp.stats32, n_scores, (float2*)side.stats.p, bad, nullptr, tail));
+        } else if (sp.stats32) AM_HIP(launch_stats_reduce(st, sp.stats32, n_scores, (float2*)side.stats.p, bad));
         else AM_HIP(launch_tile_stats(st, d_scores, n_scores, (float2*)side.stats.p, bad));
     }
     if ((rc = wide_reserve(c, (size_t)nsegs))) return rc;
diff --git a/audio-matcher_amd/csrc/am_engine.hip b/audio-matcher_amd/csrc/am_engine.hip
--- a/audio-matcher_amd/csrc/am_engine.hip
+++ b/audio-matcher_amd/csrc/am_engine.hip
@@ -30,15 +30,6 @@
 }
 
 
-struct ChunkPlan {
-    std::vector<Segment> segs, short_segs;
-    std::vector<size_t> widths, short_w;
-    std::vector<int> seg_off, short_off;
-    std::vector<int> n_chunks;
-    size_t max_scores = 0, max_segs = 1;
-    int ns(size_t k) const { return seg_off[k + 1] - seg_off[k]; }
-    bool too_many(size_t nn) const { return max_segs > (size_t)1 << 18 || segs.size() * nn > (size_t)1 << 24; }
-};
 static void plan_chunks(size_t s, const void* const* d_hays, const size_t* lens, size_t n_hay, const am_match_params* p, const Opts& o,
                         bool split_short, size_t max_windows, ChunkPlan* cp) {
     const size_t window = (size_t)(p->chunk + p->overlap);
@@ -67,15 +58,18 @@
 
 struct ScoreSets {
     Ctx* c;
-    bool overlap;
+    bool overlap, fused;
+    bool direct = false;
     size_t seq = 0;
     ScoreSets(Ctx* c_, const Opts& o, size_t n_items)
-        : c(c_), overlap(o.batch_overlap && n_items > 1 && c_->stream2 && c_->ev_k3[0] && c_->ev_k3[1] && c_->ev_pick[0] && c_->ev_pick[1]) {}
+        : c(c_), overlap(o.batch_overlap && n_items > 1 && c_->stream2 && c_->ev_k3[0] && c_->ev_k3[1] && c_->ev_pick[0] && c_->ev_pick[1]),
+          fused(o.pick_fused != 0 && c_->ev_done != nullptr) {}
     int count() const { return overlap ? 2 : 1; }
     int set() const { return overlap ? (int)(seq & 1) : 0; }
     ScoreSide& side() const { return c->side[set()]; }
     float* scores() const { return (float*)side().scores.p; }
-    hipStream_t pick_stream() const { return overlap ? c->stream2 : c->stream; }
+    hipStream_t pick_stream() const { return overlap && !direct ? c->stream2 : c->stream; }
+    void last_item() { direct = fused && overlap && seq > 0; }
     int size(size_t max_scores, size_t max_segs) {
         int rc;
         for (int set = 0; set < count(); ++set) {
@@ -94,20 +88,36 @@
     }
     int k3_done() {
         if (!overlap) return AM_OK;
+        if (direct) {
+            AM_HIP(hipEventSynchronize(c->ev_pick[set() ^ 1]));
+            return AM_OK;
+        }
         AM_HIP(hipEventRecord(c->ev_k3[set()], c->stream));
         AM_HIP(hipStreamWaitEvent(c->stream2, c->ev_k3[set()], 0));
         return AM_OK;
     }
     int pick_done() {
-        if (overlap) AM_HIP(hipEventRecord(c->ev_pick[set()], c->stream2));
+        if (overlap && !direct) AM_HIP(hipEventRecord(c->ev_pick[set()], c->stream2));
         ++seq;
         return AM_OK;
     }
     int drain() {
+        if (fused && (direct || !overlap)) {
+            AM_HIP(hipEventRecord(c->ev_done, c->stream));
+            for (int spin = 0; spin < kDrainSpins; ++spin) {
+                const hipError_t e = hipEventQuery(c->ev_done);
+                if (e == hipSuccess) { (void)hipGetLastError(); return AM_OK; }
+                if (e != hipErrorNotReady) return hip_fail(e, "hipEventQuery(ev_done)");
+            }
+            (void)hipGetLastError();
+            AM_HIP(hipEventSynchronize(c->ev_done));
+            return AM_OK;
+        }
         AM_HIP(hipStreamSynchronize(c->stream));
         if (overlap) AM_HIP(hipStreamSynchronize(c->stream2));
         return AM_OK;
     }
+    static constexpr int kDrainSpins = 1 << 16;
 };
 
 static int match_alone(am_needle* h, const void* d_hay, size_t len, const am_match_params* p, am_peak* out, size_t cap, size_t slot,
@@ -126,6 +136,7 @@
     PeakArena own{};
     if ((rc = c->spill.ensure(sizeof(am_peak) * AM_MAX_PEAKS_PER_CHUNK))) return rc;
     AM_HIP(hipMemsetAsync(c->arena_cur.p, 0, sizeof(unsigned), c->stream));
+    c->arena_clean = false;
     own.base = static_cast<am_peak*>(c->spill.p); own.cursor = static_cast<unsigned*>(c->arena_cur.p);
     own.cap = AM_MAX_PEAKS_PER_CHUNK;
     ScoreSide& side = c->side[0];
@@ -233,8 +244,11 @@
     base.seg_c = (long long)p->chunk;
     base.seg_d = (long long)(p->chunk + p->overlap) - (long long)s;
     for (size_t k = 0; k < n_hay; ++k) n_out[G(k)] = 0;
-    ChunkPlan cp;
-    plan_chunks(s, d_hays, lens, n_hay, p, o, my, part ? part->max_windows : (size_t)-1, &cp);
+    const long long key_extra[3] = {my ? 1 : 0, o.tail_window != 0 ? 1 : 0, part ? (long long)part->max_windows : -1};
+    const bool same_inputs = o.pick_fused && c->call_plan && c->call_key.same(*p, s, key_extra, d_hays, lens, n_hay);
+    std::shared_ptr<ChunkPlan> cp_hold = same_inputs ? c->call_plan : std::make_shared<ChunkPlan>();
+    if (!same_inputs) plan_chunks(s, d_hays, lens, n_hay, p, o, my, part ? part->max_windows : (size_t)-1, cp_hold.get());
+    const ChunkPlan& cp = *cp_hold;
     const std::vector<Segment>& segs = cp.segs;
     const std::vector<int>& seg_off = cp.seg_off;
     const size_t nsegs = segs.size();
@@ -278,12 +292,21 @@
         if (need.side && (rc = c->side[set].wflags.ensure(need.side))) return rc;
     }
     PeakArena arena{};
-    if ((rc = prepare_results(c, nsegs + 1, std::min<size_t>(cp.max_segs * AM_MAX_PEAKS_PER_CHUNK, (size_t)1 << 20) + nsegs * 8, &arena))) return rc;
-    std::vector<Segment> resident = segs;
-    for (const Segment& sg : cp.short_segs) resident.push_back(Segment{0, sg.b - sg.a});
-    const int local_seg = (int)resident.size();
-    resident.push_back(Segment{0, std::max<long long>(base.seg_d + 1, 1)});
-    if ((rc = upload_segments(c, resident))) return rc;
+    if ((rc = prepare_results(c, nsegs + 1, std::min<size_t>(cp.max_segs * AM_MAX_PEAKS_PER_CHUNK, (size_t)1 << 20) + nsegs * 8, &arena,
+                              o.pick_fused != 0))) return rc;
+    const int local_seg = (int)(nsegs + cp.short_segs.size());
+    if (!(same_inputs && c->call_segs_gen == c->segs_gen && c->segs.p)) {
+        std::vector<Segment> resident = segs;
+        for (const Segment& sg : cp.short_segs) resident.push_back(Segment{0, sg.b - sg.a});
+        resident.push_back(Segment{0, std::max<long long>(base.seg_d + 1, 1)});
+        c->call_key.forget();
+        if ((rc = upload_segments(c, resident))) return rc;
+        if (o.pick_fused) {
+            c->call_plan = cp_hold;
+            c->call_key.store(*p, s, key_extra, d_hays, lens, n_hay);
+            c->call_segs_gen = c->segs_gen;
+        }
+    }
     if ((rc = c->badflag.ensure(sizeof(int) * n_hay))) return rc;
     int* h_bad = static_cast<int*>(c->badflag.p);
     memset(h_bad, 0, sizeof(int) * n_hay);
@@ -309,6 +332,9 @@
     };
     const bool arm_forced = o.debug_redo_arm_at >= -1;
     bool redo_armed = device_redo && (arm_forced ? o.debug_redo_arm_at == 0 : h->redo_armed_left[sm] > 0);
+    size_t last_k = n_hay;
+    for (size_t k = 0; k < n_hay; ++k)
+        if (cp.n_chunks[k] != 0 && cp.ns(k) > 0) last_k = k;
     QueueingScope queueing(o.debug_no_realloc != 0);
     for (size_t k = 0; k < n_hay; ++k) {
         const int ns = cp.ns(k);
@@ -321,6 +347,7 @@
         if (hooks.fn) hooks.fn(hooks.user, G(k), 0, (size_t)cp.n_chunks[k]);
         chunk_events(k, 0);
         if (ns == 0) continue;
+        if (k == last_k) sets.last_item();
         const long long out_count = (long long)(lens[k] - s + 1);
         const int set = sets.set();
         const PassPlan& pp = plans[k];
@@ -359,16 +386,28 @@
         ScanResult res{};
         if ((rc = run_correlation(h, o, d_hays[k], (long long)lens[k], 0, d_scores, out_count, factor, &req, &res, src_kind, &pp))) return rc;
         if ((rc = sets.k3_done())) return rc;
+        const hipStream_t pst = sets.pick_stream();
+        TailCommit tcm{};
+        bool tail_in_pick = false;
         if (req.tail_by_caller && res.fused) {
             const TailPlan& t = pp.tail;
             const BallotLayout bl = ballot_layout(res.sparse.log_n1, res.sparse.log_n2);
             const size_t blk = (size_t)(t.T / res.sparse.hop);
-            ProfScope ps(c, KN_OTHER, c->stream2);
-            AM_HIP(launch_tail_commit(c->stream2, static_cast<const float*>(c->tail_scores.p) + (size_t)tail_slot[k] * tslots.scores, d_scores + t.T,
-                                      out_count - t.T, static_cast<const float2*>(c->tail_stats.p) + (size_t)tail_slot[k] * tslots.stats,
-                                      const_cast<float2*>(res.sparse.stats32) + t.T / 32,
-                                      res.sparse.wbits ? const_cast<unsigned long long*>(res.sparse.wbits) + blk * bl.words : nullptr, (long long)bl.words,
-                                      res.sparse.tile_theta ? const_cast<float*>(res.sparse.tile_theta) + blk * bl.tiles : nullptr, (int)bl.tiles));
+            tcm.tail_scores = static_cast<const float*>(c->tail_scores.p) + (size_t)tail_slot[k] * tslots.scores;
+            tcm.scores = d_scores;
+            tcm.tail_stats32 = static_cast<const float2*>(c->tail_stats.p) + (size_t)tail_slot[k] * tslots.stats;
+            tcm.stats32 = const_cast<float2*>(res.sparse.stats32);
+            tcm.T = t.T; tcm.n = out_count - t.T;
+            tcm.wbits = res.sparse.wbits ? const_cast<unsigned long long*>(res.sparse.wbits) + blk * bl.words : nullptr;
+            tcm.words = (long long)bl.words;
+            tcm.theta = res.sparse.tile_theta ? const_cast<float*>(res.sparse.tile_theta) + blk * bl.tiles : nullptr;
+            tcm.tiles = (int)bl.tiles;
+            tail_in_pick = o.pick_fused && !nrm.on && t.T % kTile == 0;
+            if (!tail_in_pick) {
+                ProfScope ps(c, KN_OTHER, pst);
+                AM_HIP(launch_tail_commit(pst, tcm.tail_scores, d_scores + t.T, tcm.n, tcm.tail_stats32, tcm.stats32 + t.T / 32,
+                                          tcm.wbits, tcm.words, tcm.theta, tcm.tiles));
+            }
         }
         if (res.fused && res.sparse.wbits) {
             res.sparse.fail_flags = h_fail + seg_off[k];
@@ -379,21 +418,27 @@
                 return rc;
         }
         if ((rc = launch_pick(c, side, d_scores, out_count, seg_off[k], ns, p->min_prominence,
-                              (long long)p->min_distance, bad, nrm.on ? nullptr : &res, seg_off[k], arena, pol, sets.pick_stream()))) return rc;
+                              (long long)p->min_distance, bad, nrm.on ? nullptr : &res, seg_off[k], arena, pol, pst, false,
+                              tail_in_pick ? &tcm : nullptr))) return rc;
         if (res.fused && res.sparse.redo_pairs) {
             ScanCfg cfg = res.redo_cfg;
             cfg.margin = -1.0f;
             cfg.only_pairs = d_redo;
-            { ProfScope ps(c, KN_OTHER, c->stream2);
-              AM_HIP(launch_k3(c->stream2, res.redo_job, res.redo_npairs, res.redo_work, res.redo_pl, res.redo_scale, cfg, res.redo_half)); }
+            { ProfScope ps(c, KN_OTHER, pst);
+              AM_HIP(launch_k3(pst, res.redo_job, res.redo_npairs, res.redo_work, res.redo_pl, res.redo_scale, cfg, res.redo_half)); }
             res.sparse.redo_pairs = nullptr; res.sparse.fail_flags = nullptr;
             if ((rc = launch_pick(c, side, d_scores, out_count, seg_off[k], ns, p->min_prominence, (long long)p->min_distance,
-                                  nullptr, &res, seg_off[k], arena, pol, c->stream2, true))) return rc;
+                                  nullptr, &res, seg_off[k], arena, pol, pst, true))) return rc;
         }
         if ((rc = sets.pick_done())) return rc;
     }
     queueing.end();
     if ((rc = sets.drain())) return rc;
+    if (o.pick_fused) {
+        bool clean = true;
+        for (size_t i = 0; i < nsegs && clean; ++i) clean = h_hdr[i].n <= kInlinePeaks;
+        c->arena_clean = clean;
+    }
     int worst = AM_OK;
     std::vector<am_peak> all;
     std::vector<size_t> retry_f32;
diff --git a/audio-matcher_amd/csrc/am_internal.h b/audio-matcher_amd/csrc/am_internal.h
--- a/audio-matcher_amd/csrc/am_internal.h
+++ b/audio-matcher_amd/csrc/am_internal.h
@@ -6,10 +6,12 @@
 #include <cstdio>
 #include <cstring>
 #include <map>
+#include <memory>
 #include <mutex>
 #include <string>
 #include <vector>
 
+#include "am_callkey.h"
 #include "am_kernels.h"
 #include "am_spans.h"
 
@@ -35,7 +37,7 @@
 struct Opts {
     long long log_n, pairs_per_group, half, batch_overlap, needle_group, dense, device_redo, debug_no_realloc, debug_redo_arm_at;
     long long peak_filter_order, distance_rule, tail_window, surrounding_from, k3_group, pick_group, tail_block, host_pick_wait;
-    long long profile_mask, profile_every, pick_priority;
+    long long profile_mask, profile_every, pick_priority, pick_fused;
     long long score_norm, score_norm_floor_db;
     PeakPolicy peak_policy() const { return PeakPolicy{(int)peak_filter_order, (int)(distance_rule & 1), (int)((distance_rule >> 1) & 1)}; }
 };
@@ -107,6 +109,16 @@
 
 struct ScoreSide { DevBuf scores, stats, stats32, wflags, peaks, work; };
 
+struct ChunkPlan {
+    std::vector<Segment> segs, short_segs;
+    std::vector<size_t> widths, short_w;
+    std::vector<int> seg_off, short_off;
+    std::vector<int> n_chunks;
+    size_t max_scores = 0, max_segs = 1;
+    int ns(size_t k) const { return seg_off[k + 1] - seg_off[k]; }
+    bool too_many(size_t nn) const { return max_segs > (size_t)1 << 18 || segs.size() * nn > (size_t)1 << 24; }
+};
+
 struct ProfRec { int name; hipEvent_t e0, e1; };
 enum { KN_K1 = 0, KN_K2, KN_K3, KN_STATS, KN_PEAKS, KN_OTHER, KN_COUNT };
 
@@ -122,6 +134,7 @@
     std::map<int, Plan> plans;
     ScoreSide side[2];
     DevBuf work2, segs, io_in, io_out, sum, arena_cur, wide_ctl, wide_list, wide_tiles;
+    DevBuf wide_sync;
     DevBuf norm_blk;
     DevBuf hit_tab, hit_parts, hit_flags, hit_out, hit_stage;
     HostBuf hit_io;
@@ -134,6 +147,7 @@
     DevBuf grp_stats[kMaxNeedleGroup];
     HostBuf failcnt;
     hipEvent_t ev_k3[2] = {nullptr, nullptr}, ev_pick[2] = {nullptr, nullptr};
+    hipEvent_t ev_done = nullptr;
     HostBuf pinned;
     HostBuf hdr;
     HostBuf spill;
@@ -142,6 +156,10 @@
     DevBuf big;
     DevBuf best_stats, best_lmax, best_ctl, best_trans, best_list, best_scores, best_mono;
     std::vector<Segment> segs_resident;
+    CallKey call_key;
+    std::shared_ptr<ChunkPlan> call_plan;
+    uint64_t segs_gen = 0, call_segs_gen = 0;
+    bool arena_clean = false;
     bool prof = false;
     std::vector<ProfRec> pending;
     std::vector<hipEvent_t> pool;
@@ -452,13 +470,14 @@
 void make_segments(size_t len, size_t s, const am_match_params* p, bool drop_tail, std::vector<Segment>& segs,
                    std::vector<size_t>* widths = nullptr, size_t max_windows = (size_t)-1);
 int upload_segments(Ctx* c, const std::vector<Segment>& segs);
-int prepare_results(Ctx* c, size_t nhdr, size_t arena_entries, PeakArena* arena);
+int prepare_results(Ctx* c, size_t nhdr, size_t arena_entries, PeakArena* arena, bool keep_clean = false);
 constexpr size_t kWideCtlBytes = sizeof(unsigned long long) + sizeof(int) + sizeof(unsigned) + sizeof(float) + sizeof(int);
 int wide_reserve(Ctx* c, size_t n);
 WideState wide_carve(Ctx* c, size_t n);
 int launch_pick(Ctx* c, ScoreSide& side, const float* d_scores, long long n_scores, int seg_off, int nsegs,
                 float min_prom, long long min_dist, int* bad, const ScanResult* res, int hdr_off,
-                const PeakArena& arena, const PeakPolicy& pol, hipStream_t st = nullptr, bool only_failed = false);
+                const PeakArena& arena, const PeakPolicy& pol, hipStream_t st = nullptr, bool only_failed = false,
+                const TailCommit* tail = nullptr);
 int pick_chunk_big(Ctx* c, const float* d_scores, long long n_scores, int seg_idx, const Segment& sg,
                    float min_prom, long long min_dist, const ScanResult* res, float seg_min,
                    std::vector<am_peak>& all, const PeakPolicy& pol);
diff --git a/audio-matcher_amd/csrc/am_kernels.h b/audio-matcher_amd/csrc/am_kernels.h
--- a/audio-matcher_amd/csrc/am_kernels.h
+++ b/audio-matcher_amd/csrc/am_kernels.h
@@ -125,8 +125,15 @@
     const float* theta[kMaxNeedleGroup];
     int hdr_off[kMaxNeedleGroup];
 };
+struct TailCommit {
+    const float* tail_scores; float* scores;
+    const float2* tail_stats32; float2* stats32;
+    long long T, n;
+    unsigned long long* wbits; long long words;
+    float* theta; int tiles;
+};
 hipError_t launch_stats_reduce(hipStream_t st, const float2* stats32, long long n, float2* stats, int* bad = nullptr,
-                               const PickGroup* grp = nullptr);
+                               const PickGroup* grp = nullptr, const TailCommit* tail = nullptr);
 constexpr int kInlinePeaks = 4;
 struct SegHeader {
     int n;
@@ -158,6 +165,7 @@
     unsigned cap;
     int* ntiles;
     int* tiles;
+    unsigned* sync;
 };
 constexpr int kWideTileList = 1024;
 struct PeakPolicy {
diff --git a/audio-matcher_amd/csrc/am_peaks.hip b/audio-matcher_amd/csrc/am_peaks.hip
--- a/audio-matcher_amd/csrc/am_peaks.hip
+++ b/audio-matcher_amd/csrc/am_peaks.hip
@@ -33,15 +33,46 @@
 
 __device__ __forceinline__ bool bad_run(float mn, float mx) { return !(mn <= mx) || not_finite(mn) || not_finite(mx); }
 __global__ void __launch_bounds__(256) stats_reduce(const float2* __restrict__ s32, long long n32,
-                                                    float2* __restrict__ stats, long long ntiles, int* bad, PickGroup grp) {
+                                                    float2* __restrict__ stats, long long ntiles, int* bad, PickGroup grp, TailCommit tc) {
     if (grp.n > 0) { s32 = grp.stats32[blockIdx.y]; stats = grp.stats[blockIdx.y]; }
     const long long gid = (long long)blockIdx.x * 256 + threadIdx.x;
     const long long tile = gid >> 3;
     const int l = threadIdx.x & 7;
     float mn = FLT_MAX, mx = -FLT_MAX;
     const long long idx = tile * 32 + 4 * l;
+    const long long tile0 = tc.n > 0 ? tc.T / kTile : ntiles;
+    if (tc.n > 0 && ((long long)blockIdx.x + 1) * 32 > tile0) {
+        const long long w0 = (long long)blockIdx.x * 32 * kTile;
+        const long long lo = w0 > tc.T ? w0 - tc.T : 0;
+        const long long hi = w0 + 32 * kTile - tc.T < tc.n ? w0 + 32 * kTile - tc.T : tc.n;
+        float* __restrict__ sc = tc.scores + tc.T;
+        if (((reinterpret_cast<uintptr_t>(tc.tail_scores) | reinterpret_cast<uintptr_t>(sc)) & 15) == 0) {
+            const float4* __restrict__ t4 = reinterpret_cast<const float4*>(tc.tail_scores);
+            float4* __restrict__ s4 = reinterpret_cast<float4*>(sc);
+            const long long hi4 = hi >> 2;
+            for (long long i = (lo >> 2) + threadIdx.x; i < hi4; i += 256) s4[i] = t4[i];
+            for (long long i = (hi4 << 2) + threadIdx.x; i < hi; i += 256) sc[i] = tc.tail_scores[i];
+        } else {
+            for (long long i = lo + threadIdx.x; i < hi; i += 256) sc[i] = tc.tail_scores[i];
+        }
+        const long long first_wg = tile0 / 32, nth = ((long long)gridDim.x - first_wg) * 256;
+        const long long me = ((long long)blockIdx.x - first_wg) * 256 + threadIdx.x;
+        if (tc.wbits != nullptr)
+            for (long long i = me; i < tc.words; i += nth) tc.wbits[i] = ~0ull;
+        if (tc.theta != nullptr)
+            for (long long i = me; i < tc.tiles; i += nth) tc.theta[i] = -FLT_MAX;
+    }
     if (tile < ntiles) {
-        if (idx + 3 < n32) {
+        if (tile >= tile0) {
+            const long long t32 = tc.T / 32;
+            for (int k = 0; k < 4; ++k)
+                if (idx + k < n32) {
+                    const float2 v = tc.tail_stats32[idx + k - t32];
+                    tc.stats32[idx + k] = v;
+                    mn = fminf(mn, v.x); mx = fmaxf(mx, v.y);
+                    if (bad != nullptr && bad_run(v.x, v.y)) *bad = 1;
+                }
+        } else if (idx + 3 < n32) {
             const float4 a = *reinterpret_cast<const float4*>(s32 + idx);
             const float4 b = *reinterpret_cast<const float4*>(s32 + idx + 2);
             mn = fminf(fminf(a.x, a.z), fminf(b.x, b.z));
@@ -366,11 +397,11 @@
     if (wide.list != nullptr) wide.list += zs * wide.cap;
 }
 
-__global__ void __launch_bounds__(kPeakThreads)
-peaks_kernel(const float* g, long long g_len, const float2* stats,
-             const Segment* __restrict__ segs, float min_prom, long long min_dist,
-             am_peak* out, SegHeader* hdr, SparseScores sp, PeakArena arena, WideState wide,
-             int only_failed, PeakPolicy pol, PickGroup grp) {
+__device__ __forceinline__ void
+pick_chunk(const float* g, long long g_len, const float2* stats,
+           const Segment* __restrict__ segs, float min_prom, long long min_dist,
+           am_peak* out, SegHeader* hdr, SparseScores sp, const PeakArena& arena, WideState wide,
+           int only_failed, const PeakPolicy& pol, const PickGroup& grp) {
     __shared__ float red[kWaves];
     __shared__ float seg_min_s;
     __shared__ Cand queue[kQueueCap];
@@ -638,6 +669,37 @@
 }
 
 __global__ void __launch_bounds__(kPeakThreads)
+peaks_kernel(const float* g, long long g_len, const float2* stats,
+             const Segment* __restrict__ segs, float min_prom, long long min_dist,
+             am_peak* out, SegHeader* hdr, SparseScores sp, PeakArena arena, WideState wide,
+             int only_failed, PeakPolicy pol, PickGroup grp) {
+    pick_chunk(g, g_len, stats, segs, min_prom, min_dist, out, hdr, sp, arena, wide, only_failed, pol, grp);
+    if (wide.sync == nullptr) return;
+    __shared__ int last_s;
+    __shared__ unsigned handed_s;
+    const int tid = threadIdx.x;
+    const unsigned total = gridDim.x * gridDim.y;
+    __syncthreads();
+    if (tid == 0) {
+        __threadfence();
+        last_s = atomicAdd(&wide.sync[0], 1u) == total - 1u;
+        handed_s = 0u;
+    }
+    __syncthreads();
+    if (!last_s) return;
+    __threadfence();
+    unsigned mine = 0u;
+    for (unsigned i = tid; i < total; i += kPeakThreads)
+        mine += (unsigned)(__hip_atomic_load(&wide.state[i], __ATOMIC_RELAXED, __HIP_MEMORY_SCOPE_AGENT) & 1);
+    if (mine) atomicAdd(&handed_s, mine);
+    __syncthreads();
+    if (tid == 0) {
+        wide.sync[1] = handed_s;
+        __hip_atomic_store(&wide.sync[0], 0u, __ATOMIC_RELAXED, __HIP_MEMORY_SCOPE_AGENT);
+    }
+}
+
+__global__ void __launch_bounds__(kPeakThreads)
 peaks_wide(const float* g, long long g_len, const float2* stats,
            const Segment* __restrict__ segs, int nsegs, float min_prom, long long min_dist, SparseScores sp, WideState wide, PeakPolicy pol,
            PickGroup grp) {
@@ -647,6 +709,7 @@
     __shared__ float win[kWin];
     __shared__ float2 wruns[kWinRuns];
     const int part = blockIdx.x, tid = threadIdx.x;
+    if (wide.sync != nullptr && wide.sync[1] == 0u) return;
     if (grp.n > 0) {
         SegHeader* no_hdr = nullptr; am_peak* no_out = nullptr;
         pick_group_view(grp, blockIdx.z, (unsigned)nsegs, g, stats, sp, no_hdr, no_out, wide);
@@ -789,6 +852,7 @@
     __shared__ int kept_s, spill_off_s;
     __shared__ long long pe_s;
     const int seg = blockIdx.x, tid = threadIdx.x;
+    if (wide.sync != nullptr && wide.sync[1] == 0u) return;
     if (grp.n > 0) pick_group_view(grp, blockIdx.y, gridDim.x, g, stats, sp, hdr, out, wide);
     if (!(wide.state[seg] & 1)) return;
     am_peak* my_out = out + (size_t)seg * AM_MAX_PEAKS_PER_CHUNK;
@@ -901,14 +965,20 @@
     return hipGetLastError();
 }
 
-hipError_t launch_stats_reduce(hipStream_t st, const float2* stats32, long long n, float2* stats, int* bad, const PickGroup* grp) {
+hipError_t launch_stats_reduce(hipStream_t st, const float2* stats32, long long n, float2* stats, int* bad, const PickGroup* grp,
+                               const TailCommit* tail) {
     const long long n32 = (n + 31) / 32;
     const long long tiles = (n + kTile - 1) / kTile;
     if (tiles <= 0) return hipSuccess;
     const long long blocks = (tiles * 8 + 255) / 256;
     const PickGroup none{};
+    TailCommit tc{};
+    if (tail != nullptr && tail->n > 0) {
+        if (grp != nullptr || tail->T % kTile != 0 || tail->T + tail->n != n || tail->stats32 != stats32) return hipErrorInvalidValue;
+        tc = *tail;
+    }
     hipLaunchKernelGGL(stats_reduce, dim3((unsigned)blocks, grp ? (unsigned)grp->n : 1u), dim3(256), 0, st, stats32, n32, stats, tiles, bad,
-                       grp ? *grp : none);
+                       grp ? *grp : none, tc);
     return hipGetLastError();
 }
 
@@ -939,7 +1009,9 @@
 
 hipError_t launch_peaks_wide_one(hipStream_t st, const float* g, long long g_len, const float2* stats, const Segment* d_seg,
                                  float min_prom, long long min_dist, const SparseScores& sp, const WideState& wide, const PeakPolicy& pol) {
-    hipLaunchKernelGGL(peaks_wide, dim3(kWideParts, 1), dim3(kPeakThreads), 0, st, g, g_len, stats, d_seg, 1, min_prom, min_dist, sp, wide, pol, PickGroup{});
+    WideState one = wide;
+    one.sync = nullptr;
+    hipLaunchKernelGGL(peaks_wide, dim3(kWideParts, 1), dim3(kPeakThreads), 0, st, g, g_len, stats, d_seg, 1, min_prom, min_dist, sp, one, pol, PickGroup{});
     return hipGetLastError();
 }
 hipError_t launch_peaks_big_finish(hipStream_t st, const am_peak* list, unsigned n, long long a, long long min_dist,
diff --git a/audio-matcher_amd/host/callkey_check.cpp b/audio-matcher_amd/host/callkey_check.cpp
--- /dev/null
+++ b/audio-matcher_amd/host/callkey_check.cpp
@@ -0,0 +1,92 @@
+#include <stdio.h>
+#include <stdlib.h>
+
+#include <vector>
+
+#include "../csrc/am_callkey.h"
+
+static int failures = 0;
+#define CHECK(cond)                                                          \
+    do {                                                                     \
+        if (!(cond)) { printf("FAIL %s:%d: %s\n", __FILE__, __LINE__, #cond); ++failures; } \
+    } while (0)
+
+static bool call(am::CallKey& key, const am_match_params& p, size_t s, const long long (&extra)[3], const std::vector<const void*>& hays,
+                 const std::vector<size_t>& lens) {
+    const bool same = key.same(p, s, extra, hays.data(), lens.data(), lens.size());
+    if (!same) {
+        key.forget();
+        key.store(p, s, extra, hays.data(), lens.data(), lens.size());
+    }
+    return same;
+}
+
+int main() {
+    am_match_params p{};
+    p.sr = 44100; p.chunk = 60 * 44100; p.overlap = 10 * 44100; p.min_prominence = 0.3f;
+    p.min_distance = 480 * 44100; p.overshadow_distance_s = 8.0; p.scale = 1;
+    const long long extra[3] = {0, 0, -1};
+    static const int dummy[8] = {0};
+    auto ptrs = [&](size_t n) { std::vector<const void*> v(n); for (size_t i = 0; i < n; ++i) v[i] = &dummy[i % 8]; return v; };
+    const std::vector<size_t> lens = {1000, 2000, 3000, 4000};
+
+    am::CallKey key;
+    CHECK(!call(key, p, 3000, extra, ptrs(4), lens));
+    CHECK(call(key, p, 3000, extra, ptrs(4), lens));
+    CHECK(call(key, p, 3000, extra, ptrs(4), std::vector<size_t>(lens)));
+    {
+        const std::vector<size_t> perm = {2000, 1000, 3000, 4000};
+        CHECK(!call(key, p, 3000, extra, ptrs(4), perm));
+        CHECK(call(key, p, 3000, extra, ptrs(4), perm));
+        CHECK(!call(key, p, 3000, extra, ptrs(4), lens));
+    }
+    {
+        const std::vector<size_t> shorter(lens.begin(), lens.begin() + 3);
+        std::vector<size_t> longer = lens; longer.push_back(5000);
+        CHECK(!call(key, p, 3000, extra, ptrs(3), shorter));
+        CHECK(call(key, p, 3000, extra, ptrs(3), shorter));
+        CHECK(!call(key, p, 3000, extra, ptrs(5), longer));
+        CHECK(!call(key, p, 3000, extra, ptrs(4), lens));
+        CHECK(!call(key, p, 3000, extra, ptrs(0), std::vector<size_t>()));
+        CHECK(call(key, p, 3000, extra, ptrs(0), std::vector<size_t>()));
+        CHECK(!call(key, p, 3000, extra, ptrs(4), lens));
+    }
+    {
+        std::vector<size_t> one = lens; one[3] += 1;
+        CHECK(!call(key, p, 3000, extra, ptrs(4), one));
+        CHECK(!call(key, p, 3000, extra, ptrs(4), lens));
+    }
+    {
+        am_match_params q = p; q.min_prominence = 0.31f; CHECK(!call(key, q, 3000, extra, ptrs(4), lens));
+        q = p; q.sr = 48000; CHECK(!call(key, q, 3000, extra, ptrs(4), lens));
+        q = p; q.chunk += 1; CHECK(!call(key, q, 3000, extra, ptrs(4), lens));
+        q = p; q.overlap += 1; CHECK(!call(key, q, 3000, extra, ptrs(4), lens));
+        q = p; q.min_distance += 1; CHECK(!call(key, q, 3000, extra, ptrs(4), lens));
+        q = p; q.overshadow_distance_s = 8.5; CHECK(!call(key, q, 3000, extra, ptrs(4), lens));
+        q = p; q.scale = 0; CHECK(!call(key, q, 3000, extra, ptrs(4), lens));
+        q = p; q.min_prominence = -0.0f; CHECK(!call(key, q, 3000, extra, ptrs(4), lens));
+        am_match_params z = p; z.min_prominence = 0.0f; CHECK(!call(key, z, 3000, extra, ptrs(4), lens));
+        CHECK(!call(key, p, 3000, extra, ptrs(4), lens));
+        CHECK(call(key, p, 3000, extra, ptrs(4), lens));
+    }
+    {
+        CHECK(!call(key, p, 3001, extra, ptrs(4), lens));
+        CHECK(!call(key, p, 3000, extra, ptrs(4), lens));
+        for (int i = 0; i < 3; ++i) {
+            long long e2[3] = {extra[0], extra[1], extra[2]};
+            e2[i] += 1;
+            CHECK(!call(key, p, 3000, e2, ptrs(4), lens));
+            CHECK(!call(key, p, 3000, extra, ptrs(4), lens));
+        }
+        std::vector<const void*> holes = ptrs(4);
+        holes[2] = nullptr;
+        CHECK(!call(key, p, 3000, extra, holes, lens));
+        CHECK(call(key, p, 3000, extra, holes, lens));
+        CHECK(!call(key, p, 3000, extra, ptrs(4), lens));
+    }
+    key.forget();
+    CHECK(!call(key, p, 3000, extra, ptrs(4), lens));
+    if (failures) printf("callkey_check: %d failure(s)\n", failures);
+    else printf("callkey_check: ok\n");
+    return failures ? 1 : 0;
+}
```
